# xinyandai/gradient-quantization

Hardware: NVIDIA B200
Metric: HSQ gradient elems/s (encode+allgather+decode) (higher is better)
Workload: dtype f32

## Files before the change

### gradient-quantization_b200/_lib.py

```python
import ctypes
import os

import torch

_HERE = os.path.dirname(os.path.abspath(__file__))
LIB_PATH = os.path.join(_HERE, "libgqb200.so")

c_void_p = ctypes.c_void_p
c_int = ctypes.c_int
c_i64 = ctypes.c_int64
c_u64 = ctypes.c_uint64
c_size = ctypes.c_size_t
c_float = ctypes.c_float

ALGO_AUTO, ALGO_EXACT, ALGO_TC = 0, 1, 2

_SIGNATURES = {
    "gq_abi_version": (c_int, []),
    "gq_device_info": (c_int, [ctypes.POINTER(c_int)] * 3 + [ctypes.POINTER(c_size)]),
    "gq_hsq_encode_workspace_bytes": (c_size, [c_i64, c_int, c_int, c_int]),
    "gq_hsq_encode": (c_int, [c_void_p, c_i64, c_int, c_void_p, c_int, c_void_p, c_int, c_int, c_int,
                              c_void_p, c_u64, c_u64, c_void_p, c_int, c_void_p, c_int, c_void_p,
                              c_void_p, c_void_p, c_size, c_int, c_void_p]),
    "gq_hsq_search": (c_int, [c_void_p, c_i64, c_int, c_void_p, c_int, c_void_p, c_int, c_void_p,
                              c_void_p, c_int, c_void_p, c_void_p, c_size, c_int, c_void_p]),
    "gq_norm_quantize": (c_int, [c_void_p, c_i64, c_void_p, c_int, c_int, c_int, c_void_p, c_u64, c_u64,
                                 c_void_p, c_int, c_void_p, c_void_p, c_int, c_void_p]),
    "gq_norm_dequantize": (c_int, [c_void_p, c_int, c_i64, c_void_p, c_int, c_int, c_void_p, c_void_p,
                                   c_void_p]),
    "gq_hsq_decode_reduce": (c_int, [c_void_p, c_int, c_void_p, c_int, c_void_p, c_void_p, c_i64, c_int,
                                     c_i64, c_int, c_void_p, c_int, c_void_p, c_int, c_int, c_int, c_int,
                                     c_void_p, c_void_p]),
    "gq_hsq_decode_reduce_scattered": (c_int, [c_void_p, c_int, c_void_p, c_int, c_void_p, c_void_p, c_int, c_i64,
                                               c_int, c_void_p, c_int, c_void_p, c_int, c_int, c_int, c_int,
                                               c_void_p, c_void_p]),
    "gq_f32_reduce_users_scattered": (c_int, [c_void_p, c_void_p, c_int, c_i64, c_int, c_int, c_void_p, c_void_p]),
    "gq_attach_f32_reduce": (c_int, [c_void_p, c_i64, c_void_p, c_int, c_i64, c_int, c_int, c_void_p]),
    "gq_ipc_alloc": (c_int, [c_size, ctypes.POINTER(c_void_p), c_void_p]),
    "gq_ipc_free": (c_int, [c_void_p]),
    "gq_ipc_open": (c_int, [c_void_p, ctypes.POINTER(c_void_p)]),
    "gq_ipc_close": (c_int, [c_void_p]),
    "gq_peer_barrier": (c_int, [c_void_p, c_int, c_int, ctypes.c_uint32, c_void_p]),
    "gq_peer_gather": (c_int, [c_void_p, c_void_p, c_size, c_size, c_int, c_void_p]),
    "gq_peer_push": (c_int, [c_void_p, c_void_p, c_size, c_int, c_void_p]),
    "gq_peer_push_multicast": (c_int, [c_void_p, c_void_p, c_size, c_void_p]),
    "gq_attach_remote_record": (c_int, [c_int, c_int, c_void_p, c_void_p, c_i64, c_void_p, c_int, ctypes.c_uint32]),
    "gq_attach_peer_wait": (c_int, [c_void_p, c_int, ctypes.c_uint32]),
    "gq_f32_reduce_users": (c_int, [c_void_p, c_i64, c_int, c_i64, c_int, c_int, c_void_p, c_void_p]),
    "gq_qsgd_wire_bits": (c_int, [c_int]),
    "gq_qsgd_encode": (c_int, [c_void_p, c_i64, c_void_p, c_i64, c_int, c_int, c_int, c_void_p, c_u64,
                               c_u64, c_void_p, c_void_p, c_void_p, c_void_p, c_void_p]),
    "gq_qsgd_decode_reduce": (c_int, [c_void_p, c_void_p, c_i64, c_int, c_i64, c_void_p, c_i64, c_int,
                                      c_int, c_int, c_int, c_void_p, c_void_p]),
    "gq_qsgd_decode_unpacked": (c_int, [c_void_p, c_void_p, c_void_p, c_i64, c_void_p, c_i64, c_int, c_int,
                                        c_void_p, c_void_p]),
    "gq_sign_encode": (c_int, [c_void_p, c_i64, c_void_p, c_void_p, c_void_p]),
    "gq_sign_decode_reduce": (c_int, [c_void_p, c_i64, c_int, c_i64, c_int, c_int, c_void_p, c_void_p]),
    "gq_sign_t5_bytes": (c_i64, [c_i64]),
    "gq_sign_encode_t5": (c_int, [c_void_p, c_i64, c_void_p, c_void_p]),
    "gq_sign_decode_reduce_t5": (c_int, [c_void_p, c_i64, c_int, c_i64, c_int, c_int, c_void_p, c_void_p]),
    "gq_topk_workspace_bytes": (c_size, [c_i64, c_int]),
    "gq_topk_select": (c_int, [c_void_p, c_i64, c_void_p, c_void_p, c_void_p, c_int, c_void_p, c_void_p,
                               c_void_p, c_void_p, c_size, c_void_p]),
    "gq_topk_scatter_reduce": (c_int, [c_void_p, c_void_p, c_i64, c_int, c_i64, c_i64, c_int, c_int,
                                       c_void_p, c_void_p]),
    "gq_pvc_search": (c_int, [c_void_p, c_i64, c_int, c_void_p, c_int, c_void_p, c_u64, c_u64, c_void_p,
                              c_int, c_void_p, c_void_p]),
    "gq_hsq_tc_debug": (c_int, [c_void_p, c_i64, c_void_p, c_void_p, c_void_p, c_void_p, c_int, c_void_p,
                                c_int, c_void_p]),
    "gq_hsq_tc2_trace": (c_int, [c_void_p, c_i64, c_void_p, c_void_p, c_void_p, c_void_p, c_int, c_void_p, c_void_p, c_void_p,
                                 c_void_p, c_void_p]),
    "gq_gather_f32": (c_int, [c_void_p, c_void_p, c_void_p, c_int, c_void_p, c_int, c_float, c_void_p]),
    "gq_axpy": (c_int, [c_void_p, c_void_p, c_float, c_i64, c_void_p, c_void_p]),
    "gq_sub": (c_int, [c_void_p, c_void_p, c_i64, c_void_p, c_void_p]),
    "gq_hsq_host_scratch_bytes": (c_size, [c_i64, c_int, c_int, c_int]),
    "gq_hsq_roundtrip_host": (c_int, [c_void_p, c_void_p, c_i64, c_int, c_void_p, c_int, c_void_p, c_int,
                                      c_int, c_int, c_u64, c_u64, c_void_p, c_size, c_int, c_void_p]),
}

EXPORTS = ["gq_last_error"] + sorted(_SIGNATURES)

_lib = None


class GQError(RuntimeError):
    pass


def load():
    global _lib
    if _lib is not None:
        return _lib
    if not os.path.exists(LIB_PATH):
        raise ImportError(
            "libgqb200.so is missing (%s). Build it with `python gradient-quantization_b200/build.py` "
            "or __graft_entry__.build(); there is no CPU fallback." % LIB_PATH)
    lib = ctypes.CDLL(LIB_PATH)
    lib.gq_last_error.restype = ctypes.c_char_p
    lib.gq_last_error.argtypes = []
    for name, (res, args) in _SIGNATURES.items():
        fn = getattr(lib, name)
        fn.restype = res
        fn.argtypes = args
    _lib = lib
    return lib


def call(name, *args):
    lib = load()
    rc = getattr(lib, name)(*args)
    if rc != 0:
        raise GQError("%s failed (%d): %s" % (name, rc, lib.gq_last_error().decode()))


def value(name, *args):
    return getattr(load(), name)(*args)


def require_cuda(t, what="tensor"):
    if not isinstance(t, torch.Tensor) or not t.is_cuda:
        raise GQError("%s must be a CUDA tensor: this implementation has no CPU path" % what)
    return t


def ptr(t):
    return None if t is None else t.data_ptr()


def stream():
    return torch.cuda.current_stream().cuda_stream


def f32c(t, what="tensor"):
    require_cuda(t, what)
    if t.dtype != torch.float32:
        t = t.float()
    return t if t.is_contiguous() else t.contiguous()


_M64 = 0xFFFFFFFFFFFFFFFF


def _mix64(seed, k):
    z = (seed + (k + 1) * 0x9E3779B97F4A7C15) & _M64
    z = ((z ^ (z >> 30)) * 0xBF58476D1CE4E5B9) & _M64
    z = ((z ^ (z >> 27)) * 0x94D049BB133111EB) & _M64
    return z ^ (z >> 31)


class PhiloxState:

    SHARED_STREAM = 1 << 32

    def __init__(self):
        self.shared_seed = None
        self.shared_offset = 0

    def _gen(self):
        return torch.cuda.default_generators[torch.cuda.current_device()]

    def take(self, n, user=0):
        gen = self._gen()
        seed = gen.initial_seed() & _M64
        off = int(gen.get_offset())
        gen.set_offset(off + (int(n) + 3) // 4 * 4)
        return _mix64(seed, int(user)), off

    def share_seed(self, seed=None):
        self.shared_seed = (self._gen().initial_seed() if seed is None else int(seed)) & _M64
        self.shared_offset = 0
        return self.shared_seed

    def take_shared(self, n):
        if self.shared_seed is None:
            self.share_seed()
        off = self.shared_offset
        self.shared_offset = off + (int(n) + 3) // 4 * 4
        return _mix64(self.shared_seed, self.SHARED_STREAM), off


PHILOX = PhiloxState()
```

### gradient-quantization_b200/csrc/abi.cu

```cuda
#include <stdarg.h>
#include <stdlib.h>
#include <string.h>

#include "gq_internal.cuh"

namespace gq {

static thread_local char g_err[512] = "";

void set_error(const char *fmt, ...)
{
    va_list ap;
    va_start(ap, fmt);
    vsnprintf(g_err, sizeof(g_err), fmt, ap);
    va_end(ap);
}

int check_cuda(cudaError_t e, const char *what)
{
    if (e == cudaSuccess) return GQ_OK;
    set_error("CUDA error %d (%s) at %s", (int)e, cudaGetErrorString(e), what);
    return GQ_ERR_CUDA;
}

int sm_count()
{
    static int cached[64] = {0};
    int dev = 0;
    if (cudaGetDevice(&dev) != cudaSuccess || dev < 0 || dev >= 64) return 148;
    if (cached[dev] == 0) {
        int n = 0;
        if (cudaDeviceGetAttribute(&n, cudaDevAttrMultiProcessorCount, dev) != cudaSuccess || n <= 0) n = 148;
        cached[dev] = n;
    }
    return cached[dev];
}

bool pdl_enabled()
{
    static const bool on = [] { const char *f = getenv("GQ_PDL"); return !(f && atoi(f) == 0); }();
    return on;
}

static size_t align_up(size_t x, size_t a) { return (x + a - 1) / a * a; }

int tc_generation()
{
    const char *f = getenv("GQ_TC_V");
    return (f && atoi(f) == 1) ? 1 : 2;
}

static thread_local Tc2Remote g_remote = {};
void set_remote(const Tc2Remote &r) { g_remote = r; }
Tc2Remote take_remote()
{
    Tc2Remote r = g_remote;
    g_remote = Tc2Remote{};
    return r;
}

}

using namespace gq;

extern "C" {

const char *gq_last_error(void) { return g_err; }
int gq_abi_version(void) { return 1; }

int gq_device_info(int *sm, int *cc_major, int *cc_minor, size_t *total_mem)
{
    int dev = 0;
    GQ_CUDA(cudaGetDevice(&dev));
    cudaDeviceProp p;
    GQ_CUDA(cudaGetDeviceProperties(&p, dev));
    if (sm) *sm = p.multiProcessorCount;
    if (cc_major) *cc_major = p.major;
    if (cc_minor) *cc_minor = p.minor;
    if (total_mem) *total_mem = p.totalGlobalMem;
    return GQ_OK;
}

size_t gq_hsq_encode_workspace_bytes(int64_t n_chunks, int d, int K, int n_seg)
{
    (void)d; (void)K;
    size_t keys = align_up((size_t)(n_seg > 0 ? n_seg : 1) * 2 * sizeof(uint32_t), 256);
    return keys + 256  + hsq_tc_workspace_bytes(n_chunks) + hsq_tck_workspace_bytes(d, K);
}

static int validate_group(const void *grad, int64_t n_chunks, int d, const void *codebook, int K,
                          const int64_t *seg_start, int n_seg)
{
    GQ_REQUIRE(n_chunks >= 0, "n_chunks %lld < 0", (long long)n_chunks);
    GQ_REQUIRE(d >= 1, "chunk dim %d < 1", d);
    GQ_REQUIRE(K >= 1, "codebook size %d < 1", K);
    GQ_REQUIRE(n_chunks == 0 || grad != nullptr, "null gradient pointer");
    GQ_REQUIRE(codebook != nullptr, "null codebook pointer");
    GQ_REQUIRE(n_seg >= 1 && seg_start != nullptr, "segment table required (n_seg >= 1)");
    return GQ_OK;
}

int gq_hsq_search(const float *grad, int64_t n_chunks, int d, const float *codebook, int K,
                  void *codes, int code_bytes, float *u_out, const int64_t *seg_start, int n_seg,
                  uint32_t *minmax_keys, void *workspace, size_t workspace_bytes, int algo,
                  gq_stream_t stream)
{
    int e = validate_group(grad, n_chunks, d, codebook, K, seg_start, n_seg);
    if (e) return e;
    GQ_REQUIRE(code_bytes == 1 || code_bytes == 4, "code_bytes must be 1 or 4 (got %d)", code_bytes);
    GQ_REQUIRE(code_bytes == 4 || K <= 256, "uint8 codes need K <= 256 (K = %d)", K);
    GQ_REQUIRE(n_chunks == 0 || (codes && u_out), "null output pointer");
    GQ_REQUIRE(((uintptr_t)grad & 15) == 0, "gradient must be 16-byte aligned");
    cudaStream_t st = as_stream(stream);
    const bool tc_ok = tc_generation() == 2 ? hsq_tc2_supported(d, K, code_bytes) : hsq_tc_supported(d, K, code_bytes);
    const bool tck_ok = !tc_ok && hsq_tck_supported(d, K, code_bytes) && workspace != nullptr &&
                        ((uintptr_t)workspace & 255) == 0 && workspace_bytes >= hsq_tck_workspace_bytes(d, K);
    if (algo == GQ_ALGO_TC && !tc_ok && !tck_ok) {
        set_error("tcgen05 search supports d in {8, 16, 32} with K == 256 (uint8 codes) or d == 16 with K = 512..4096, a multiple of 512 "
                  "(int32 codes, workspace of gq_hsq_encode_workspace_bytes); got d=%d K=%d code_bytes=%d",
                  d, K, code_bytes);
        return GQ_ERR_UNSUPPORTED;
    }
    if (tck_ok && algo != GQ_ALGO_EXACT && n_chunks > 0)
        return hsq_search_tck(grad, n_chunks, codebook, K, codes, u_out, seg_start, n_seg, minmax_keys, workspace,
                              workspace_bytes, st);
    if (tc_ok && algo != GQ_ALGO_EXACT && n_chunks > 0) {
        if (tc_generation() == 1)
            return hsq_search_tc(grad, n_chunks, d, codebook, K, codes, code_bytes, u_out, seg_start, n_seg,
                                 minmax_keys, workspace, workspace_bytes, st);
        return hsq_encode_tc2(grad, n_chunks, d, codebook, codes, u_out, seg_start, n_seg, minmax_keys, nullptr, nullptr,
                              Rider{}, nullptr, nullptr, st);
    }
    return hsq_search_exact(grad, n_chunks, d, codebook, K, codes, code_bytes, u_out, seg_start, n_seg,
                            minmax_keys, st);
}

int gq_hsq_tc2_trace(const float *grad, int64_t n_chunks, const float *codebook, void *codes, float *u_out,
                     const int64_t *seg_start, int n_seg, void *l, float *lbub, void *workspace, int64_t *trace,
                     gq_stream_t stream)
{
    GQ_REQUIRE(hsq_tc_supported(16, 256, 1), "tcgen05 search needs an sm_100 device");
    if (l == nullptr)
        return hsq_tc2_trace(grad, n_chunks, codebook, codes, u_out, nullptr, 0, nullptr, nullptr, nullptr, nullptr,
                             reinterpret_cast<long long *>(trace), as_stream(stream));
    GQ_REQUIRE(seg_start && n_seg >= 1 && lbub && workspace && ((uintptr_t)workspace & 255) == 0, "bad arguments");
    uint32_t *keys = reinterpret_cast<uint32_t *>(workspace);
    uint32_t *barrier = reinterpret_cast<uint32_t *>((char *)workspace + align_up((size_t)n_seg * 8, 256));
    Tc2Tail tail = {(uint8_t *)l, lbub, nullptr, 1234u, 0u, 6, 1};
    return hsq_tc2_trace(grad, n_chunks, codebook, codes, u_out, seg_start, n_seg, keys, reinterpret_cast<uint64_t *>(barrier) + 1,
                         barrier, &tail, reinterpret_cast<long long *>(trace), as_stream(stream));
}

int gq_norm_quantize(const float *u, int64_t n, const int64_t *seg_start, int n_seg, int n_bit,
                     int random, const float *uniforms, uint64_t philox_seed, uint64_t philox_offset,
                     void *l, int l_bytes, float *lbub, uint32_t *minmax_keys, int precomputed,
                     gq_stream_t stream)
{
    GQ_REQUIRE(n >= 0 && n_seg >= 1 && seg_start, "bad segment table");
    GQ_REQUIRE(n_bit >= 1 && n_bit <= 24, "n_bit %d out of range 1..24", n_bit);
    GQ_REQUIRE(l_bytes == 1 || l_bytes == 4, "l_bytes must be 1 or 4");
    GQ_REQUIRE(l_bytes == 4 || n_bit <= 7, "uint8 norm codes need n_bit <= 7 (levels 0..2^n)");
    GQ_REQUIRE(l && lbub && minmax_keys, "null output pointer");
    cudaStream_t st = as_stream(stream);
    if (!precomputed) {
        int e = launch_minmax_init(minmax_keys, n_seg, st);
        if (e) return e;
        e = launch_seg_minmax(u, n, seg_start, n_seg, minmax_keys, st);
        if (e) return e;
    }
    return launch_norm_quantize(u, n, seg_start, n_seg, n_bit, random, uniforms, philox_seed,
                                philox_offset, l, l_bytes, lbub, minmax_keys, st);
}

int gq_norm_dequantize(const void *l, int l_bytes, int64_t n, const int64_t *seg_start, int n_seg,
                       int n_bit, const float *lbub, float *out, gq_stream_t stream)
{
    GQ_REQUIRE(n >= 0 && n_seg >= 1 && seg_start, "bad segment table");
    GQ_REQUIRE(n_bit >= 1 && n_bit <= 24, "n_bit %d out of range 1..24", n_bit);
    GQ_REQUIRE(l_bytes == 1 || l_bytes == 4, "l_bytes must be 1 or 4");
    return launch_norm_dequantize(l, l_bytes, n, seg_start, n_seg, n_bit, lbub, out, as_stream(stream));
}

int gq_hsq_encode(const float *grad, int64_t n_chunks, int d, const float *codebook, int K,
                  const int64_t *seg_start, int n_seg, int n_bit, int random, const float *uniforms,
                  uint64_t philox_seed, uint64_t philox_offset, void *codes, int code_bytes, void *l,
                  int l_bytes, float *lbub, float *u_out, void *workspace, size_t workspace_bytes,
                  int algo, gq_stream_t stream)
{
    const Rider rider = take_rider();
    const Tc2Remote remote = take_remote();
    GQ_REQUIRE(n_bit == 32 || (n_bit >= 1 && n_bit <= 24), "n_bit %d out of range (1..24 or 32)", n_bit);
    const size_t need = gq_hsq_encode_workspace_bytes(n_chunks, d, K, n_seg);
    if (workspace_bytes < need || workspace == nullptr) {
        set_error("workspace too small: %zu < %zu", workspace_bytes, need);
        return GQ_ERR_WORKSPACE;
    }
    GQ_REQUIRE(((uintptr_t)workspace & 255) == 0, "workspace must be 256-byte aligned");
    cudaStream_t st = as_stream(stream);
    uint32_t *keys = reinterpret_cast<uint32_t *>(workspace);
    const size_t keys_bytes = align_up((size_t)n_seg * 2 * sizeof(uint32_t), 256);
    uint32_t *barrier = reinterpret_cast<uint32_t *>((char *)workspace + keys_bytes);
    const size_t head = keys_bytes + 256;
    int e = GQ_OK;
    static const bool want_fused = [] { const char *f = getenv("GQ_TC_FUSED"); return f && atoi(f) == 1; }();
    const bool fused = want_fused && (n_bit != 32) && (l_bytes == 1) && (algo != GQ_ALGO_EXACT) && n_chunks > 0 &&
                       hsq_tc_supported(d, K, code_bytes);
    if (fused) {
        e = validate_group(grad, n_chunks, d, codebook, K, seg_start, n_seg);
        if (e) return e;
        GQ_REQUIRE(codes && l && lbub && u_out, "null output pointer");
        GQ_REQUIRE(n_bit <= 7, "uint8 norm codes need n_bit <= 7 (levels 0..2^n)");
        GQ_REQUIRE(((uintptr_t)grad & 15) == 0, "gradient must be 16-byte aligned");
        e = launch_minmax_init_rider(keys, n_seg, st, barrier, rider);
        if (e) return e;
        return hsq_encode_tc_fused(grad, n_chunks, codebook, codes, u_out, seg_start, n_seg, keys, barrier, n_bit,
                                   random, uniforms, philox_seed, philox_offset, (uint8_t *)l, lbub, st);
    }
    const bool tc2_ok = tc_generation() == 2 && algo != GQ_ALGO_EXACT && n_chunks > 0 && hsq_tc2_supported(d, K, code_bytes);
    if (remote.n > 0 && !(tc2_ok && n_bit != 32 && hsq_tc2_tail_supported(n_seg, n_bit, l_bytes, u_out, uniforms, l, codes))) {
        set_error("a remote delivery is attached, but this encode cannot run as the fused tcgen05 kernel");
        return GQ_ERR_UNSUPPORTED;
    }
    if (tc2_ok) {
        e = validate_group(grad, n_chunks, d, codebook, K, seg_start, n_seg);
        if (e) return e;
        GQ_REQUIRE(codes && u_out, "null output pointer");
        uint64_t *flag = reinterpret_cast<uint64_t *>(barrier) + 1;
        if (n_bit == 32) {
            return hsq_encode_tc2(grad, n_chunks, d, codebook, codes, u_out, seg_start, n_seg, nullptr, nullptr, nullptr,
                                  rider, nullptr, nullptr, st);
        }
        GQ_REQUIRE(l && lbub, "null output pointer");
        if (hsq_tc2_tail_supported(n_seg, n_bit, l_bytes, u_out, uniforms, l, codes)) {
            Tc2Tail tail = {(uint8_t *)l, lbub, uniforms, philox_seed, philox_offset, n_bit, random};
            return hsq_encode_tc2(grad, n_chunks, d, codebook, codes, u_out, seg_start, n_seg, keys, flag, barrier, rider,
                                  &tail, remote.n > 0 ? &remote : nullptr, st);
        }
        e = hsq_encode_tc2(grad, n_chunks, d, codebook, codes, u_out, seg_start, n_seg, keys, flag, nullptr, rider,
                           nullptr, nullptr, st);
        if (e) return e;
        return gq_norm_quantize(u_out, n_chunks, seg_start, n_seg, n_bit, random, uniforms, philox_seed,
                                philox_offset, l, l_bytes, lbub, keys, 1, stream);
    }
    static const bool in_kernel_init = [] { const char *f = getenv("GQ_TC_INIT"); return !(f && atoi(f) == 0); }();
    if (n_bit != 32 && in_kernel_init && algo != GQ_ALGO_EXACT && n_chunks > 0 && hsq_tc_supported(d, K, code_bytes)) {
        e = validate_group(grad, n_chunks, d, codebook, K, seg_start, n_seg);
        if (e) return e;
        GQ_REQUIRE(codes && u_out, "null output pointer");
        GQ_REQUIRE(((uintptr_t)grad & 15) == 0, "gradient must be 16-byte aligned");
        e = hsq_search_tc_prepared(grad, n_chunks, codebook, codes, u_out, seg_start, n_seg, keys,
                                   reinterpret_cast<uint64_t *>(barrier) + 1, rider, st);
        if (e) return e;
        return gq_norm_quantize(u_out, n_chunks, seg_start, n_seg, n_bit, random, uniforms, philox_seed,
                                philox_offset, l, l_bytes, lbub, keys, 1, stream);
    }
    if (n_bit != 32) {
        e = launch_minmax_init_rider(keys, n_seg, st, nullptr, rider);
        if (e) return e;
    } else {
        e = launch_rider(rider, st);
        if (e) return e;
    }
    e = gq_hsq_search(grad, n_chunks, d, codebook, K, codes, code_bytes, u_out, seg_start, n_seg,
                      n_bit != 32 ? keys : nullptr, (char *)workspace + head, workspace_bytes - head, algo,
                      stream);
    if (e) return e;
    if (n_bit == 32) return GQ_OK;
    return gq_norm_quantize(u_out, n_chunks, seg_start, n_seg, n_bit, random, uniforms, philox_seed,
                            philox_offset, l, l_bytes, lbub, keys, 1, stream);
}

int gq_hsq_decode_reduce(const void *codes, int code_bytes, const void *l, int l_bytes,
                         const float *lbub, const float *norms_f32, int64_t user_stride_bytes,
                         int n_users, int64_t n_chunks, int d, const float *codebook, int K,
                         const int64_t *seg_start, int n_seg, int n_bit, int mean, int accumulate,
                         float *out, gq_stream_t stream)
{
    const Rider pending = take_rider();
    int e = validate_group(out, n_chunks, d, codebook, K, seg_start, n_seg);
    if (e) return e;
    GQ_REQUIRE(n_users >= 1, "n_users %d < 1", n_users);
    GQ_REQUIRE(code_bytes == 1 || code_bytes == 4, "code_bytes must be 1 or 4");
    GQ_REQUIRE(n_bit == 32 || (n_bit >= 1 && n_bit <= 24), "n_bit %d out of range", n_bit);
    if (n_bit == 32) {
        GQ_REQUIRE(norms_f32 != nullptr, "n_bit == 32 needs norms_f32");
        l_bytes = 1;
    } else {
        GQ_REQUIRE(l && lbub, "null l / lbub");
        GQ_REQUIRE(l_bytes == 1 || l_bytes == 4, "l_bytes must be 1 or 4");
    }
    GQ_REQUIRE(n_users == 1 || (user_stride_bytes % 4) == 0, "user stride must be a multiple of 4 bytes");
    GQ_REQUIRE(((uintptr_t)out & 15) == 0, "output must be 16-byte aligned");
    set_rider(pending);
    e = hsq_decode_reduce(codes, code_bytes, l, l_bytes, lbub, norms_f32, user_stride_bytes, nullptr, n_users,
                          n_chunks, d, codebook, K, seg_start, n_seg, n_bit, mean, accumulate, out,
                          as_stream(stream));
    const Rider left = take_rider();
    if (e) return e;
    return launch_rider(left, as_stream(stream));
}

int gq_hsq_decode_reduce_scattered(const void *codes, int code_bytes, const void *l, int l_bytes,
                                   const float *lbub, const int64_t *user_byte_offsets, int n_users,
                                   int64_t n_chunks, int d, const float *codebook, int K,
                                   const int64_t *seg_start, int n_seg, int n_bit, int mean, int accumulate,
                                   float *out, gq_stream_t stream)
{
    const Rider pending = take_rider();
    int e = validate_group(out, n_chunks, d, codebook, K, seg_start, n_seg);
    if (e) return e;
    GQ_REQUIRE(n_users >= 1 && n_users <= 8 && user_byte_offsets, "1..8 users with an offset table");
    GQ_REQUIRE(code_bytes == 1 || code_bytes == 4, "code_bytes must be 1 or 4");
    GQ_REQUIRE(n_bit >= 1 && n_bit <= 24 && l && lbub, "quantized norms required (n_bit 1..24)");
    GQ_REQUIRE(l_bytes == 1 || l_bytes == 4, "l_bytes must be 1 or 4");
    GQ_REQUIRE(((uintptr_t)out & 15) == 0, "output must be 16-byte aligned");
    set_rider(pending);
    e = hsq_decode_reduce(codes, code_bytes, l, l_bytes, lbub, nullptr, 0, user_byte_offsets, n_users, n_chunks,
                          d, codebook, K, seg_start, n_seg, n_bit, mean, accumulate, out, as_stream(stream));
    const Rider left = take_rider();
    if (e) return e;
    return launch_rider(left, as_stream(stream));
}

int gq_f32_reduce_users(const float *in, int64_t user_stride_bytes, int n_users, int64_t n, int mean,
                        int accumulate, float *out, gq_stream_t stream)
{
    GQ_REQUIRE(n >= 0 && n_users >= 1, "bad sizes");
    GQ_REQUIRE(n == 0 || (in && out), "null pointer");
    return launch_f32_reduce_users(in, user_stride_bytes, nullptr, n_users, n, mean, accumulate, out,
                                   as_stream(stream));
}

int gq_f32_reduce_users_scattered(const float *in, const int64_t *user_byte_offsets, int n_users, int64_t n,
                                  int mean, int accumulate, float *out, gq_stream_t stream)
{
    GQ_REQUIRE(n >= 0 && n_users >= 1 && n_users <= 8 && user_byte_offsets, "1..8 users with an offset table");
    GQ_REQUIRE(n == 0 || (in && out), "null pointer");
    return launch_f32_reduce_users(in, 0, user_byte_offsets, n_users, n, mean, accumulate, out, as_stream(stream));
}

int gq_attach_f32_reduce(const float *in, int64_t user_stride_bytes, const int64_t *user_byte_offsets, int n_users,
                         int64_t n, int mean, int accumulate, float *out)
{
    GQ_REQUIRE(n >= 0 && n_users >= 1 && n_users <= 8, "1..8 users");
    GQ_REQUIRE(n == 0 || (in && out), "null pointer");
    Rider r = {};
    r.in = in;
    for (int u = 0; u < n_users; ++u) r.off[u] = user_byte_offsets ? user_byte_offsets[u] : (int64_t)u * user_stride_bytes;
    r.n_users = n_users;
    r.n = n;
    r.mean = mean;
    r.accumulate = accumulate;
    r.out = out;
    set_rider(r);
    return GQ_OK;
}

int gq_axpy(const float *a, const float *b, float alpha, int64_t n, float *out, gq_stream_t stream)
{
    GQ_REQUIRE(n >= 0 && (n == 0 || (a && b && out)), "bad arguments");
    return launch_axpy(a, b, alpha, n, out, 0, as_stream(stream));
}

int gq_sub(const float *a, const float *b, int64_t n, float *out, gq_stream_t stream)
{
    GQ_REQUIRE(n >= 0 && (n == 0 || (a && b && out)), "bad arguments");
    return launch_axpy(a, b, 0.0f, n, out, 1, as_stream(stream));
}

static size_t host_scratch_layout(int64_t n_chunks, int d, int K, int n_seg, size_t off[6])
{
    size_t p = 0;
    off[0] = p; p += align_up((size_t)n_chunks * d * 4, 256);
    off[1] = p; p += align_up((size_t)n_chunks, 256);
    off[2] = p; p += align_up((size_t)n_chunks, 256);
    off[3] = p; p += align_up((size_t)n_seg * 2 * 4, 256);
    off[4] = p; p += align_up((size_t)n_chunks * 4, 256);
    off[5] = p; p += gq_hsq_encode_workspace_bytes(n_chunks, d, K, n_seg);
    return p;
}

size_t gq_hsq_host_scratch_bytes(int64_t n_chunks, int d, int K, int n_seg)
{
    size_t off[6];
    return host_scratch_layout(n_chunks, d, K, n_seg, off);
}

int gq_hsq_roundtrip_host(const float *host_grad, float *host_out, int64_t n_chunks, int d,
                          const float *dev_codebook, int K, const int64_t *dev_seg_start, int n_seg,
                          int n_bit, int random, uint64_t philox_seed, uint64_t philox_offset,
                          void *dev_scratch, size_t scratch_bytes, int algo, gq_stream_t stream)
{
    GQ_REQUIRE(K <= 256 && n_bit <= 7, "host round trip uses the uint8 wire format (K <= 256, n_bit <= 7)");
    size_t off[6];
    const size_t need = host_scratch_layout(n_chunks, d, K, n_seg, off);
    if (scratch_bytes < need || !dev_scratch) {
        set_error("scratch too small: %zu < %zu", scratch_bytes, need);
        return GQ_ERR_WORKSPACE;
    }
    cudaStream_t st = as_stream(stream);
    char *base = (char *)dev_scratch;
    float *g = (float *)(base + off[0]);
    const size_t bytes = (size_t)n_chunks * d * 4;
    GQ_CUDA(cudaMemcpyAsync(g, host_grad, bytes, cudaMemcpyHostToDevice, st));
    int e = gq_hsq_encode(g, n_chunks, d, dev_codebook, K, dev_seg_start, n_seg, n_bit, random, nullptr,
                          philox_seed, philox_offset, base + off[1], 1, base + off[2], 1,
                          (float *)(base + off[3]), (float *)(base + off[4]), base + off[5],
                          need - off[5], algo, stream);
    if (e) return e;
    e = gq_hsq_decode_reduce(base + off[1], 1, base + off[2], 1, (float *)(base + off[3]), nullptr, 0, 1,
                             n_chunks, d, dev_codebook, K, dev_seg_start, n_seg, n_bit, 0, 0, g, stream);
    if (e) return e;
    GQ_CUDA(cudaMemcpyAsync(host_out, g, bytes, cudaMemcpyDeviceToHost, st));
    GQ_CUDA(cudaStreamSynchronize(st));
    return GQ_OK;
}

}
```

### gradient-quantization_b200/csrc/gq_common.cuh

```cuda
#pragma once
#include <cuda_runtime.h>
#include <stdint.h>
#include <stdio.h>

#include "../../include/gqb200.h"

#if defined(__CUDA_ARCH__) && (__CUDA_ARCH__ < 1000)
#error "libgqb200 is written for sm_100a (B200) only"
#endif

namespace gq {

void set_error(const char *fmt, ...);
int check_cuda(cudaError_t e, const char *what);
int sm_count();

#define GQ_REQUIRE(cond, ...)                \
    do {                                     \
        if (!(cond)) {                       \
            gq::set_error(__VA_ARGS__);      \
            return GQ_ERR_INVALID;           \
        }                                    \
    } while (0)

#define GQ_CUDA(expr)                                        \
    do {                                                     \
        int _e = gq::check_cuda((expr), #expr);              \
        if (_e) return _e;                                   \
    } while (0)

#define GQ_LAUNCH_CHECK(name) GQ_CUDA((cudaError_t)cudaPeekAtLastError())

static inline cudaStream_t as_stream(gq_stream_t s) { return reinterpret_cast<cudaStream_t>(s); }

__device__ __forceinline__ void pdl_launch_dependents() { asm volatile("griddepcontrol.launch_dependents;" ::: "memory"); }
__device__ __forceinline__ void pdl_wait() { asm volatile("griddepcontrol.wait;" ::: "memory"); }
bool pdl_enabled();

template <typename... KArgs, typename... Args>
static inline cudaError_t launch_pdl(void (*kern)(KArgs...), dim3 grid, dim3 block, size_t smem, cudaStream_t st,
                                     Args... args)
{
    cudaLaunchConfig_t cfg = {};
    cfg.gridDim = grid;
    cfg.blockDim = block;
    cfg.dynamicSmemBytes = smem;
    cfg.stream = st;
    cudaLaunchAttribute attr[1];
    attr[0].id = cudaLaunchAttributeProgrammaticStreamSerialization;
    attr[0].val.programmaticStreamSerializationAllowed = 1;
    cfg.attrs = attr;
    cfg.numAttrs = pdl_enabled() ? 1 : 0;
    return cudaLaunchKernelEx(&cfg, kern, KArgs(args)...);
}

__host__ __device__ __forceinline__ uint32_t float_to_key(float f)
{
#ifdef __CUDA_ARCH__
    uint32_t b = __float_as_uint(f);
#else
    union { float f; uint32_t u; } c; c.f = f; uint32_t b = c.u;
#endif
    return (b & 0x80000000u) ? ~b : (b | 0x80000000u);
}
__host__ __device__ __forceinline__ float key_to_float(uint32_t k)
{
    uint32_t b = (k & 0x80000000u) ? (k & 0x7fffffffu) : ~k;
#ifdef __CUDA_ARCH__
    return __uint_as_float(b);
#else
    union { float f; uint32_t u; } c; c.u = b; return c.f;
#endif
}
#define GQ_KEY_MIN_INIT 0xffffffffu
#define GQ_KEY_MAX_INIT 0x00000000u
#define GQ_KEY_NAN 0xffc00000u

__device__ __forceinline__ uint4 philox4x32_10(uint64_t seed, uint64_t idx)
{
    uint32_t k0 = (uint32_t)seed, k1 = (uint32_t)(seed >> 32);
    uint32_t c0 = (uint32_t)idx, c1 = (uint32_t)(idx >> 32), c2 = 0u, c3 = 0u;
#pragma unroll
    for (int r = 0; r < 10; ++r) {
        uint32_t hi0 = __umulhi(0xD2511F53u, c0), lo0 = 0xD2511F53u * c0;
        uint32_t hi1 = __umulhi(0xCD9E8D57u, c2), lo1 = 0xCD9E8D57u * c2;
        uint32_t n0 = hi1 ^ c1 ^ k0, n1 = lo1, n2 = hi0 ^ c3 ^ k1, n3 = lo0;
        c0 = n0; c1 = n1; c2 = n2; c3 = n3;
        k0 += 0x9E3779B9u; k1 += 0xBB67AE85u;
    }
    return make_uint4(c0, c1, c2, c3);
}
__device__ __forceinline__ float u01(uint32_t x) { return (float)(x >> 8) * 5.9604644775390625e-08f; }
__device__ __forceinline__ float philox_uniform(uint64_t seed, uint64_t offset, uint64_t i)
{
    uint64_t g = offset + i;
    uint4 w = philox4x32_10(seed, g >> 2);
    uint32_t s = (uint32_t)(g & 3u);
    uint32_t x = (s == 0) ? w.x : (s == 1) ? w.y : (s == 2) ? w.z : w.w;
    return u01(x);
}

__device__ __forceinline__ int find_segment(const int64_t *__restrict__ seg_start, int n_seg, int64_t i)
{
    int lo = 0, hi = n_seg;
    while (hi - lo > 1) {
        int mid = (lo + hi) >> 1;
        if (__ldg(seg_start + mid) <= i) lo = mid; else hi = mid;
    }
    return lo;
}

struct SegCache {
    int seg = 0;
    int64_t lo = 0, hi = 0;
};
__device__ __forceinline__ int cached_segment(SegCache &sc, const int64_t *__restrict__ seg_start, int n_seg,
                                              int64_t i)
{
    if (i < sc.lo || i >= sc.hi) {
        sc.seg = find_segment(seg_start, n_seg, i);
        sc.lo = __ldg(seg_start + sc.seg);
        sc.hi = __ldg(seg_start + sc.seg + 1);
    }
    return sc.seg;
}

__device__ __forceinline__ int find_segment_smem(const int64_t *s_seg, int n_seg, int64_t i)
{
    int lo = 0, hi = n_seg;
    while (hi - lo > 1) {
        int mid = (lo + hi) >> 1;
        if (s_seg[mid] <= i) lo = mid; else hi = mid;
    }
    return lo;
}
__device__ __forceinline__ int cached_segment_smem(SegCache &sc, const int64_t *s_seg, int n_seg, int64_t i)
{
    if (i < sc.lo || i >= sc.hi) {
        sc.seg = find_segment_smem(s_seg, n_seg, i);
        sc.lo = s_seg[sc.seg];
        sc.hi = s_seg[sc.seg + 1];
    }
    return sc.seg;
}

__device__ __forceinline__ int psc_level(float v, float lb, float ub, float s, int random, float r)
{
    if (lb - ub == 0.0f) return 0;
    float scaled = fabsf(__fdiv_rn(__fsub_rn(v, lb), __fsub_rn(ub, lb))) * s;
    float c = fminf(fmaxf(scaled, 0.0f), s - 1.0f);
    int li = (int)c;
    if (random) {
        float prob = __fsub_rn(scaled, (float)li);
        li += (prob > r) ? 1 : 0;
    }
    return li;
}
__device__ __forceinline__ float psc_value(int l, float lb, float ub, float inv_s)
{
    return __fadd_rn(__fmul_rn(__fmul_rn((float)l, __fsub_rn(ub, lb)), inv_s), lb);
}

__device__ __forceinline__ float warp_min(float v)
{
#pragma unroll
    for (int o = 16; o > 0; o >>= 1) v = fminf(v, __shfl_xor_sync(0xffffffffu, v, o));
    return v;
}
__device__ __forceinline__ float warp_max(float v)
{
#pragma unroll
    for (int o = 16; o > 0; o >>= 1) v = fmaxf(v, __shfl_xor_sync(0xffffffffu, v, o));
    return v;
}

__device__ __forceinline__ float4 ld_stream_f4(const float4 *p)
{
    float4 r;
    asm volatile("ld.global.nc.L1::no_allocate.v4.f32 {%0,%1,%2,%3}, [%4];"
                 : "=f"(r.x), "=f"(r.y), "=f"(r.z), "=f"(r.w) : "l"(p));
    return r;
}

}
```

### gradient-quantization_b200/csrc/gq_internal.cuh

```cuda
#pragma once
#include "gq_common.cuh"

namespace gq {

int launch_minmax_init(uint32_t *keys, int n_seg, cudaStream_t st, uint32_t *barrier = nullptr);

struct Rider {
    const float *in;
    int64_t off[8];
    int n_users;
    int64_t n;
    int mean, accumulate;
    float *out;
};
Rider take_rider();
void set_rider(const Rider &r);
int launch_rider(const Rider &r, cudaStream_t st);
__device__ __forceinline__ void rider_run(const Rider &r, int64_t tid, int64_t nthreads)
{
    for (int64_t i = tid; i < r.n; i += nthreads) {
        float acc = 0.0f;
#pragma unroll
        for (int u = 0; u < 8; ++u) {
            if (u < r.n_users) {
                const float x = *reinterpret_cast<const float *>(reinterpret_cast<const char *>(r.in) + r.off[u] + 4 * i);
                acc = (u == 0) ? x : __fadd_rn(acc, x);
            }
        }
        if (r.mean) acc = __fdiv_rn(acc, (float)r.n_users);
        if (r.accumulate) acc = (r.accumulate == 2) ? __fsub_rn(r.out[i], acc) : __fadd_rn(r.out[i], acc);
        r.out[i] = acc;
    }
}
int launch_minmax_init_rider(uint32_t *keys, int n_seg, cudaStream_t st, uint32_t *barrier, const Rider &rider);
int hsq_search_exact(const float *grad, int64_t n_chunks, int d, const float *codebook, int K,
                     void *codes, int code_bytes, float *u_out, const int64_t *seg_start, int n_seg,
                     uint32_t *minmax_keys, cudaStream_t st);

bool hsq_tc_supported(int d, int K, int code_bytes);
size_t hsq_tc_workspace_bytes(int64_t n_chunks);
int hsq_search_tc(const float *grad, int64_t n_chunks, int d, const float *codebook, int K,
                  void *codes, int code_bytes, float *u_out, const int64_t *seg_start, int n_seg,
                  uint32_t *minmax_keys, void *workspace, size_t workspace_bytes, cudaStream_t st);

int hsq_search_tc_prepared(const float *grad, int64_t n_chunks, const float *codebook, void *codes, float *u_out,
                           const int64_t *seg_start, int n_seg, uint32_t *minmax_keys, uint64_t *flag,
                           const Rider &rider, cudaStream_t st);

int hsq_encode_tc_fused(const float *grad, int64_t n_chunks, const float *codebook, void *codes, float *u_out,
                        const int64_t *seg_start, int n_seg, uint32_t *minmax_keys, uint32_t *barrier,
                        int n_bit, int random, const float *uniforms, uint64_t seed, uint64_t offset,
                        uint8_t *l, float *lbub, cudaStream_t st);

bool hsq_tck_supported(int d, int K, int code_bytes);
size_t hsq_tck_workspace_bytes(int d, int K);
int hsq_search_tck(const float *grad, int64_t n_chunks, const float *codebook, int K, void *codes, float *u_out,
                   const int64_t *seg_start, int n_seg, uint32_t *minmax_keys, void *workspace, size_t workspace_bytes,
                   cudaStream_t st);

int tc_generation();

struct Tc2Tail {
    uint8_t *l;
    float *lbub;
    const float *uniforms;
    uint64_t seed, offset;
    int n_bit, random;
};
struct Tc2Remote {
    int n;
    int multicast;
    int64_t delta[7];
    const uint8_t *ident;
    int64_t ident_bytes;
    uint32_t *flag[8];
    int n_flag;
    uint32_t epoch;
};
bool hsq_tc2_tail_supported(int n_seg, int n_bit, int l_bytes, const void *u_out, const void *uniforms, const void *l,
                            const void *codes);
bool hsq_tc2_supported(int d, int K, int code_bytes);
int hsq_encode_tc2(const float *grad, int64_t n_chunks, int d, const float *codebook, void *codes, float *u_out,
                   const int64_t *seg_start, int n_seg, uint32_t *keys, uint64_t *flag, uint32_t *barrier,
                   const Rider &rider, const Tc2Tail *tail, const Tc2Remote *remote, cudaStream_t st);
int hsq_tc2_trace(const float *grad, int64_t n_chunks, const float *codebook, void *codes, float *u_out,
                  const int64_t *seg_start, int n_seg, uint32_t *keys, uint64_t *flag, uint32_t *barrier,
                  const Tc2Tail *tail, long long *trace, cudaStream_t st);
Tc2Remote take_remote();
void set_remote(const Tc2Remote &r);

struct PeerWait {
    const uint32_t *flags;
    int n;
    uint32_t epoch;
    unsigned long long timeout_ns;
};
void set_wait(const PeerWait &w);
PeerWait take_wait();
int flush_wait(cudaStream_t st);
__device__ __forceinline__ void peer_wait_flag(const uint32_t *flag, uint32_t epoch, unsigned long long timeout_ns)
{
    unsigned long long t0 = 0ull;
    for (;;) {
        uint32_t seen;
        asm volatile("ld.acquire.sys.global.u32 %0, [%1];" : "=r"(seen) : "l"(flag) : "memory");
        if ((int32_t)(seen - epoch) >= 0) return;
        __nanosleep(64);
        unsigned long long now;
        asm volatile("mov.u64 %0, %%globaltimer;" : "=l"(now));
        if (t0 == 0ull) t0 = now;
        else if (now - t0 > timeout_ns) __trap();
    }
}
unsigned long long peer_timeout_ns();
#define GQ_CUDA_INT(expr) do { int _e2 = (expr); if (_e2) return _e2; } while (0)

int launch_seg_minmax(const float *u, int64_t n, const int64_t *seg_start, int n_seg, uint32_t *keys,
                      cudaStream_t st);
int launch_norm_quantize(const float *u, int64_t n, const int64_t *seg_start, int n_seg, int n_bit,
                         int random, const float *uniforms, uint64_t seed, uint64_t offset, void *l,
                         int l_bytes, float *lbub, const uint32_t *keys, cudaStream_t st);
int launch_norm_dequantize(const void *l, int l_bytes, int64_t n, const int64_t *seg_start, int n_seg,
                           int n_bit, const float *lbub, float *out, cudaStream_t st);
struct UserOffsets {
    int64_t off[8];
};
int hsq_decode_reduce(const void *codes, int code_bytes, const void *l, int l_bytes, const float *lbub,
                      const float *norms_f32, int64_t user_stride, const int64_t *user_offsets, int n_users,
                      int64_t n_chunks, int d,
                      const float *codebook, int K, const int64_t *seg_start, int n_seg, int n_bit,
                      int mean, int accumulate, float *out, cudaStream_t st);
int launch_f32_reduce_users(const float *in, int64_t user_stride, const int64_t *user_offsets, int n_users,
                            int64_t n, int mean, int accumulate, float *out, cudaStream_t st);
int launch_axpy(const float *a, const float *b, float alpha, int64_t n, float *out, int sub,
                cudaStream_t st);

template <typename CodeT>
__device__ __forceinline__ void search_epilogue(bool valid, int64_t c, int best_k, float best_u,
                                                CodeT *__restrict__ codes, float *__restrict__ u_out,
                                                const int64_t *__restrict__ seg_start, int n_seg,
                                                uint32_t *__restrict__ minmax_keys, SegCache &segc)
{
    if (valid) {
        codes[c] = (CodeT)best_k;
        u_out[c] = best_u;
    }
    if (minmax_keys == nullptr) return;
    int seg = valid ? cached_segment(segc, seg_start, n_seg, c) : -1;
    int seg0 = __shfl_sync(0xffffffffu, seg, 0);
    bool uniform = __all_sync(0xffffffffu, (seg == seg0) || !valid) && (seg0 >= 0);
    if (valid && best_u != best_u) atomicMax(minmax_keys + 2 * seg + 1, GQ_KEY_NAN);
    if (uniform) {
        float mn = warp_min(valid ? best_u : INFINITY);
        float mx = warp_max(valid ? best_u : -INFINITY);
        if ((threadIdx.x & 31) == 0) {
            atomicMin(minmax_keys + 2 * seg0, float_to_key(mn));
            atomicMax(minmax_keys + 2 * seg0 + 1, float_to_key(mx));
        }
    } else if (valid) {
        atomicMin(minmax_keys + 2 * seg, float_to_key(best_u));
        atomicMax(minmax_keys + 2 * seg + 1, float_to_key(best_u));
    }
}


template <typename LT, bool VOLATILE_KEYS>
__device__ __forceinline__ void quantize_range(const float *__restrict__ u, int64_t i_begin, int64_t i_end,
                                               int64_t n, int tid, int nthreads,
                                               const int64_t *__restrict__ seg_start, int n_seg, float s,
                                               int random, const float *__restrict__ uniforms, uint64_t seed,
                                               uint64_t offset, LT *__restrict__ l, const uint32_t *keys)
{
    SegCache segc;
    float lb = 0.0f, ub = 0.0f;
    int cur = -1;
    const bool aligned = ((reinterpret_cast<uintptr_t>(u) & 15) == 0) &&
                         (uniforms == nullptr || (reinterpret_cast<uintptr_t>(uniforms) & 15) == 0) &&
                         ((reinterpret_cast<uintptr_t>(l) & (4 * sizeof(LT) - 1)) == 0);
    for (int64_t i0 = i_begin + 4 * (int64_t)tid; i0 < i_end; i0 += 4 * (int64_t)nthreads) {
        const int64_t q = i0 >> 2;
        const bool full = aligned && (i0 + 3 < n);
        float x[4], r[4] = {0.f, 0.f, 0.f, 0.f};
        if (full) {
            const float4 t = VOLATILE_KEYS ? __ldcg(reinterpret_cast<const float4 *>(u) + q)
                                           : __ldg(reinterpret_cast<const float4 *>(u) + q);
            x[0] = t.x; x[1] = t.y; x[2] = t.z; x[3] = t.w;
        } else {
#pragma unroll
            for (int t = 0; t < 4; ++t) x[t] = (i0 + t < n) ? u[i0 + t] : 0.0f;
        }
        if (random) {
            if (uniforms) {
                if (full) {
                    const float4 t = __ldg(reinterpret_cast<const float4 *>(uniforms) + q);
                    r[0] = t.x; r[1] = t.y; r[2] = t.z; r[3] = t.w;
                } else {
#pragma unroll
                    for (int t = 0; t < 4; ++t) r[t] = (i0 + t < n) ? uniforms[i0 + t] : 0.0f;
                }
            } else if (((offset + (uint64_t)i0) & 3u) == 0) {
                const uint4 w = philox4x32_10(seed, (offset + (uint64_t)i0) >> 2);
                r[0] = u01(w.x); r[1] = u01(w.y); r[2] = u01(w.z); r[3] = u01(w.w);
            } else {
#pragma unroll
                for (int t = 0; t < 4; ++t) r[t] = philox_uniform(seed, offset, (uint64_t)(i0 + t));
            }
        }
        int lv[4];
#pragma unroll
        for (int t = 0; t < 4; ++t) {
            const int64_t i = i0 + t;
            if (i < n) {
                const int seg = cached_segment(segc, seg_start, n_seg, i);
                if (seg != cur) {
                    cur = seg;
                    if (VOLATILE_KEYS) {
                        lb = key_to_float(__ldcg(keys + 2 * seg));
                        ub = key_to_float(__ldcg(keys + 2 * seg + 1));
                    } else {
                        lb = key_to_float(__ldg(keys + 2 * seg));
                        ub = key_to_float(__ldg(keys + 2 * seg + 1));
                    }
                }
                lv[t] = psc_level(x[t], lb, ub, s, random, r[t]);
            } else {
                lv[t] = 0;
            }
        }
        if (full) {
            if (sizeof(LT) == 1) {
                reinterpret_cast<uint32_t *>(l)[q] =
                    (uint32_t)lv[0] | ((uint32_t)lv[1] << 8) | ((uint32_t)lv[2] << 16) | ((uint32_t)lv[3] << 24);
            } else {
                reinterpret_cast<int4 *>(l)[q] = make_int4(lv[0], lv[1], lv[2], lv[3]);
            }
        } else {
#pragma unroll
            for (int t = 0; t < 4; ++t)
                if (i0 + t < n) l[i0 + t] = (LT)lv[t];
        }
    }
}

struct MinMaxAcc {
    int seg = -1;
    float mn = INFINITY, mx = -INFINITY;
};
__device__ __forceinline__ void minmax_flush_warp(MinMaxAcc &a, uint32_t *__restrict__ keys)
{
    const uint32_t have = __ballot_sync(0xffffffffu, a.seg >= 0);
    if (have != 0u) {
        const int seg0 = __shfl_sync(0xffffffffu, a.seg, __ffs(have) - 1);
        const bool uniform = __all_sync(0xffffffffu, a.seg == seg0 || a.seg < 0);
        if (uniform) {
            const float mn = warp_min(a.mn), mx = warp_max(a.mx);
            if ((threadIdx.x & 31) == 0) {
                atomicMin(keys + 2 * seg0, float_to_key(mn));
                atomicMax(keys + 2 * seg0 + 1, float_to_key(mx));
            }
        } else if (a.seg >= 0) {
            atomicMin(keys + 2 * a.seg, float_to_key(a.mn));
            atomicMax(keys + 2 * a.seg + 1, float_to_key(a.mx));
        }
    }
    a.seg = -1;
    a.mn = INFINITY;
    a.mx = -INFINITY;
}
__device__ __forceinline__ void minmax_add_warp(MinMaxAcc &a, bool valid, int seg, float u,
                                                uint32_t *__restrict__ keys)
{
    if (__any_sync(0xffffffffu, valid && a.seg >= 0 && seg != a.seg)) minmax_flush_warp(a, keys);
    if (valid && u != u) atomicMax(keys + 2 * seg + 1, GQ_KEY_NAN);
    if (valid) {
        a.seg = seg;
        a.mn = fminf(a.mn, u);
        a.mx = fmaxf(a.mx, u);
    }
}

}
```

### gradient-quantization_b200/csrc/hsq_tail.cu

```cuda
#include <stdlib.h>

#include "gq_internal.cuh"

namespace gq {

__global__ void __launch_bounds__(256)
seg_minmax_kernel(const float *__restrict__ u, int64_t n, const int64_t *__restrict__ seg_start,
                  int n_seg, uint32_t *__restrict__ keys)
{
    SegCache segc;
    for (int64_t base = (int64_t)blockIdx.x * 256; base < n; base += (int64_t)gridDim.x * 256) {
        int64_t i = base + threadIdx.x;
        bool valid = i < n;
        float x = valid ? u[i] : 0.0f;
        int seg = valid ? cached_segment(segc, seg_start, n_seg, i) : -1;
        int seg0 = __shfl_sync(0xffffffffu, seg, 0);
        bool uniform = __all_sync(0xffffffffu, (seg == seg0) || !valid) && (seg0 >= 0);
        if (valid && x != x) atomicMax(keys + 2 * seg + 1, GQ_KEY_NAN);
        if (uniform) {
            float mn = warp_min(valid ? x : INFINITY);
            float mx = warp_max(valid ? x : -INFINITY);
            if ((threadIdx.x & 31) == 0) {
                atomicMin(keys + 2 * seg0, float_to_key(mn));
                atomicMax(keys + 2 * seg0 + 1, float_to_key(mx));
            }
        } else if (valid) {
            atomicMin(keys + 2 * seg, float_to_key(x));
            atomicMax(keys + 2 * seg + 1, float_to_key(x));
        }
    }
}

template <typename LT>
__global__ void __launch_bounds__(256)
norm_quantize_kernel(const float *__restrict__ u, int64_t n, const int64_t *__restrict__ seg_start,
                     int n_seg, float s, int random, const float *__restrict__ uniforms,
                     uint64_t seed, uint64_t offset, LT *__restrict__ l, float *__restrict__ lbub,
                     const uint32_t *__restrict__ keys)
{
    if (blockIdx.x == 0) {
        for (int i = threadIdx.x; i < 2 * n_seg; i += 256) lbub[i] = key_to_float(keys[i]);
    }
    quantize_range<LT, false>(u, 0, n, n, (int)(blockIdx.x * 256 + threadIdx.x), (int)(gridDim.x * 256), seg_start,
                              n_seg, s, random, uniforms, seed, offset, l, keys);
}

constexpr int kQuantMaxSeg = 1024;
__device__ __forceinline__ int psc_level_nz(float v, float lb, float den, float s, int random, float r)
{
    const float scaled = fabsf(__fdiv_rn(__fsub_rn(v, lb), den)) * s;
    const float c = fminf(fmaxf(scaled, 0.0f), s - 1.0f);
    int li = (int)c;
    if (random) li += (__fsub_rn(scaled, (float)li) > r) ? 1 : 0;
    return li;
}
template <typename LT>
__global__ void __launch_bounds__(256)
norm_quantize_smem_kernel(const float *__restrict__ u, int n, const int64_t *__restrict__ seg_start,
                          int n_seg, float s, int random, const float *__restrict__ uniforms,
                          uint64_t seed, uint64_t offset, LT *__restrict__ l, float *__restrict__ lbub,
                          const uint32_t *__restrict__ keys, int items)
{
    extern __shared__ int s_segi[];
    float2 *s_lbub2 = reinterpret_cast<float2 *>(s_segi + ((n_seg + 2) & ~1));
    const int tid = threadIdx.x;
    pdl_launch_dependents();
    for (int i = tid; i <= n_seg; i += 256) s_segi[i] = (int)seg_start[i];
    pdl_wait();
    for (int i = tid; i < n_seg; i += 256) {
        const float lb = key_to_float(keys[2 * i]), ub = key_to_float(keys[2 * i + 1]);
        s_lbub2[i] = make_float2(lb, ub);
        if (blockIdx.x == 0) {
            lbub[2 * i] = lb;
            lbub[2 * i + 1] = ub;
        }
    }
    const int n4 = (n + 3) >> 2;
    const int stride = gridDim.x * 256;
    int q = blockIdx.x * 256 + tid;
    float4 xv = make_float4(0.f, 0.f, 0.f, 0.f), rv = make_float4(0.f, 0.f, 0.f, 0.f);
    if (q < n4 && q * 4 + 3 < n) {
        xv = __ldg(reinterpret_cast<const float4 *>(u) + q);
        if (random && uniforms) rv = __ldg(reinterpret_cast<const float4 *>(uniforms) + q);
    }
    const bool philox = random && !uniforms;
    const bool philox_aligned = (offset & 3u) == 0;
    __syncthreads();
    for (int it = 0; it < items; ++it, q += stride) {
        const int block_i0 = (blockIdx.x * 256 + it * stride) * 4;
        int base = -1;
        for (int j0 = 0; j0 < n_seg; j0 += 256)
            base += __syncthreads_count(j0 + tid < n_seg && s_segi[j0 + tid] <= block_i0);
        if (q >= n4) continue;
        const bool full = q * 4 + 3 < n;
        const int i0 = q * 4;
        float x[4] = {xv.x, xv.y, xv.z, xv.w}, r[4] = {rv.x, rv.y, rv.z, rv.w};
        {
            const int qn = q + stride;
            if (it + 1 < items && qn < n4 && qn * 4 + 3 < n) {
                xv = __ldg(reinterpret_cast<const float4 *>(u) + qn);
                if (random && uniforms) rv = __ldg(reinterpret_cast<const float4 *>(uniforms) + qn);
            }
        }
        if (!full) {
#pragma unroll
            for (int t = 0; t < 4; ++t) {
                x[t] = (i0 + t < n) ? u[i0 + t] : 0.0f;
                r[t] = (random && uniforms && i0 + t < n) ? uniforms[i0 + t] : 0.0f;
            }
        }
        if (philox) {
            if (philox_aligned) {
                const uint4 w = philox4x32_10(seed, (offset + (uint64_t)i0) >> 2);
                r[0] = u01(w.x); r[1] = u01(w.y); r[2] = u01(w.z); r[3] = u01(w.w);
            } else {
#pragma unroll
                for (int t = 0; t < 4; ++t) r[t] = philox_uniform(seed, offset, (uint64_t)(i0 + t));
            }
        }
        int seg = base < 0 ? 0 : base;
        while (i0 >= s_segi[seg + 1]) ++seg;
        int lv[4];
        if (i0 + 3 < s_segi[seg + 1]) {
            const float2 b = s_lbub2[seg];
            if (b.x - b.y == 0.0f) {
                lv[0] = lv[1] = lv[2] = lv[3] = 0;
            } else {
                const float den = __fsub_rn(b.y, b.x);
#pragma unroll
                for (int t = 0; t < 4; ++t) lv[t] = psc_level_nz(x[t], b.x, den, s, random, r[t]);
            }
        } else {
#pragma unroll
            for (int t = 0; t < 4; ++t) {
                const int i = i0 + t;
                if (i < n) {
                    while (i >= s_segi[seg + 1]) ++seg;
                    const float2 b = s_lbub2[seg];
                    lv[t] = psc_level(x[t], b.x, b.y, s, random, r[t]);
                } else {
                    lv[t] = 0;
                }
            }
        }
        if (full) {
            if (sizeof(LT) == 1) {
                reinterpret_cast<uint32_t *>(l)[q] =
                    (uint32_t)lv[0] | ((uint32_t)lv[1] << 8) | ((uint32_t)lv[2] << 16) | ((uint32_t)lv[3] << 24);
            } else {
                reinterpret_cast<int4 *>(l)[q] = make_int4(lv[0], lv[1], lv[2], lv[3]);
            }
        } else {
#pragma unroll
            for (int t = 0; t < 4; ++t)
                if (i0 + t < n) l[i0 + t] = (LT)lv[t];
        }
    }
}

template <typename LT>
__global__ void __launch_bounds__(256)
norm_dequantize_kernel(const LT *__restrict__ l, int64_t n, const int64_t *__restrict__ seg_start,
                       int n_seg, float s, const float *__restrict__ lbub, float *__restrict__ out)
{
    SegCache segc;
    for (int64_t base = (int64_t)blockIdx.x * 256; base < n; base += (int64_t)gridDim.x * 256) {
        int64_t i = base + threadIdx.x;
        if (i >= n) continue;
        int seg = cached_segment(segc, seg_start, n_seg, i);
        out[i] = psc_value((int)l[i], __ldg(lbub + 2 * seg), __ldg(lbub + 2 * seg + 1), 1.0f / s);
    }
}

static int grid_for(int64_t n, int per_block, int waves = 8)
{
    int64_t blocks = (n + per_block - 1) / per_block;
    int64_t cap = (int64_t)sm_count() * waves;
    int64_t g = blocks < cap ? blocks : cap;
    return (int)(g < 1 ? 1 : g);
}

int launch_seg_minmax(const float *u, int64_t n, const int64_t *seg_start, int n_seg, uint32_t *keys,
                      cudaStream_t st)
{
    if (n == 0) return GQ_OK;
    seg_minmax_kernel<<<grid_for(n, 256), 256, 0, st>>>(u, n, seg_start, n_seg, keys);
    GQ_LAUNCH_CHECK("seg_minmax");
    return GQ_OK;
}

int launch_norm_quantize(const float *u, int64_t n, const int64_t *seg_start, int n_seg, int n_bit,
                         int random, const float *uniforms, uint64_t seed, uint64_t offset, void *l,
                         int l_bytes, float *lbub, const uint32_t *keys, cudaStream_t st)
{
    const float s = (float)(1u << n_bit);
    const int64_t n4 = (n + 3) / 4;
    const bool aligned = (((uintptr_t)u & 15) == 0) && (uniforms == nullptr || ((uintptr_t)uniforms & 15) == 0) &&
                         (((uintptr_t)l & (4 * (size_t)l_bytes - 1)) == 0);
    if (n_seg <= kQuantMaxSeg && aligned && n4 > 0 && n < ((int64_t)1 << 31) - 8) {
        const size_t smem = (size_t)((n_seg + 2) & ~1) * 4 + (size_t)n_seg * 8;
        const int64_t blocks = (n4 + 255) / 256;
        int occ = 1;
        if (l_bytes == 1)
            GQ_CUDA(cudaOccupancyMaxActiveBlocksPerMultiprocessor(&occ, norm_quantize_smem_kernel<uint8_t>, 256, smem));
        else
            GQ_CUDA(cudaOccupancyMaxActiveBlocksPerMultiprocessor(&occ, norm_quantize_smem_kernel<int32_t>, 256, smem));
        const int64_t cap = (int64_t)sm_count() * (occ < 1 ? 1 : occ);
        const int items = (int)((blocks + cap - 1) / cap);
        const unsigned grid = (unsigned)((blocks + items - 1) / items);
        if (l_bytes == 1)
            GQ_CUDA(launch_pdl(norm_quantize_smem_kernel<uint8_t>, dim3(grid), dim3(256), smem, st, u, (int)n, seg_start,
                               n_seg, s, random, uniforms, seed, offset, (uint8_t *)l, lbub, keys, items));
        else
            GQ_CUDA(launch_pdl(norm_quantize_smem_kernel<int32_t>, dim3(grid), dim3(256), smem, st, u, (int)n, seg_start,
                               n_seg, s, random, uniforms, seed, offset, (int32_t *)l, lbub, keys, items));
        return GQ_OK;
    }
    const int grid = grid_for(n > 0 ? n4 : 1, 256);
    if (l_bytes == 1)
        norm_quantize_kernel<uint8_t><<<grid, 256, 0, st>>>(u, n, seg_start, n_seg, s, random, uniforms,
                                                            seed, offset, (uint8_t *)l, lbub, keys);
    else
        norm_quantize_kernel<int32_t><<<grid, 256, 0, st>>>(u, n, seg_start, n_seg, s, random, uniforms,
                                                            seed, offset, (int32_t *)l, lbub, keys);
    GQ_LAUNCH_CHECK("norm_quantize");
    return GQ_OK;
}

int launch_norm_dequantize(const void *l, int l_bytes, int64_t n, const int64_t *seg_start, int n_seg,
                           int n_bit, const float *lbub, float *out, cudaStream_t st)
{
    if (n == 0) return GQ_OK;
    const float s = (float)(1u << n_bit);
    const int grid = grid_for(n, 256);
    if (l_bytes == 1)
        norm_dequantize_kernel<uint8_t><<<grid, 256, 0, st>>>((const uint8_t *)l, n, seg_start, n_seg, s, lbub, out);
    else
        norm_dequantize_kernel<int32_t><<<grid, 256, 0, st>>>((const int32_t *)l, n, seg_start, n_seg, s, lbub, out);
    GQ_LAUNCH_CHECK("norm_dequantize");
    return GQ_OK;
}

__device__ __forceinline__ float combine1(float o, float r, int accumulate)
{
    return accumulate == 2 ? __fsub_rn(o, r) : __fadd_rn(o, r);
}
__device__ __forceinline__ float4 combine4(float4 o, float4 r, int accumulate)
{
    return accumulate == 2 ? make_float4(__fsub_rn(o.x, r.x), __fsub_rn(o.y, r.y), __fsub_rn(o.z, r.z), __fsub_rn(o.w, r.w))
                           : make_float4(__fadd_rn(o.x, r.x), __fadd_rn(o.y, r.y), __fadd_rn(o.z, r.z), __fadd_rn(o.w, r.w));
}

constexpr int kDecodeThreads = 256;
constexpr int kDecodeUnroll = 4;

template <int D, typename CodeT, typename LT, bool CB_SMEM>
__global__ void __launch_bounds__(kDecodeThreads)
hsq_decode_reduce_kernel(const CodeT *__restrict__ codes, const LT *__restrict__ l,
                         const float *__restrict__ lbub, const float *__restrict__ norms_f32,
                         int64_t user_stride, int n_users, int64_t n_chunks,
                         const float *__restrict__ codebook, int K,
                         const int64_t *__restrict__ seg_start, int n_seg, float s, int n_bit,
                         int mean, int accumulate, float *__restrict__ out)
{
    extern __shared__ float4 s_cbd[];
    constexpr int D4 = D / 4;
    const float4 *cb4g = reinterpret_cast<const float4 *>(codebook);
    if (CB_SMEM) {
        for (int i = threadIdx.x; i < K * D4; i += kDecodeThreads) s_cbd[i] = __ldg(cb4g + i);
        __syncthreads();
    }
    const float inv_s = 1.0f / s;
    const float nu = (float)n_users;
    const bool pow2 = (n_users & (n_users - 1)) == 0;
    const float inv_nu = 1.0f / nu;
    SegCache segc;
    const int64_t n4 = n_chunks * D4;
    constexpr int64_t kSpan = (int64_t)kDecodeThreads * kDecodeUnroll;
    float4 *o4 = reinterpret_cast<float4 *>(out);
    for (int64_t base = (int64_t)blockIdx.x * kSpan; base < n4; base += (int64_t)gridDim.x * kSpan) {
        int64_t f[kDecodeUnroll], c[kDecodeUnroll];
        int part[kDecodeUnroll], seg[kDecodeUnroll];
        bool ok[kDecodeUnroll];
        float4 acc[kDecodeUnroll];
#pragma unroll
        for (int j = 0; j < kDecodeUnroll; ++j) {
            f[j] = base + j * kDecodeThreads + threadIdx.x;
            ok[j] = f[j] < n4;
            c[j] = ok[j] ? f[j] / D4 : 0;
            part[j] = (int)(f[j] % D4);
            seg[j] = (ok[j] && n_bit != 32) ? cached_segment(segc, seg_start, n_seg, c[j]) : 0;
            acc[j] = make_float4(0.f, 0.f, 0.f, 0.f);
        }
        for (int u = 0; u < n_users; ++u) {
            const char *cu = reinterpret_cast<const char *>(codes) + u * user_stride;
            int code[kDecodeUnroll];
            float norm[kDecodeUnroll];
            if (n_bit == 32) {
                const char *nup = reinterpret_cast<const char *>(norms_f32) + u * user_stride;
#pragma unroll
                for (int j = 0; j < kDecodeUnroll; ++j) {
                    code[j] = ok[j] ? (int)reinterpret_cast<const CodeT *>(cu)[c[j]] : 0;
                    norm[j] = ok[j] ? reinterpret_cast<const float *>(nup)[c[j]] : 0.0f;
                }
            } else {
                const char *lu = reinterpret_cast<const char *>(l) + u * user_stride;
                const float *b = reinterpret_cast<const float *>(reinterpret_cast<const char *>(lbub) + u * user_stride);
                int lv[kDecodeUnroll];
#pragma unroll
                for (int j = 0; j < kDecodeUnroll; ++j) {
                    code[j] = ok[j] ? (int)reinterpret_cast<const CodeT *>(cu)[c[j]] : 0;
                    lv[j] = ok[j] ? (int)reinterpret_cast<const LT *>(lu)[c[j]] : 0;
                }
#pragma unroll
                for (int j = 0; j < kDecodeUnroll; ++j)
                    norm[j] = psc_value(lv[j], __ldg(b + 2 * seg[j]), __ldg(b + 2 * seg[j] + 1), inv_s);
            }
#pragma unroll
            for (int j = 0; j < kDecodeUnroll; ++j) {
                const float4 cw = CB_SMEM ? s_cbd[code[j] * D4 + part[j]]
                                          : __ldg(cb4g + (int64_t)code[j] * D4 + part[j]);
                float4 pr;
                pr.x = __fmul_rn(cw.x, norm[j]); pr.y = __fmul_rn(cw.y, norm[j]);
                pr.z = __fmul_rn(cw.z, norm[j]); pr.w = __fmul_rn(cw.w, norm[j]);
                if (u == 0) {
                    acc[j] = pr;
                } else {
                    acc[j].x = __fadd_rn(acc[j].x, pr.x); acc[j].y = __fadd_rn(acc[j].y, pr.y);
                    acc[j].z = __fadd_rn(acc[j].z, pr.z); acc[j].w = __fadd_rn(acc[j].w, pr.w);
                }
            }
        }
#pragma unroll
        for (int j = 0; j < kDecodeUnroll; ++j) {
            if (!ok[j]) continue;
            float4 r = acc[j];
            if (mean && n_users > 1) {
                if (pow2) {
                    r.x = __fmul_rn(r.x, inv_nu); r.y = __fmul_rn(r.y, inv_nu);
                    r.z = __fmul_rn(r.z, inv_nu); r.w = __fmul_rn(r.w, inv_nu);
                } else {
                    r.x = __fdiv_rn(r.x, nu); r.y = __fdiv_rn(r.y, nu);
                    r.z = __fdiv_rn(r.z, nu); r.w = __fdiv_rn(r.w, nu);
                }
            }
            if (accumulate) {
                const float4 o = o4[f[j]];
                r = combine4(o, r, accumulate);
            }
            o4[f[j]] = r;
        }
    }
}

template <typename CodeT, typename LT>
__global__ void __launch_bounds__(256)
hsq_decode_reduce_generic_kernel(const CodeT *__restrict__ codes, const LT *__restrict__ l,
                                 const float *__restrict__ lbub, const float *__restrict__ norms_f32,
                                 int64_t user_stride, int n_users, int64_t n_chunks, int d,
                                 const float *__restrict__ codebook,
                                 const int64_t *__restrict__ seg_start, int n_seg, float s, int n_bit,
                                 int mean, int accumulate, float *__restrict__ out)
{
    const int64_t n = n_chunks * (int64_t)d;
    for (int64_t e = (int64_t)blockIdx.x * 256 + threadIdx.x; e < n; e += (int64_t)gridDim.x * 256) {
        const int64_t c = e / d;
        const int j = (int)(e % d);
        int seg = (n_bit != 32) ? find_segment(seg_start, n_seg, c) : 0;
        float acc = 0.0f;
        for (int u = 0; u < n_users; ++u) {
            const char *cu = reinterpret_cast<const char *>(codes) + u * user_stride;
            int code = (int)reinterpret_cast<const CodeT *>(cu)[c];
            float norm;
            if (n_bit == 32) {
                const char *nu = reinterpret_cast<const char *>(norms_f32) + u * user_stride;
                norm = reinterpret_cast<const float *>(nu)[c];
            } else {
                const char *lu = reinterpret_cast<const char *>(l) + u * user_stride;
                const char *bu = reinterpret_cast<const char *>(lbub) + u * user_stride;
                const float *b = reinterpret_cast<const float *>(bu);
                norm = psc_value((int)reinterpret_cast<const LT *>(lu)[c], __ldg(b + 2 * seg),
                                 __ldg(b + 2 * seg + 1), 1.0f / s);
            }
            float pr = __fmul_rn(__ldg(codebook + (int64_t)code * d + j), norm);
            acc = (u == 0) ? pr : __fadd_rn(acc, pr);
        }
        if (mean) acc = __fdiv_rn(acc, (float)n_users);
        if (accumulate) acc = combine1(out[e], acc, accumulate);
        out[e] = acc;
    }
}

__device__ __forceinline__ float2 mul2(float2 a, float b)
{
    float2 r;
    asm("{\n\t.reg .b64 ra, rb, rd;\n\t"
        "mov.b64 ra, {%2, %3};\n\tmov.b64 rb, {%4, %4};\n\t"
        "mul.rn.f32x2 rd, ra, rb;\n\t"
        "mov.b64 {%0, %1}, rd;\n\t}"
        : "=f"(r.x), "=f"(r.y) : "f"(a.x), "f"(a.y), "f"(b));
    return r;
}
template <int D, int MAXU, typename CodeT, typename LT>
__global__ void __launch_bounds__(kDecodeThreads)
hsq_decode_reduce_warp_kernel(const CodeT *__restrict__ codes, const LT *__restrict__ l,
                              const float *__restrict__ lbub, const float *__restrict__ norms_f32,
                              const UserOffsets uoff, int n_users, int64_t n_chunks,
                              const float *__restrict__ codebook, int K,
                              const int64_t *__restrict__ seg_start, int n_seg, float s, int n_bit,
                              int mean, int accumulate, float *__restrict__ out)
{
    extern __shared__ float4 s_cbd[];
    constexpr int D4 = D / 4;
    static_assert((D4 & (D4 - 1)) == 0 && D4 <= 4, "D = 4, 8 or 16");
    const float4 *cb4g = reinterpret_cast<const float4 *>(codebook);
    pdl_launch_dependents();
    for (int i = threadIdx.x; i < K * D4; i += kDecodeThreads) s_cbd[i] = __ldg(cb4g + i);
    __syncthreads();
    pdl_wait();
    const int lane = threadIdx.x & 31;
    constexpr int kWarps = kDecodeThreads / 32;
    const float inv_s = 1.0f / s;
    const float nu = (float)n_users;
    const bool pow2 = (n_users & (n_users - 1)) == 0;
    const float inv_nu = 1.0f / nu;
    SegCache segc;
    const int64_t n_slots = (n_chunks + 31) / 32;
    const int64_t n4 = n_chunks * D4;
    float4 *o4 = reinterpret_cast<float4 *>(out);
    for (int64_t slot = (int64_t)blockIdx.x * kWarps + (threadIdx.x >> 5); slot < n_slots;
         slot += (int64_t)gridDim.x * kWarps) {
        const int64_t c = slot * 32 + lane;
        const bool ok = c < n_chunks;
        int code[MAXU];
        float nrm[MAXU];
#pragma unroll
        for (int u = 0; u < MAXU; ++u) {
            code[u] = 0;
            nrm[u] = 0.0f;
            if (u < n_users && ok) {
                const char *cu = reinterpret_cast<const char *>(codes) + uoff.off[u];
                code[u] = (int)reinterpret_cast<const CodeT *>(cu)[c];
                if (n_bit == 32) {
                    const char *nf = reinterpret_cast<const char *>(norms_f32) + uoff.off[u];
                    nrm[u] = reinterpret_cast<const float *>(nf)[c];
                } else {
                    const char *lu = reinterpret_cast<const char *>(l) + uoff.off[u];
                    nrm[u] = (float)(int)reinterpret_cast<const LT *>(lu)[c];
                }
            }
        }
        if (n_bit != 32) {
            const int seg = ok ? cached_segment(segc, seg_start, n_seg, c) : 0;
#pragma unroll
            for (int u = 0; u < MAXU; ++u) {
                if (u < n_users) {
                    const float *b = reinterpret_cast<const float *>(reinterpret_cast<const char *>(lbub) + uoff.off[u]);
                    const float lb = __ldg(b + 2 * seg), ub = __ldg(b + 2 * seg + 1);
                    nrm[u] = __fadd_rn(__fmul_rn(__fmul_rn(nrm[u], __fsub_rn(ub, lb)), inv_s), lb);
                }
            }
        }
        const int64_t f0 = slot * 32 * D4;
#pragma unroll
        for (int r = 0; r < D4; ++r) {
            const int fl = r * 32 + lane;
            const int owner = fl / D4;
            const int part = fl % D4;
            float2 a0 = make_float2(0.f, 0.f), a1 = make_float2(0.f, 0.f);
#pragma unroll
            for (int u = 0; u < MAXU; ++u) {
                if (u < n_users) {
                    const int cd = __shfl_sync(0xffffffffu, code[u], owner);
                    const float nm = __shfl_sync(0xffffffffu, nrm[u], owner);
                    const float4 cw = s_cbd[cd * D4 + part];
                    const float2 p0 = mul2(make_float2(cw.x, cw.y), nm);
                    const float2 p1 = mul2(make_float2(cw.z, cw.w), nm);
                    if (u == 0) {
                        a0 = p0; a1 = p1;
                    } else {
                        a0.x = __fadd_rn(a0.x, p0.x); a0.y = __fadd_rn(a0.y, p0.y);
                        a1.x = __fadd_rn(a1.x, p1.x); a1.y = __fadd_rn(a1.y, p1.y);
                    }
                }
            }
            float4 acc = make_float4(a0.x, a0.y, a1.x, a1.y);
            const int64_t f = f0 + fl;
            if (f < n4) {
                if (mean && n_users > 1) {
                    if (pow2) {
                        acc.x = __fmul_rn(acc.x, inv_nu); acc.y = __fmul_rn(acc.y, inv_nu);
                        acc.z = __fmul_rn(acc.z, inv_nu); acc.w = __fmul_rn(acc.w, inv_nu);
                    } else {
                        acc.x = __fdiv_rn(acc.x, nu); acc.y = __fdiv_rn(acc.y, nu);
                        acc.z = __fdiv_rn(acc.z, nu); acc.w = __fdiv_rn(acc.w, nu);
                    }
                }
                if (accumulate) {
                    const float4 o = o4[f];
                    acc = combine4(o, acc, accumulate);
                }
                o4[f] = acc;
            }
        }
    }
}

constexpr int kStTile = 1024;
__device__ __forceinline__ void cp_async16(void *smem_dst, const void *gsrc)
{
    asm volatile("cp.async.cg.shared.global [%0], [%1], 16;" ::"r"((uint32_t)__cvta_generic_to_shared(smem_dst)),
                 "l"(gsrc) : "memory");
}
__device__ __forceinline__ float4 lds128(uint32_t saddr)
{
    float4 r;
    asm("ld.shared.v4.f32 {%0, %1, %2, %3}, [%4];" : "=f"(r.x), "=f"(r.y), "=f"(r.z), "=f"(r.w) : "r"(saddr));
    return r;
}
__device__ __forceinline__ uint32_t lds_u8(uint32_t saddr)
{
    uint32_t r;
    asm volatile("ld.shared.u8 %0, [%1];" : "=r"(r) : "r"(saddr) : "memory");
    return r;
}
template <int NU>
__global__ void __launch_bounds__(kDecodeThreads)
hsq_decode_reduce_staged_kernel(const uint8_t *__restrict__ codes, const uint8_t *__restrict__ l,
                                const float *__restrict__ lbub, const UserOffsets uoff,
                                int64_t n_chunks, const float *__restrict__ codebook,
                                const int64_t *__restrict__ seg_start, int n_seg, float s, int mean,
                                int accumulate, float *__restrict__ out, const Rider rider, const PeerWait wait)
{
    extern __shared__ float4 s_dyn[];
    float4 *s_cb = s_dyn;
    uint8_t *s_stage = reinterpret_cast<uint8_t *>(s_cb + 256 * 8);
    float2 *s_lbub = reinterpret_cast<float2 *>(s_stage + 2 * NU * 2 * kStTile);
    int64_t *s_seg = reinterpret_cast<int64_t *>(s_lbub + NU * n_seg);
    __shared__ int64_t s_off[8];
    const int tid = threadIdx.x, lane = tid & 31;
    const int warp = __shfl_sync(0xffffffffu, tid >> 5, 0);
    pdl_launch_dependents();
    if (tid == 0) {
#pragma unroll
        for (int u = 0; u < 8; ++u) s_off[u] = uoff.off[u];
    }
    for (int i = tid; i < 256 * 8; i += kDecodeThreads)
        s_cb[i] = __ldg(reinterpret_cast<const float4 *>(codebook) + (i >> 3) * 4 + (i & 3));
    for (int i = tid; i <= n_seg; i += kDecodeThreads) s_seg[i] = __ldg(seg_start + i);
    __syncthreads();
    pdl_wait();
    if (wait.n > 0) {
        if (tid < wait.n) peer_wait_flag(wait.flags + tid, wait.epoch, wait.timeout_ns);
        __syncthreads();
    }
    const int64_t n_tiles = (n_chunks + kStTile - 1) / kStTile;
    auto issue = [&](int64_t tile, int buf) {
        const int64_t c0 = tile * kStTile;
        const int64_t left = n_chunks - c0;
        const int pieces = (int)(((left < kStTile ? left : (int64_t)kStTile) + 15) >> 4);
        for (int i = tid; i < NU * 128; i += kDecodeThreads) {
            const int u = i >> 7, which = (i >> 6) & 1, piece = i & 63;
            if (piece < pieces) {
                const char *src = (which ? reinterpret_cast<const char *>(l) : reinterpret_cast<const char *>(codes)) +
                                  s_off[u] + c0 + piece * 16;
                cp_async16(s_stage + ((buf * NU + u) * 2 + which) * kStTile + piece * 16, src);
            }
        }
        asm volatile("cp.async.commit_group;" ::: "memory");
    };
    const float inv_s = 1.0f / s;
    const float nu = (float)NU;
    constexpr bool pow2 = (NU & (NU - 1)) == 0;
    const float inv_nu = 1.0f / nu;
    const uint32_t cb_lane = (uint32_t)__cvta_generic_to_shared(s_cb) + (uint32_t)(((lane >> 2) & 1) * 64 + (lane & 3) * 16);
    const uint32_t stage0 = (uint32_t)__cvta_generic_to_shared(s_stage);
    SegCache segc;
    float4 *o4 = reinterpret_cast<float4 *>(out);
    const int64_t n4 = n_chunks * 4;
    int64_t tile = blockIdx.x;
    int buf = 0;
    if (tile < n_tiles) issue(tile, 0);
    for (int i = tid; i < NU * n_seg; i += kDecodeThreads) {
        const int u = i / n_seg, sg = i - u * n_seg;
        const float2 *b = reinterpret_cast<const float2 *>(reinterpret_cast<const char *>(lbub) + s_off[u]);
        s_lbub[i] = __ldcv(b + sg);
    }
    rider_run(rider, (int64_t)blockIdx.x * kDecodeThreads + tid, (int64_t)gridDim.x * kDecodeThreads);
    for (; tile < n_tiles; tile += gridDim.x, buf ^= 1) {
        const int64_t next = tile + gridDim.x;
        if (next < n_tiles) {
            issue(next, buf ^ 1);
            asm volatile("cp.async.wait_group 1;" ::: "memory");
        } else {
            asm volatile("cp.async.wait_group 0;" ::: "memory");
        }
        __syncthreads();
        const uint32_t st = stage0 + (uint32_t)(buf * NU * 2 * kStTile);
        const int64_t c0 = tile * kStTile;
        for (int sl = warp; sl < kStTile / 32; sl += kDecodeThreads / 32) {
            const int64_t c = c0 + sl * 32 + lane;
            if (c0 + sl * 32 >= n_chunks) break;
            const bool ok = c < n_chunks;
            const int seg = ok ? cached_segment_smem(segc, s_seg, n_seg, c) : 0;
            constexpr bool kPack = NU >= 3;
            const int seg0 = __shfl_sync(0xffffffffu, seg, 0);
            const bool uni = kPack && __all_sync(0xffffffffu, !ok || seg == seg0);
            uint32_t code[NU];
            float nrm[NU];
            float den[NU];
            uint32_t pk[(NU + 1) / 2];
#pragma unroll
            for (int u = 0; u < NU; ++u) {
                const uint32_t cb8 = lds_u8(st + (uint32_t)((u * 2) * kStTile + sl * 32 + lane));
                const uint32_t lv8 = lds_u8(st + (uint32_t)((u * 2 + 1) * kStTile + sl * 32 + lane));
                const float2 b = s_lbub[u * n_seg + (uni ? seg0 : seg)];
                code[u] = cb8 << 7;
                den[u] = __fsub_rn(b.y, b.x);
                if (uni) {
                    nrm[u] = b.x;
                    const uint32_t h = cb8 | (lv8 << 8);
                    if (u & 1) pk[u >> 1] |= h << 16; else pk[u >> 1] = h;
                } else {
                    nrm[u] = __fadd_rn(__fmul_rn(__fmul_rn((float)(int)lv8, den[u]), inv_s), b.x);
                }
            }
            const int64_t f0 = (c0 + sl * 32) * 4;
#pragma unroll
            for (int r = 0; r < 4; ++r) {
                const int owner = r * 8 + (lane >> 2);
                float4 cw[NU];
                float nm[NU];
                if (uni) {
#pragma unroll
                    for (int j = 0; j < (NU + 1) / 2; ++j) {
                        const uint32_t w = __shfl_sync(0xffffffffu, pk[j], owner);
                        cw[2 * j] = lds128(cb_lane + ((w & 0xffu) << 7));
                        nm[2 * j] = __fadd_rn(__fmul_rn(__fmul_rn((float)(int)((w >> 8) & 0xffu), den[2 * j]), inv_s), nrm[2 * j]);
                        if (2 * j + 1 < NU) {
                            cw[2 * j + 1] = lds128(cb_lane + (((w >> 16) & 0xffu) << 7));
                            nm[2 * j + 1] = __fadd_rn(__fmul_rn(__fmul_rn((float)(int)(w >> 24), den[2 * j + 1]), inv_s), nrm[2 * j + 1]);
                        }
                    }
                } else {
#pragma unroll
                    for (int u = 0; u < NU; ++u) {
                        const uint32_t cd = __shfl_sync(0xffffffffu, code[u], owner);
                        nm[u] = __shfl_sync(0xffffffffu, nrm[u], owner);
                        cw[u] = lds128(cb_lane + cd);
                    }
                }
                float2 a0 = mul2(make_float2(cw[0].x, cw[0].y), nm[0]);
                float2 a1 = mul2(make_float2(cw[0].z, cw[0].w), nm[0]);
#pragma unroll
                for (int u = 1; u < NU; ++u) {
                    const float2 p0 = mul2(make_float2(cw[u].x, cw[u].y), nm[u]);
                    const float2 p1 = mul2(make_float2(cw[u].z, cw[u].w), nm[u]);
                    a0.x = __fadd_rn(a0.x, p0.x); a0.y = __fadd_rn(a0.y, p0.y);
                    a1.x = __fadd_rn(a1.x, p1.x); a1.y = __fadd_rn(a1.y, p1.y);
                }
                float4 acc = make_float4(a0.x, a0.y, a1.x, a1.y);
                const int64_t f = f0 + r * 32 + lane;
                if (f < n4) {
                    if (mean && NU > 1) {
                        if (pow2) {
                            acc.x = __fmul_rn(acc.x, inv_nu); acc.y = __fmul_rn(acc.y, inv_nu);
                            acc.z = __fmul_rn(acc.z, inv_nu); acc.w = __fmul_rn(acc.w, inv_nu);
                        } else {
                            acc.x = __fdiv_rn(acc.x, nu); acc.y = __fdiv_rn(acc.y, nu);
                            acc.z = __fdiv_rn(acc.z, nu); acc.w = __fdiv_rn(acc.w, nu);
                        }
                    }
                    if (accumulate) {
                        const float4 o = o4[f];
                        acc = combine4(o, acc, accumulate);
                    }
                    o4[f] = acc;
                }
            }
        }
        __syncthreads();
    }
}

template <int NU>
static int launch_decode_staged(const void *codes, const void *l, const float *lbub, const UserOffsets &uoff,
                                int64_t n_chunks, const float *codebook, const int64_t *seg_start,
                                int n_seg, float s, int mean, int accumulate, float *out, cudaStream_t st)
{
    auto kern = hsq_decode_reduce_staged_kernel<NU>;
    const size_t smem = 256 * 128 + (size_t)2 * NU * 2 * kStTile + (size_t)NU * n_seg * 8 + (size_t)(n_seg + 1) * 8;
    GQ_CUDA(cudaFuncSetAttribute(kern, cudaFuncAttributeMaxDynamicSharedMemorySize, (int)smem));
    int occ = 1;
    GQ_CUDA(cudaOccupancyMaxActiveBlocksPerMultiprocessor(&occ, kern, kDecodeThreads, smem));
    const int64_t n_tiles = (n_chunks + kStTile - 1) / kStTile;
    const int64_t cap = (int64_t)sm_count() * (occ < 1 ? 1 : occ);
    const int64_t per = (n_tiles + cap - 1) / cap;
    int64_t grid = (n_tiles + per - 1) / per;
    if (grid < 1) grid = 1;
    const Rider rider = take_rider();
    const PeerWait wait = take_wait();
    GQ_CUDA(launch_pdl(kern, dim3((unsigned)grid), dim3(kDecodeThreads), smem, st, (const uint8_t *)codes,
                       (const uint8_t *)l, lbub, uoff, n_chunks, codebook, seg_start, n_seg, s, mean,
                       accumulate, out, rider, wait));
    return GQ_OK;
}

template <int D, int MAXU, typename CodeT, typename LT>
static int launch_decode_warp(const void *codes, const void *l, const float *lbub, const float *norms_f32,
                              const UserOffsets &uoff, int n_users, int64_t n_chunks, const float *codebook,
                              int K, const int64_t *seg_start, int n_seg, float s, int n_bit, int mean,
                              int accumulate, float *out, cudaStream_t st)
{
    const size_t cb_bytes = (size_t)K * D * 4;
    auto kern = hsq_decode_reduce_warp_kernel<D, MAXU, CodeT, LT>;
    GQ_CUDA(cudaFuncSetAttribute(kern, cudaFuncAttributeMaxDynamicSharedMemorySize, (int)cb_bytes));
    int occ = 1;
    GQ_CUDA(cudaOccupancyMaxActiveBlocksPerMultiprocessor(&occ, kern, kDecodeThreads, cb_bytes));
    const int64_t iters = (n_chunks + 31) / 32;
    const int64_t wblocks = (iters + kDecodeThreads / 32 - 1) / (kDecodeThreads / 32);
    int64_t cap = (int64_t)sm_count() * (occ < 1 ? 1 : occ);
    int grid = (int)(wblocks < cap ? wblocks : cap);
    GQ_CUDA(launch_pdl(kern, dim3(grid < 1 ? 1 : grid), dim3(kDecodeThreads), cb_bytes, st, (const CodeT *)codes,
                       (const LT *)l, lbub, norms_f32, uoff, n_users, n_chunks, codebook, K, seg_start, n_seg, s,
                       n_bit, mean, accumulate, out));
    return GQ_OK;
}

template <int D, typename CodeT, typename LT>
static int launch_decode_d(const void *codes, const void *l, const float *lbub, const float *norms_f32,
                           int64_t user_stride, const int64_t *user_offsets, int n_users, int64_t n_chunks,
                           const float *codebook, int K, const int64_t *seg_start, int n_seg, int n_bit,
                           int mean, int accumulate, float *out, cudaStream_t st)
{
    const float s = (n_bit == 32) ? 1.0f : (float)(1u << n_bit);
    const size_t cb_bytes = (size_t)K * D * 4;
    const int64_t span = (int64_t)kDecodeThreads * kDecodeUnroll;
    const int64_t blocks = (n_chunks * (D / 4) + span - 1) / span;
    constexpr int D4c = D / 4;
    constexpr bool kWarpPath = ((D4c & (D4c - 1)) == 0) && D4c <= 4;
    constexpr int DW = kWarpPath ? D : 16;
    if (kWarpPath && cb_bytes <= 64 * 1024 && n_users <= 8) {
        UserOffsets uoff;
        for (int u = 0; u < 8; ++u)
            uoff.off[u] = (u < n_users) ? (user_offsets ? user_offsets[u] : (int64_t)u * user_stride) : 0;
        bool staged = true;
        if (const char *e = getenv("GQ_DECODE_STAGED")) staged = atoi(e) != 0;
        if (staged && D == 16 && K == 256 && sizeof(CodeT) == 1 && sizeof(LT) == 1 && n_bit != 32 &&
            (size_t)n_users * n_seg * 8 <= 48 * 1024) {
            bool aligned = (((uintptr_t)codes | (uintptr_t)l | (uintptr_t)lbub) & 15) == 0;
            for (int u = 0; u < n_users; ++u) aligned = aligned && ((uoff.off[u] & 15) == 0);
            if (aligned) {
#define GQ_S(MU) case MU: return launch_decode_staged<MU>(codes, l, lbub, uoff, n_chunks, codebook, seg_start, n_seg, s, mean, accumulate, out, st)
                switch (n_users) {
                    GQ_S(1); GQ_S(2); GQ_S(3); GQ_S(4); GQ_S(5); GQ_S(6); GQ_S(7); GQ_S(8);
                    default: break;
                }
#undef GQ_S
            }
        }
        GQ_CUDA_INT(flush_wait(st));
#define GQ_W(MU) return launch_decode_warp<DW, MU, CodeT, LT>(codes, l, lbub, norms_f32, uoff, n_users, n_chunks, codebook, K, seg_start, n_seg, s, n_bit, mean, accumulate, out, st)
        if (n_users == 1) GQ_W(1);
        if (n_users == 2) GQ_W(2);
        if (n_users <= 4) GQ_W(4);
        GQ_W(8);
#undef GQ_W
    }
    if (user_offsets != nullptr) {
        set_error("scattered user records need chunk dim 4/8/16, a codebook <= 64 KB and <= 8 users");
        return GQ_ERR_UNSUPPORTED;
    }
    GQ_CUDA_INT(flush_wait(st));
    if (cb_bytes <= 64 * 1024) {
        auto kern = hsq_decode_reduce_kernel<D, CodeT, LT, true>;
        GQ_CUDA(cudaFuncSetAttribute(kern, cudaFuncAttributeMaxDynamicSharedMemorySize, (int)cb_bytes));
        int occ = 1;
        GQ_CUDA(cudaOccupancyMaxActiveBlocksPerMultiprocessor(&occ, kern, kDecodeThreads, cb_bytes));
        int64_t cap = (int64_t)sm_count() * (occ < 1 ? 1 : occ);
        int grid = (int)(blocks < cap ? blocks : cap);
        kern<<<grid < 1 ? 1 : grid, kDecodeThreads, cb_bytes, st>>>(
            (const CodeT *)codes, (const LT *)l, lbub, norms_f32, user_stride, n_users, n_chunks,
            codebook, K, seg_start, n_seg, s, n_bit, mean, accumulate, out);
    } else {
        auto kern = hsq_decode_reduce_kernel<D, CodeT, LT, false>;
        int64_t cap = (int64_t)sm_count() * 8;
        int grid = (int)(blocks < cap ? blocks : cap);
        kern<<<grid < 1 ? 1 : grid, kDecodeThreads, 0, st>>>(
            (const CodeT *)codes, (const LT *)l, lbub, norms_f32, user_stride, n_users, n_chunks,
            codebook, K, seg_start, n_seg, s, n_bit, mean, accumulate, out);
    }
    GQ_LAUNCH_CHECK("hsq_decode_reduce");
    return GQ_OK;
}

template <typename CodeT, typename LT>
static int launch_decode(const void *codes, const void *l, const float *lbub, const float *norms_f32,
                         int64_t user_stride, const int64_t *user_offsets, int n_users, int64_t n_chunks, int d,
                         const float *codebook, int K, const int64_t *seg_start, int n_seg, int n_bit,
                         int mean, int accumulate, float *out, cudaStream_t st)
{
    switch (d) {
#define GQ_CASE(DD) case DD: return launch_decode_d<DD, CodeT, LT>(codes, l, lbub, norms_f32, user_stride, user_offsets, n_users, n_chunks, codebook, K, seg_start, n_seg, n_bit, mean, accumulate, out, st);
        GQ_CASE(4) GQ_CASE(8) GQ_CASE(12) GQ_CASE(16) GQ_CASE(24) GQ_CASE(32) GQ_CASE(48) GQ_CASE(64)
#undef GQ_CASE
        default: break;
    }
    if (user_offsets != nullptr) {
        set_error("scattered user records are not supported for chunk dim %d", d);
        return GQ_ERR_UNSUPPORTED;
    }
    const float s = (n_bit == 32) ? 1.0f : (float)(1u << n_bit);
    GQ_CUDA_INT(flush_wait(st));
    hsq_decode_reduce_generic_kernel<CodeT, LT><<<grid_for(n_chunks * (int64_t)d, 256), 256, 0, st>>>(
        (const CodeT *)codes, (const LT *)l, lbub, norms_f32, user_stride, n_users, n_chunks, d,
        codebook, seg_start, n_seg, s, n_bit, mean, accumulate, out);
    GQ_LAUNCH_CHECK("hsq_decode_reduce_generic");
    return GQ_OK;
}

int hsq_decode_reduce(const void *codes, int code_bytes, const void *l, int l_bytes, const float *lbub,
                      const float *norms_f32, int64_t user_stride, const int64_t *user_offsets, int n_users,
                      int64_t n_chunks, int d,
                      const float *codebook, int K, const int64_t *seg_start, int n_seg, int n_bit,
                      int mean, int accumulate, float *out, cudaStream_t st)
{
    if (n_chunks == 0) return GQ_OK;
#define GQ_GO(CT, LTT) return launch_decode<CT, LTT>(codes, l, lbub, norms_f32, user_stride, user_offsets, n_users, n_chunks, d, codebook, K, seg_start, n_seg, n_bit, mean, accumulate, out, st)
    if (code_bytes == 1 && l_bytes == 1) GQ_GO(uint8_t, uint8_t);
    if (code_bytes == 1 && l_bytes == 4) GQ_GO(uint8_t, int32_t);
    if (code_bytes == 4 && l_bytes == 1) GQ_GO(int32_t, uint8_t);
    GQ_GO(int32_t, int32_t);
#undef GQ_GO
}

__global__ void __launch_bounds__(256)
f32_reduce_users_kernel(const float *__restrict__ in, int64_t user_stride, int n_users, int64_t n,
                        int mean, int accumulate, float *__restrict__ out)
{
    pdl_launch_dependents();
    pdl_wait();
    for (int64_t i = (int64_t)blockIdx.x * 256 + threadIdx.x; i < n; i += (int64_t)gridDim.x * 256) {
        float acc = in[i];
        for (int u = 1; u < n_users; ++u)
            acc = __fadd_rn(acc, *reinterpret_cast<const float *>(
                                     reinterpret_cast<const char *>(in) + u * user_stride + 4 * i));
        if (mean) acc = __fdiv_rn(acc, (float)n_users);
        if (accumulate) acc = combine1(out[i], acc, accumulate);
        out[i] = acc;
    }
}

__global__ void __launch_bounds__(256)
f32_reduce_users_scattered_kernel(const float *__restrict__ in, const UserOffsets uoff, int n_users, int64_t n,
                                  int mean, int accumulate, float *__restrict__ out)
{
    for (int64_t i = (int64_t)blockIdx.x * 256 + threadIdx.x; i < n; i += (int64_t)gridDim.x * 256) {
        float acc = 0.0f;
#pragma unroll
        for (int u = 0; u < 8; ++u) {
            if (u < n_users) {
                const float x = *reinterpret_cast<const float *>(reinterpret_cast<const char *>(in) + uoff.off[u] + 4 * i);
                acc = (u == 0) ? x : __fadd_rn(acc, x);
            }
        }
        if (mean) acc = __fdiv_rn(acc, (float)n_users);
        if (accumulate) acc = combine1(out[i], acc, accumulate);
        out[i] = acc;
    }
}

int launch_f32_reduce_users(const float *in, int64_t user_stride, const int64_t *user_offsets, int n_users,
                            int64_t n, int mean, int accumulate, float *out, cudaStream_t st)
{
    if (n == 0) return GQ_OK;
    if (user_offsets != nullptr) {
        GQ_REQUIRE(n_users <= 8, "scattered user records support at most 8 users");
        UserOffsets uoff;
        for (int u = 0; u < 8; ++u) uoff.off[u] = (u < n_users) ? user_offsets[u] : 0;
        f32_reduce_users_scattered_kernel<<<grid_for(n, 256), 256, 0, st>>>(in, uoff, n_users, n, mean, accumulate, out);
        GQ_LAUNCH_CHECK("f32_reduce_users_scattered");
        return GQ_OK;
    }
    GQ_CUDA(launch_pdl(f32_reduce_users_kernel, dim3(grid_for(n, 256)), dim3(256), 0, st, in, user_stride, n_users,
                       n, mean, accumulate, out));
    return GQ_OK;
}

static thread_local PeerWait g_wait = {};
void set_wait(const PeerWait &w) { g_wait = w; }
PeerWait take_wait()
{
    PeerWait w = g_wait;
    g_wait = PeerWait{};
    return w;
}
__global__ void peer_wait_kernel(const PeerWait wait)
{
    pdl_launch_dependents();
    pdl_wait();
    if ((int)threadIdx.x < wait.n) peer_wait_flag(wait.flags + threadIdx.x, wait.epoch, wait.timeout_ns);
}
int flush_wait(cudaStream_t st)
{
    const PeerWait w = take_wait();
    if (w.n <= 0) return GQ_OK;
    GQ_CUDA(launch_pdl(peer_wait_kernel, dim3(1), dim3(32), 0, st, w));
    return GQ_OK;
}

static thread_local Rider g_rider = {};

void set_rider(const Rider &r) { g_rider = r; }

Rider take_rider()
{
    Rider r = g_rider;
    g_rider = Rider{};
    return r;
}

__global__ void __launch_bounds__(256) rider_kernel(const Rider rider)
{
    pdl_launch_dependents();
    pdl_wait();
    rider_run(rider, (int64_t)blockIdx.x * 256 + threadIdx.x, (int64_t)gridDim.x * 256);
}

int launch_rider(const Rider &r, cudaStream_t st)
{
    if (r.n == 0) return GQ_OK;
    GQ_CUDA(launch_pdl(rider_kernel, dim3(grid_for(r.n, 256)), dim3(256), 0, st, r));
    return GQ_OK;
}

__global__ void __launch_bounds__(256)
axpy_kernel(const float *__restrict__ a, const float *__restrict__ b, float alpha, int64_t n,
            float *__restrict__ out, int sub)
{
    for (int64_t i = (int64_t)blockIdx.x * 256 + threadIdx.x; i < n; i += (int64_t)gridDim.x * 256) {
        out[i] = sub ? __fsub_rn(a[i], b[i]) : __fadd_rn(a[i], __fmul_rn(alpha, b[i]));
    }
}

int launch_axpy(const float *a, const float *b, float alpha, int64_t n, float *out, int sub,
                cudaStream_t st)
{
    if (n == 0) return GQ_OK;
    axpy_kernel<<<grid_for(n, 256), 256, 0, st>>>(a, b, alpha, n, out, sub);
    GQ_LAUNCH_CHECK("axpy");
    return GQ_OK;
}

}
```

### gradient-quantization_b200/csrc/hsq_tc2.cu

```cuda
#include <cuda.h>
#include <stdlib.h>
#include <string.h>
#include <time.h>

#include <atomic>
#include <mutex>

#include "gq_internal.cuh"
#include "tc_ptx.cuh"

namespace gq {
namespace tc2 {

using namespace tcptx;

constexpr int kK = 256;
constexpr int kTileM = 128;
constexpr int kGroup = 4;
constexpr int kNumGroups = kK / kGroup;
template <int D>
struct Dim {
    static_assert(D == 8 || D == 16 || D == 32, "chunk dimension");
    static constexpr uint32_t kRowBytes = D * 4;
    static constexpr uint32_t kTileBytes = kTileM * kRowBytes;
// ... 406 lines not shown
                        }
                    }
                    tmem_ld_wait16(sb);
                    if (h + 1 < kK / 32) tmem_ld16(taddr + h * 32 + 32, sa);
#pragma unroll
                    for (int g = 0; g < 4; ++g) {
                        if (PAIR) {
                            gm[h * 8 + 4 + g] = pair_group_max(sb[4 * g], sb[4 * g + 1], sb[4 * g + 2], sb[4 * g + 3]);
                        } else {
                            const float m = fmaxf(fabsf(__uint_as_float(sb[4 * g])), fabsf(__uint_as_float(sb[4 * g + 1])));
                            gm[h * 8 + 4 + g] = max3(m, fabsf(__uint_as_float(sb[4 * g + 2])), fabsf(__uint_as_float(sb[4 * g + 3])));
                        }
                    }
                    if (h + 1 < kK / 32) tmem_ld_wait16(sa);
                }
            }
            tc_fence_before();
            __syncwarp();
            if (lane == 0) mbar_arrive(bar_tempty + 8 * s);
            if (tracer) GQ_TRACE(3, it);
            if (TRACE && quad != 0 && lane == 0) GQ_TRACE(8 + quad, it);

            mbar_wait_hw(bar_full + 8 * s, ph);
            float v[kD];
            {
                const uint32_t arow = smem_u32(s_a) + s * kTileBytes + row * kRowBytes;
                const uint32_t sw = Dim<D>::sw(row);
#pragma unroll
                for (int u = 0; u < kUnits; ++u) {
                    const float4 t = lds_f4(arow + ((u ^ sw) << 4));
                    v[4 * u] = t.x; v[4 * u + 1] = t.y; v[4 * u + 2] = t.z; v[4 * u + 3] = t.w;
                }
            }
            float n2 = 0.0f;
#pragma unroll
            for (int j = 0; j < kD; ++j) n2 = fmaf(v[j], v[j], n2);
            const uint32_t all_loaded = __ballot_sync(0xffffffffu, !(n2 < 0.0f));
            if (lane == 0) mbar_arrive(bar_empty + 8 * s + ((all_loaded == 0u) ? 8u : 0u));
            if (tracer) GQ_TRACE(4, it);

            float am[4];
#pragma unroll
            for (int q = 0; q < 4; ++q) {
                am[q] = max3(gm[16 * q], gm[16 * q + 1], gm[16 * q + 2]);
#pragma unroll
                for (int g = 3; g < 15; g += 2) am[q] = max3(am[q], gm[16 * q + g], gm[16 * q + g + 1]);
                am[q] = fmaxf(am[q], gm[16 * q + 15]);
            }
            const float amax = fmaxf(fmaxf(am[0], am[1]), fmaxf(am[2], am[3]));
            float nrm;
            asm("sqrt.approx.f32 %0, %1;" : "=f"(nrm) : "f"(n2));
            const float thr = amax - margin * nrm;
            uint32_t clo, chi;
            bool special;
            if (FMASK) {
                special = !(n2 < 3.0e38f) || !(amax < 3.0e38f) || (n2 < 1.0e-30f) || !(thr >= 1.0e-30f);
                const uint32_t tb = __float_as_uint(thr);
                const float thrm = __uint_as_float(tb - 1u);
                const float S = __uint_as_float(0x8B000000u - (tb & 0x7F800000u));
                const float T = -__fmul_rn(thrm, S);
                const unsigned long long two2 = pack2(2.0f, 2.0f);
                unsigned long long mk01 = pack2(1.0f, 1.0f), mk23 = mk01;
#pragma unroll
                for (int g = 15; g >= 0; --g) {
                    mk01 = ffma2(mk01, two2, pack2(fma_sat(gm[g], S, T), fma_sat(gm[16 + g], S, T)));
                    mk23 = ffma2(mk23, two2, pack2(fma_sat(gm[32 + g], S, T), fma_sat(gm[48 + g], S, T)));
                }
                float mk[4];
                unpack2(mk01, mk[0], mk[1]);
                unpack2(mk23, mk[2], mk[3]);
                clo = ((__float_as_uint(mk[0]) >> 7) & 0xffffu) | ((__float_as_uint(mk[1]) << 9) & 0xffff0000u);
                chi = ((__float_as_uint(mk[2]) >> 7) & 0xffffu) | ((__float_as_uint(mk[3]) << 9) & 0xffff0000u);
            } else {
                special = !(n2 < 3.0e38f) || !(amax < 3.0e38f) || (n2 < 1.0e-30f);
                uint32_t bl[4] = {0u, 0u, 0u, 0u};
#pragma unroll
                for (int g = 15; g >= 0; --g) {
#pragma unroll
                    for (int q = 0; q < 4; ++q)
                        bl[q] = __funnelshift_l(__float_as_uint(gm[16 * q + g] - thr), bl[q], 1);
                }
                clo = ~((bl[0] & 0xffffu) | (bl[1] << 16));
                chi = ~((bl[2] & 0xffffu) | (bl[3] << 16));
            }
            if (special || (clo | chi) == 0u) {
                uint32_t any = 0u;
#pragma unroll
                for (int j = 0; j < kD; ++j) any |= __float_as_uint(v[j]);
                const bool zero = (any << 1) == 0u;
                clo = zero ? 1u : 0xffffffffu;
                chi = zero ? 0u : 0xffffffffu;
            }

            if (TRACE) {
                __syncwarp();
                if (tracer) GQ_TRACE(5, it);
            }
            int n_iter = 0;
            int best_bits = -1, best_k = 0;
            float best_u = 0.0f;
            unsigned long long vv[F2 ? kD : 1];
            if constexpr (F2) {
#pragma unroll
                for (int j = 0; j < kD; ++j) vv[j] = pack2(v[j], v[j]);
            }
            auto score_group = [&](int g, float (&p)[kGroup]) {
                if constexpr (F2) {
                    const uint32_t slot = pbase + (uint32_t)g * 256u;
                    unsigned long long a01, a23;
#pragma unroll
                    for (int t = 0; t < kD / 2; ++t) {
                        unsigned long long c0, c1, e0, e1;
                        lds_2x64(slot + uo[t], c0, c1);
                        lds_2x64(slot + 128u + uo[t], e0, e1);
                        if (t == 0) {
                            a01 = fmul2(c0, vv[0]);
                            a23 = fmul2(e0, vv[0]);
                        } else {
                            a01 = ffma2(c0, vv[2 * t], a01);
                            a23 = ffma2(e0, vv[2 * t], a23);
                        }
                        a01 = ffma2(c1, vv[2 * t + 1], a01);
                        a23 = ffma2(e1, vv[2 * t + 1], a23);
                    }
                    unpack2(a01, p[0], p[1]);
                    unpack2(a23, p[2], p[3]);
                } else {
                    const uint32_t rowa = pbase + (uint32_t)(g * kGroup) * 128u;
#pragma unroll
                    for (int u = 0; u < kUnits; ++u) {
#pragma unroll
                        for (int i = 0; i < kGroup; ++i) {
                            const float4 c = lds_f4(rowa + 128u * i + uo[u]);
                            p[i] = (u == 0) ? __fmul_rn(c.x, v[0]) : __fmaf_rn(c.x, v[4 * u], p[i]);
                            p[i] = __fmaf_rn(c.y, v[4 * u + 1], p[i]);
                            p[i] = __fmaf_rn(c.z, v[4 * u + 2], p[i]);
                            p[i] = __fmaf_rn(c.w, v[4 * u + 3], p[i]);
                        }
                    }
                }
            };
            auto take_group = [&](int g, const float (&p)[kGroup]) {
                const float gmax = fmaxf(fmaxf(fabsf(p[0]), fabsf(p[1])), fmaxf(fabsf(p[2]), fabsf(p[3])));
                const int gb = __float_as_int(gmax);
                const float psum = (p[0] + p[1]) + (p[2] + p[3]);
                if (gb > best_bits || psum != psum) {
#pragma unroll
                    for (int i = 0; i < kGroup; ++i) {
                        const int ab = __float_as_int(p[i]) & 0x7fffffff;
                        if (ab > best_bits) { best_bits = ab; best_k = g * kGroup + i; best_u = p[i]; }
                    }
                }
            };
            uint32_t cur = clo, nxt = chi;
            int gbase = 0;
            if (cur == 0u) { cur = nxt; nxt = 0u; gbase = 32; }
            while (cur != 0u) {
                const int g0 = gbase + __ffs((int)cur) - 1;
                cur &= cur - 1u;
                if (cur == 0u) { cur = nxt; nxt = 0u; gbase = 32; }
                if constexpr (R2) {
                    int g1 = g0;
                    if (cur != 0u) {
                        g1 = gbase + __ffs((int)cur) - 1;
                        cur &= cur - 1u;
                        if (cur == 0u) { cur = nxt; nxt = 0u; gbase = 32; }
                    }
                    float p0[kGroup], p1[kGroup];
                    score_group(g0, p0);
                    score_group(g1, p1);
                    take_group(g0, p0);
                    take_group(g1, p1);
                } else {
                    float p0[kGroup];
                    score_group(g0, p0);
                    take_group(g0, p0);
                }
                if (TRACE) ++n_iter;
            }
            __syncwarp();
            if (TRACE) {
                n_iter = (int)__reduce_max_sync(0xffffffffu, (unsigned)n_iter);
                if (tracer) {
                    GQ_TRACE(6, it);
                    if (blockIdx.x == 0 && it < 128) P.trace[8 * 128 + it] = n_iter;
                }
            }
            if (valid) P.u_out[c] = best_u;
            if (codes16) {
                uint8_t *slot = s_codes + (warp - 4) * 32;
                slot[lane] = valid ? (uint8_t)best_k : (uint8_t)0;
                __syncwarp();
                if ((lane & 15) == 0) {
                    const uint4 w = *reinterpret_cast<const uint4 *>(slot + lane);
                    if (c + 15 < n_chunks) {
                        *reinterpret_cast<uint4 *>(P.codes + c) = w;
                    } else {
                        for (int t = 0; t < 16; ++t)
                            if (c + t < n_chunks) P.codes[c + t] = slot[lane + t];
                    }
                    if (P.remote.n > 0 && c < n_chunks) remote_st128(P.remote, P.codes + c, w);
                }
                __syncwarp();
            } else if (valid) {
                P.codes[c] = (uint8_t)best_k;
            }
            if (P.keys != nullptr) {
                if (!keys_ready) {
                    unsigned long long seen;
                    uint32_t spins = 0;
#pragma unroll 1
                    do {
                        asm volatile("ld.acquire.gpu.global.u64 %0, [%1];" : "=l"(seen) : "l"(P.flag) : "memory");
                        if (seen == P.id) break;
                        __nanosleep(64);
                    } while (++spins < (1u << 22));
                    if (seen != P.id) __trap();
                    keys_ready = true;
                }
                const int seg = valid ? cached_segment(segc, P.seg_start, P.n_seg, (int64_t)c) : -1;
                minmax_add_warp(mm, valid, seg, best_u, P.keys);
            }
            if (tracer) GQ_TRACE(7, it);
        }
        if (P.keys != nullptr) minmax_flush_warp(mm, P.keys);
    }

    tc_fence_before();
    __syncthreads();
    tc_fence_after();
    if (warp == 2) {
        asm volatile("tcgen05.dealloc.cta_group::1.sync.aligned.b32 %0, %1;" ::"r"(tmem_base), "r"(512));
    }
    GQ_STAMP(1);
    if (P.l == nullptr) return;

    if (threadIdx.x == 0) {
        __threadfence();
        atomicAdd(P.barrier, 1u);
    }
    const int n_seg = P.n_seg;
    int *s_seg = reinterpret_cast<int *>(smem + L::kOffA);
    float2 *s_lbub = reinterpret_cast<float2 *>(smem + L::kOffA + 4 * ((n_seg + 2) & ~1));
    for (int i = threadIdx.x; i <= n_seg; i += kThreads) s_seg[i] = (int)P.seg_start[i];
    const Remote &R = P.remote;
    const int c_begin = tile0 * kTileM;
    const int c_end = min((tile0 + my_tiles) * kTileM, n_chunks);
    const int qb = c_begin >> 2, qe = (c_end + 3) >> 2;
    const float s = P.s;
    const int random = P.random;
    const bool ext = random && P.uniforms != nullptr;
    const bool philox = random && P.uniforms == nullptr;
    const bool philox_aligned = (P.offset & 3u) == 0;
    constexpr int J = 5;
    auto load_pass = [&](int q0, float4 (&xv)[J], float4 (&rv)[J]) {
#pragma unroll
        for (int j = 0; j < J; ++j) {
            const int q = q0 + j * kThreads;
            xv[j] = make_float4(0.f, 0.f, 0.f, 0.f);
            rv[j] = make_float4(0.f, 0.f, 0.f, 0.f);
            if (q < qe) {
                if (q * 4 + 3 < n_chunks) {
                    xv[j] = __ldcg(reinterpret_cast<const float4 *>(P.u_out) + q);
                    if (ext) rv[j] = __ldg(reinterpret_cast<const float4 *>(P.uniforms) + q);
                } else {
                    float x[4] = {0.f, 0.f, 0.f, 0.f}, r[4] = {0.f, 0.f, 0.f, 0.f};
                    for (int t = 0; t < 4; ++t) {
                        if (q * 4 + t < n_chunks) {
                            x[t] = __ldcg(P.u_out + q * 4 + t);
                            if (ext) r[t] = __ldg(P.uniforms + q * 4 + t);
                        }
                    }
                    xv[j] = make_float4(x[0], x[1], x[2], x[3]);
                    rv[j] = make_float4(r[0], r[1], r[2], r[3]);
                }
            }
        }
        if (philox) {
#pragma unroll
            for (int j = 0; j < J; ++j) {
                const int q = q0 + j * kThreads;
                if (q >= qe) continue;
                const int i0 = q * 4;
                if (philox_aligned) {
                    const uint4 w = philox4x32_10(P.seed, (P.offset + (uint64_t)i0) >> 2);
                    rv[j] = make_float4(u01(w.x), u01(w.y), u01(w.z), u01(w.w));
                } else {
                    rv[j] = make_float4(philox_uniform(P.seed, P.offset, (uint64_t)i0), philox_uniform(P.seed, P.offset, (uint64_t)(i0 + 1)),
                                        philox_uniform(P.seed, P.offset, (uint64_t)(i0 + 2)), philox_uniform(P.seed, P.offset, (uint64_t)(i0 + 3)));
                }
            }
        }
    };
    auto finish_pass = [&](int q0, const float4 (&xv)[J], const float4 (&rv)[J], int &seg) {
#pragma unroll
        for (int j = 0; j < J; ++j) {
            const int q = q0 + j * kThreads;
            const bool act = q < qe;
            uint32_t packed = 0u;
            if (act) {
            const int i0 = q * 4;
            const float x[4] = {xv[j].x, xv[j].y, xv[j].z, xv[j].w};
            const float r[4] = {rv[j].x, rv[j].y, rv[j].z, rv[j].w};
            while (i0 >= s_seg[seg + 1]) ++seg;
            int lv[4];
            if (i0 + 3 < s_seg[seg + 1]) {
                const float2 bb = s_lbub[seg];
                if (bb.x - bb.y == 0.0f) {
                    lv[0] = lv[1] = lv[2] = lv[3] = 0;
                } else {
                    const float den = __fsub_rn(bb.y, bb.x);
#pragma unroll
                    for (int t = 0; t < 4; ++t) {
                        const float scaled = fabsf(__fdiv_rn(__fsub_rn(x[t], bb.x), den)) * s;
                        const float cl = fminf(fmaxf(scaled, 0.0f), s - 1.0f);
                        int li = (int)cl;
                        if (random) li += (__fsub_rn(scaled, (float)li) > r[t]) ? 1 : 0;
                        lv[t] = li;
                    }
                }
            } else {
                int sg = seg;
#pragma unroll
                for (int t = 0; t < 4; ++t) {
                    const int i = i0 + t;
                    if (i < n_chunks) {
                        while (i >= s_seg[sg + 1]) ++sg;
                        const float2 bb = s_lbub[sg];
                        lv[t] = psc_level(x[t], bb.x, bb.y, s, random, r[t]);
                    } else {
                        lv[t] = 0;
                    }
                }
            }
            packed = (uint32_t)lv[0] | ((uint32_t)lv[1] << 8) | ((uint32_t)lv[2] << 16) | ((uint32_t)lv[3] << 24);
            if (i0 + 3 < n_chunks) {
                reinterpret_cast<uint32_t *>(P.l)[q] = packed;
            } else {
                for (int t = 0; t < 4; ++t)
                    if (i0 + t < n_chunks) P.l[i0 + t] = (uint8_t)lv[t];
            }
            }
            if (R.n > 0) {
                const uint32_t p1 = __shfl_down_sync(0xffffffffu, packed, 1), p2 = __shfl_down_sync(0xffffffffu, packed, 2);
                const uint32_t p3 = __shfl_down_sync(0xffffffffu, packed, 3);
                if (act && (threadIdx.x & 3) == 0)
                    remote_st128(R, reinterpret_cast<uint32_t *>(P.l) + q, make_uint4(packed, p1, p2, p3));
            }
        }
    };
    float4 xv[J], rv[J];
    int q0 = qb + (int)threadIdx.x;
    load_pass(q0, xv, rv);
    if (threadIdx.x == 0) {
        uint32_t seen, spins = 0;
        do {
            asm volatile("ld.acquire.gpu.global.u32 %0, [%1];" : "=r"(seen) : "l"(P.barrier) : "memory");
            if (seen >= gridDim.x) break;
            __nanosleep(32);
        } while (++spins < (1u << 24));
        if (seen < gridDim.x) __trap();
    }
    __syncthreads();
    GQ_STAMP(2);
    for (int i = threadIdx.x; i < n_seg; i += kThreads) {
        const float lb = key_to_float(__ldcg(P.keys + 2 * i)), ub = key_to_float(__ldcg(P.keys + 2 * i + 1));
        s_lbub[i] = make_float2(lb, ub);
        if (blockIdx.x == 0) {
            P.lbub[2 * i] = lb;
            P.lbub[2 * i + 1] = ub;
            if (R.n > 0) {
                remote_st32(R, P.lbub + 2 * i, __float_as_uint(lb));
                remote_st32(R, P.lbub + 2 * i + 1, __float_as_uint(ub));
            }
        }
    }
    __syncthreads();
    {
        int seg = 0;
        {
            int lo = 0, hi = n_seg;
            while (hi - lo > 1) {
                const int mid = (lo + hi) >> 1;
                if (s_seg[mid] <= c_begin) lo = mid; else hi = mid;
            }
            seg = lo;
        }
        finish_pass(q0, xv, rv, seg);
        for (q0 += J * kThreads; q0 - (int)threadIdx.x < qe; q0 += J * kThreads) {
            load_pass(q0, xv, rv);
            finish_pass(q0, xv, rv, seg);
        }
    }
    if (TRACE) __syncthreads();
    GQ_STAMP(3);
    if (R.n > 0) {
        const int64_t n16 = R.ident_bytes >> 4;
        for (int64_t i = (int64_t)blockIdx.x * kThreads + threadIdx.x; i < n16; i += (int64_t)gridDim.x * kThreads) {
            const uint4 w = __ldcg(reinterpret_cast<const uint4 *>(R.ident) + i);
            remote_st128(R, const_cast<uint8_t *>(R.ident) + 16 * i, w);
        }
        __threadfence_system();
        __syncthreads();
        if (threadIdx.x == 0) {
            const uint32_t prev = atomicAdd(R.done, 1u);
            s_misc[0] = (prev == gridDim.x - 1) ? 1 : 0;
            __threadfence_system();
        }
        __syncthreads();
        if (s_misc[0] && (int)threadIdx.x < R.n_flag)
            asm volatile("st.release.sys.global.u32 [%0], %1;" ::"l"(R.flag[threadIdx.x]), "r"(R.epoch) : "memory");
    }
}

typedef CUresult (*EncodeTiledFn)(CUtensorMap *, CUtensorMapDataType, cuuint32_t, void *, const cuuint64_t *,
                                  const cuuint64_t *, const cuuint32_t *, const cuuint32_t *,
                                  CUtensorMapInterleave, CUtensorMapSwizzle, CUtensorMapL2promotion,
                                  CUtensorMapFloatOOBfill);

static EncodeTiledFn encode_fn()
{
    static EncodeTiledFn fn = nullptr;
    static std::once_flag once;
    std::call_once(once, [] {
        void *p = nullptr;
        cudaDriverEntryPointQueryResult q;
        if (cudaGetDriverEntryPoint("cuTensorMapEncodeTiled", &p, cudaEnableDefault, &q) == cudaSuccess &&
            q == cudaDriverEntryPointSuccess)
            fn = reinterpret_cast<EncodeTiledFn>(p);
    });
    return fn;
}

static int make_map(CUtensorMap *map, const float *base, int64_t rows, int kD = 16)
{
    EncodeTiledFn fn = encode_fn();
    if (!fn) {
        set_error("cuTensorMapEncodeTiled is not available from the driver");
        return GQ_ERR_CUDA;
    }
    cuuint64_t dims[2] = {(cuuint64_t)kD, (cuuint64_t)rows};
    cuuint64_t strides[1] = {(cuuint64_t)kD * 4};
    cuuint32_t box[2] = {(cuuint32_t)kD, (cuuint32_t)kTileM};
    cuuint32_t estr[2] = {1, 1};
    CUresult r = fn(map, CU_TENSOR_MAP_DATA_TYPE_FLOAT32, 2, const_cast<float *>(base), dims, strides, box, estr,
                    CU_TENSOR_MAP_INTERLEAVE_NONE,
                    kD == 8 ? CU_TENSOR_MAP_SWIZZLE_32B : (kD == 16 ? CU_TENSOR_MAP_SWIZZLE_64B : CU_TENSOR_MAP_SWIZZLE_128B),
                    CU_TENSOR_MAP_L2_PROMOTION_L2_128B,
                    CU_TENSOR_MAP_FLOAT_OOB_FILL_NONE);
    if (r != CUDA_SUCCESS) {
        set_error("cuTensorMapEncodeTiled failed with CUresult %d (base %p, rows %lld)", (int)r, (const void *)base,
                  (long long)rows);
        return GQ_ERR_CUDA;
    }
    return GQ_OK;
}

struct Variant {
    int groups;
    bool pair, fmask, f2, r2;
};

static Variant pick_variant()
{
    Variant v = {3, true, true, true, false};
    if (const char *e = getenv("GQ_TC2")) {
        if (strstr(e, "g4")) v.groups = 4;
        if (strstr(e, "g3")) v.groups = 3;
        if (strstr(e, "nopair")) v.pair = false; else if (strstr(e, "pair")) v.pair = true;
        if (strstr(e, "nofmask")) v.fmask = false; else if (strstr(e, "fmask")) v.fmask = true;
        if (strstr(e, "nof2")) v.f2 = false; else if (strstr(e, "f2")) v.f2 = true;
        if (strstr(e, "r1")) v.r2 = false; else if (strstr(e, "r2")) v.r2 = true;
    }
    return v;
}

template <int G, bool PAIR, bool FMASK, bool F2, bool R2, int D = 16>
static int launch_one(const CUtensorMap &mg, const Enc2 &P, int grid, cudaStream_t st)
{
    auto kern = hsq_encode_tc2_kernel<G, PAIR, FMASK, F2, R2, false, D>;
    static bool attr_set = false;
    if (!attr_set) {
        GQ_CUDA(cudaFuncSetAttribute(kern, cudaFuncAttributeMaxDynamicSharedMemorySize, (int)Layout<G, D>::kSmemBytes));
        attr_set = true;
    }
    GQ_CUDA(launch_pdl(kern, dim3(grid), dim3(128 + 128 * G), (size_t)Layout<G, D>::kSmemBytes, st, mg, P));
    return GQ_OK;
}

static int launch_variant(const Variant &v, const CUtensorMap &mg, const Enc2 &P, int grid, cudaStream_t st)
{
    const int sel = (v.groups == 4 ? 16 : 0) | (v.pair ? 8 : 0) | (v.fmask ? 4 : 0) | (v.f2 ? 2 : 0) | (v.r2 ? 1 : 0);
    switch (sel) {
    case 0: return launch_one<3, false, false, false, false>(mg, P, grid, st);
    case 8: return launch_one<3, true, false, false, false>(mg, P, grid, st);
    case 12: return launch_one<3, true, true, false, false>(mg, P, grid, st);
    case 13: return launch_one<3, true, true, false, true>(mg, P, grid, st);
    case 14: return launch_one<3, true, true, true, false>(mg, P, grid, st);
    case 15: return launch_one<3, true, true, true, true>(mg, P, grid, st);
    case 9: return launch_one<3, true, false, false, true>(mg, P, grid, st);
    case 16 + 14: return launch_one<4, true, true, true, false>(mg, P, grid, st);
    case 16 + 15: return launch_one<4, true, true, true, true>(mg, P, grid, st);
    case 16 + 13: return launch_one<4, true, true, false, true>(mg, P, grid, st);
    case 16 + 12: return launch_one<4, true, true, false, false>(mg, P, grid, st);
    default:
        set_error("GQ_TC2: this combination of switches is not built");
        return GQ_ERR_UNSUPPORTED;
    }
}


}

int hsq_tc2_trace(const float *grad, int64_t n_chunks, const float *codebook, void *codes, float *u_out,
                  const int64_t *seg_start, int n_seg, uint32_t *keys, uint64_t *flag, uint32_t *barrier,
                  const Tc2Tail *tail, long long *trace, cudaStream_t st)
{
    using namespace tc2;
    GQ_REQUIRE(((uintptr_t)grad & 15) == 0 && ((uintptr_t)codebook & 15) == 0, "TMA needs 16-byte aligned bases");
    GQ_REQUIRE(n_chunks > 0 && n_chunks < ((int64_t)1 << 31) - 256 && trace, "bad arguments");
    CUtensorMap mg;
    int e = make_map(&mg, grad, n_chunks);
    if (e) return e;
    static std::atomic<unsigned long long> counter{0x7ace000000000000ull};
    Enc2 P = {};
    P.codebook = codebook;
    P.n_chunks = (int)n_chunks;
    P.codes = (uint8_t *)codes;
    P.u_out = u_out;
    P.trace = trace;
    if (tail != nullptr) {
        P.seg_start = seg_start;
        P.n_seg = n_seg;
        P.keys = keys;
        P.flag = reinterpret_cast<unsigned long long *>(flag);
        P.id = counter.fetch_add(1) + 1;
        P.l = tail->l;
        P.lbub = tail->lbub;
        P.barrier = barrier;
        P.uniforms = tail->uniforms;
        P.seed = tail->seed;
        P.offset = tail->offset;
        P.s = (float)(1u << tail->n_bit);
        P.random = tail->random;
    }
    const int n_tiles = (int)((n_chunks + kTileM - 1) / kTileM);
    int sms = sm_count();
    if (const char *g = getenv("GQ_TC_GRID")) {
        int v = atoi(g);
        if (v > 0 && v < sms) sms = v;
    }
    const int grid = n_tiles < sms ? n_tiles : sms;
    const Variant v = pick_variant();
    auto launch = [&](auto kern, int threads, size_t smem) -> int {
        GQ_CUDA(cudaFuncSetAttribute(kern, cudaFuncAttributeMaxDynamicSharedMemorySize, (int)smem));
        GQ_CUDA(launch_pdl(kern, dim3(grid), dim3(threads), smem, st, mg, P));
        return GQ_OK;
    };
    if (v.groups == 4) e = launch(hsq_encode_tc2_kernel<4, true, true, true, true, true>, 640, Layout<4>::kSmemBytes);
    else if (v.r2) e = launch(hsq_encode_tc2_kernel<3, true, true, true, true, true>, 512, Layout<3>::kSmemBytes);
    else e = launch(hsq_encode_tc2_kernel<3, true, true, true, false, true>, 512, Layout<3>::kSmemBytes);
    if (e) return e;
    GQ_LAUNCH_CHECK("hsq_tc2_trace");
    return GQ_OK;
}

bool hsq_tc2_supported(int d, int K, int code_bytes)
{
    return (d == 8 || d == 16 || d == 32) && K == tc2::kK && code_bytes == 1;
}

bool hsq_tc2_tail_supported(int n_seg, int n_bit, int l_bytes, const void *u_out, const void *uniforms, const void *l,
                            const void *codes)
{
    return n_seg <= tc2::kTailMaxSeg && n_bit >= 1 && n_bit <= 7 && l_bytes == 1 && ((uintptr_t)u_out & 15) == 0 &&
           ((uintptr_t)uniforms & 15) == 0 && ((uintptr_t)l & 3) == 0 && ((uintptr_t)codes & 3) == 0;
}

int hsq_encode_tc2(const float *grad, int64_t n_chunks, int d, const float *codebook, void *codes, float *u_out,
                   const int64_t *seg_start, int n_seg, uint32_t *keys, uint64_t *flag, uint32_t *barrier,
                   const Rider &rider, const Tc2Tail *tail, const Tc2Remote *remote, cudaStream_t st)
{
    using namespace tc2;
    GQ_REQUIRE(d == 8 || d == 16 || d == 32, "tcgen05 encode: chunk dimension %d (8, 16 or 32)", d);
    GQ_REQUIRE(((uintptr_t)grad & 15) == 0 && ((uintptr_t)codebook & 15) == 0, "TMA needs 16-byte aligned bases");
    GQ_REQUIRE(n_chunks > 0 && n_chunks < ((int64_t)1 << 31) - 256, "n_chunks out of range for one tensor map");
    CUtensorMap mg;
    int e = make_map(&mg, grad, n_chunks, d);
    if (e) return e;
    static std::atomic<unsigned long long> counter{[] {
        unsigned long long seed = (unsigned long long)(uintptr_t)&seed ^ (unsigned long long)clock();
        seed = seed * 6364136223846793005ull + 1442695040888963407ull;
        return (seed >> 16) << 32;
    }()};
    Enc2 P = {};
    P.codebook = codebook;
    P.n_chunks = (int)n_chunks;
    P.codes = (uint8_t *)codes;
    P.u_out = u_out;
    P.seg_start = seg_start;
    P.n_seg = n_seg;
    P.keys = keys;
    P.flag = keys ? reinterpret_cast<unsigned long long *>(flag) : nullptr;
    P.id = counter.fetch_add(1) + 1;
    P.rider = rider;
    if (tail != nullptr) {
        GQ_REQUIRE(keys && flag && barrier, "the fused tail needs keys, flag and barrier scratch");
        P.l = tail->l;
        P.lbub = tail->lbub;
        P.barrier = barrier;
        P.uniforms = tail->uniforms;
        P.seed = tail->seed;
        P.offset = tail->offset;
        P.s = (float)(1u << tail->n_bit);
        P.random = tail->random;
        if (remote != nullptr && remote->n > 0) {
            GQ_REQUIRE(((uintptr_t)codes & 15) == 0 && ((uintptr_t)tail->l & 15) == 0,
                       "remote delivery needs 16-byte aligned codes / l sections");
            Remote &R = P.remote;
            R.n = remote->n;
            R.multicast = remote->multicast;
            for (int i = 0; i < 7; ++i) R.delta[i] = i < remote->n ? remote->delta[i] : 0;
            R.ident = remote->ident;
            R.ident_bytes = remote->ident_bytes;
            R.done = barrier + 1;
            R.n_flag = remote->n_flag;
            for (int i = 0; i < 8; ++i) R.flag[i] = i < remote->n_flag ? remote->flag[i] : nullptr;
            R.epoch = remote->epoch;
        }
    }
    const int n_tiles = (int)((n_chunks + kTileM - 1) / kTileM);
    int sms = sm_count();
    if (const char *g = getenv("GQ_TC_GRID")) {
        int v = atoi(g);
        if (v > 0 && v < sms) sms = v;
    }
    const int grid = n_tiles < sms ? n_tiles : sms;
// ... 15 lines not shown
```

### gradient-quantization_b200/quantizers/fused.py

```python
import torch

from .. import _lib
from ..compressors import (IdenticalCompressor, NearestNeighborCompressor, QSGDCompressor,
                           SignSGDCompressor, TopKSparsificationCompressor)
from ..compressors._common import chunk_dim, load_codebook

_ALIGN = 256


def _up(x, a=_ALIGN):
    return (x + a - 1) // a * a


class _Group:

    def __init__(self, kind, key):
        self.kind, self.key = kind, key
        self.tensors = []
        self.sizes = []
        self.arena_off = 0
        self.n = 0

    def add(self, idx, size):
        self.tensors.append(idx)
        self.sizes.append(size)
        self.n += size


class FusedPlan:
    SUPPORTED = (NearestNeighborCompressor, QSGDCompressor, SignSGDCompressor,
                 TopKSparsificationCompressor, IdenticalCompressor)

    @classmethod
    def supports(cls, Compressor):
        return Compressor in cls.SUPPORTED

    def __init__(self, Compressor, shapes, args, device, n_users):
        self.Compressor = Compressor
        self.shapes = [tuple(s) for s in shapes]
        self.sizes = [int(torch.Size(s).numel()) for s in self.shapes]
        self.args = args
        self.device = device
        self.n_users = n_users
        self.random = 1 if getattr(args, "random", True) else 0
        self.algo = getattr(args, "hsq_algo", _lib.ALGO_AUTO)
        self.groups = []
        self._classify()
        self._layout()
        self.arena = torch.zeros(self.arena_elems, dtype=torch.float32, device=device)
        self.records = torch.zeros(n_users, self.record_bytes, dtype=torch.uint8, device=device)
        self.workspace = torch.empty(max(self.workspace_bytes, _ALIGN), dtype=torch.uint8, device=device)
        self.u_scratch = torch.empty(max(self.max_chunks, 1), dtype=torch.float32, device=device)

    def _classify(self):
        a = self.args
        by_key = {}
        order = []

        def group(kind, key):
            if (kind, key) not in by_key:
                by_key[(kind, key)] = _Group(kind, key)
                order.append((kind, key))
            return by_key[(kind, key)]

        self.tensor_group = []
        for i, size in enumerate(self.sizes):
            if size <= 1000 or self.Compressor is IdenticalCompressor:
                g = group("identity", None)
            elif self.Compressor is NearestNeighborCompressor:
                assert a.c_dim > 0 and a.k_bit >= 0 and a.n_bit > 0
                dim = chunk_dim(size, a.c_dim)
                assert size % dim == 0, "not divisible size {} c_dim {} dim {}".format(size, a.c_dim, dim)
                K = dim if a.k_bit <= 0 else 2 ** a.k_bit
                if K == dim:
                    raise _lib.GQError("fused plan: random orthogonal codebooks (K == dim) are per-tensor; "
                                       "use the per-parameter path")
                g = group("hsq", (dim, K))
            elif self.Compressor is QSGDCompressor:
                dim = chunk_dim(size, a.c_dim)
                assert dim != 0 and size % dim == 0
                g = group("qsgd", "tensor" if (a.c_dim == 0 or size < a.c_dim) else dim)
            elif self.Compressor is SignSGDCompressor:
                g = group("sign", None)
            elif self.Compressor is TopKSparsificationCompressor:
                g = group("topk", None)
            else:
                raise _lib.GQError("fused plan does not support %r" % (self.Compressor,))
            g.add(i, size)
            self.tensor_group.append(g)
        for (kind, key), g in by_key.items():
            if kind == "hsq":
                pairs = sorted(zip(g.tensors, g.sizes), key=lambda p: (p[1] // key[0]) % 16 != 0)
                g.tensors, g.sizes = [p[0] for p in pairs], [p[1] for p in pairs]
        self.groups = [by_key[k] for k in order if k[0] != "identity"]
        self.groups += [by_key[k] for k in order if k[0] == "identity"]

    def _layout(self):
        a = self.args
        dev = self.device
        off_el = 0
        rec = 0
        ws = 0
        self.max_chunks = 0
        self.tensor_off = [0] * len(self.sizes)
        for g in self.groups:
            off_el = _up(off_el * 4) // 4
            g.arena_off = off_el
            t_off = off_el
            for idx, size in zip(g.tensors, g.sizes):
                self.tensor_off[idx] = t_off
                t_off += size
            off_el += g.n
            if g.kind == "hsq":
                dim, K = g.key
                g.dim, g.K = dim, K
                g.n_chunks = g.n // dim
                g.n_seg = len(g.tensors)
                starts = [0]
                for size in g.sizes:
                    starts.append(starts[-1] + size // dim)
                g.seg_start = torch.tensor(starts, dtype=torch.int64, device=dev)
                g.seg_start_host = starts
                g.codebook = torch.from_numpy(load_codebook(dim, K)).to(dev)
                g.code_bytes = 1 if a.k_bit <= 8 else 4
                g.n_bit = a.n_bit
                g.l_bytes = 1 if a.n_bit <= 7 else 4
                g.codes_off = rec
                rec += _up(g.n_chunks * g.code_bytes)
                g.l_off = rec
                rec += _up(g.n_chunks * (4 if a.n_bit == 32 else g.l_bytes))
                g.lbub_off = rec
                rec += _up(g.n_seg * 8)
                ws = max(ws, _lib.value("gq_hsq_encode_workspace_bytes", g.n_chunks, dim, K, g.n_seg))
                self.max_chunks = max(self.max_chunks, g.n_chunks)
            elif g.kind == "qsgd":
                g.n_bit = a.n_bit
                g.bits = _lib.value("gq_qsgd_wire_bits", a.n_bit)
                if g.key == "tensor":
                    g.dim = 0
                    g.n_chunks = len(g.tensors)
                    starts = [0]
                    for size in g.sizes:
                        starts.append(starts[-1] + size)
                    g.chunk_start = torch.tensor(starts, dtype=torch.int64, device=dev)
                else:
                    g.dim = g.key
                    g.n_chunks = g.n // g.dim
                    g.chunk_start = None
                g.norm_off = rec
                rec += _up(g.n_chunks * 4)
                g.packed_off = rec
                rec += _up((g.n + 3) // 4 * 4 * g.bits // 8)
            elif g.kind == "sign":
                g.t5 = getattr(a, "sign_wire", "2bit") == "t5"
                g.wire_bytes = int(_lib.value("gq_sign_t5_bytes", g.n)) if g.t5 else (g.n + 3) // 4
                g.packed_off = rec
                rec += _up(g.wire_bytes)
            elif g.kind == "topk":
                g.n_seg = len(g.tensors)
                starts, ks, kp = [0], [], [0]
                for size in g.sizes:
                    starts.append(starts[-1] + size)
                    ks.append(size // a.cr)
                    kp.append(kp[-1] + ks[-1])
                g.k_total = kp[-1]
                g.seg_start = torch.tensor(starts, dtype=torch.int64, device=dev)
                g.k = torch.tensor(ks, dtype=torch.int64, device=dev)
                g.k_prefix = torch.tensor(kp[:-1], dtype=torch.int64, device=dev)
                g.idx_off = rec
                rec += _up(g.k_total * 4)
                g.val_off = rec
                rec += _up(g.k_total * 4)
                ws = max(ws, _lib.value("gq_topk_workspace_bytes", g.n, g.n_seg))
            elif g.kind == "identity":
                g.raw_off = rec
                rec += _up(g.n * 4)
        self.arena_elems = _up(off_el * 4) // 4
        self.record_bytes = _up(rec)
        self.workspace_bytes = ws

    def make_parts(self, n_parts):
        n_parts = max(1, int(n_parts))
        for g in self.groups:
            g.part_cuts = None
            if g.kind != "hsq" or n_parts == 1 or g.n_bit == 32:
                continue
            starts = g.seg_start_host
            cuts = [0]
            for k in range(1, n_parts):
                target = g.n_chunks * k // n_parts
                t = next((i for i in range(cuts[-1] + 1, g.n_seg) if starts[i] >= target and starts[i] % 16 == 0), None)
                if t is None:
                    break
                cuts.append(t)
            cuts.append(g.n_seg)
            if len(cuts) > 2:
                g.part_cuts = cuts
                g.part_seg = [torch.tensor([x - starts[cuts[k]] for x in starts[cuts[k]:cuts[k + 1] + 1]],
                                           dtype=torch.int64, device=self.device) for k in range(len(cuts) - 1)]
        self.n_parts = max([len(g.part_cuts) - 1 for g in self.groups if getattr(g, "part_cuts", None)] or [1])
        return self.n_parts

    def _part_range(self, g, part):
        cuts = getattr(g, "part_cuts", None)
        if cuts is None:
            return (0, g.n_seg, 0, g.n_chunks) if part == 0 else None
        if part >= len(cuts) - 1:
            return None
        ta, tb = cuts[part], cuts[part + 1]
        return ta, tb, g.seg_start_host[ta], g.seg_start_host[tb]

    def part_byte_ranges(self, part):
        out = []
        for g in self.groups:
            if g.kind == "hsq" and getattr(g, "part_cuts", None) is not None:
                r = self._part_range(g, part)
                if r is None:
                    continue
                ta, tb, ca, cb = r
                out.append((g.codes_off + ca * g.code_bytes, g.codes_off + cb * g.code_bytes))
                out.append((g.l_off + ca * g.l_bytes, g.l_off + cb * g.l_bytes))
                out.append((g.lbub_off + 8 * ta, g.lbub_off + 8 * tb))
            elif part == 0:
                if g.kind == "hsq":
                    out.append((g.codes_off, g.lbub_off + _up(g.n_seg * 8)))
                elif g.kind == "qsgd":
                    out.append((g.norm_off, g.packed_off + _up((g.n + 3) // 4 * 4 * g.bits // 8)))
                elif g.kind == "sign":
                    out.append((g.packed_off, g.packed_off + _up(g.wire_bytes)))
                elif g.kind == "topk":
                    out.append((g.idx_off, g.val_off + _up(g.k_total * 4)))
                elif g.kind == "identity" and g.n:
                    out.append((g.raw_off, g.raw_off + _up(g.n * 4)))
        return out

    def view(self, i, buf=None):
        buf = self.arena if buf is None else buf
        o = self.tensor_off[i]
        return buf[o:o + self.sizes[i]].view(self.shapes[i])

    def views(self, buf=None):
        return [self.view(i, buf) for i in range(len(self.sizes))]

    def locate(self, tensors):
        if len(tensors) != len(self.sizes) or not tensors:
            return None
        base = tensors[0].data_ptr() - self.tensor_off[0] * 4
        for t, o in zip(tensors, self.tensor_off):
            if t.data_ptr() != base + o * 4 or t.dtype != torch.float32 or not t.is_contiguous():
                return None
        return base if base % 256 == 0 else None

    def gather(self, tensors, buf=None, feedback=0, scale=0.0):
        import ctypes
        buf = self.arena if buf is None else buf
        base = buf.data_ptr()
        ptrs, offs, sizes, keep = [], [], [], []
        for i, t in enumerate(tensors):
            if t.data_ptr() == base + self.tensor_off[i] * 4 and not feedback:
                continue
            if t.dtype != torch.float32 or not t.is_contiguous():
                t = _lib.f32c(t.detach())
                keep.append(t)
            _lib.require_cuda(t, "gradient")
            ptrs.append(t.data_ptr())
            offs.append(self.tensor_off[i])
            sizes.append(self.sizes[i])
        n = len(ptrs)
        if n:
            _lib.call("gq_gather_f32", (ctypes.c_void_p * n)(*ptrs), (ctypes.c_int64 * n)(*offs),
                      (ctypes.c_int64 * n)(*sizes), n, base, int(feedback), float(scale), _lib.stream())

    def compressed_elems(self):
        return sum(g.n for g in self.groups if g.kind != "identity")

    def total_elems(self):
        return sum(self.sizes)

    def wire_bytes(self):
        b = 0
        for g in self.groups:
            if g.kind == "hsq":
                b += g.n_chunks * g.code_bytes + g.n_chunks * (4 if g.n_bit == 32 else g.l_bytes) + g.n_seg * 8
            elif g.kind == "qsgd":
                b += g.n_chunks * 4 + (g.n * g.bits + 7) // 8
            elif g.kind == "sign":
                b += g.wire_bytes
            elif g.kind == "topk":
                b += g.k_total * 8
            else:
                b += g.n * 4
        return b

    def split_uniform_stream(self, stream, skip=()):
        per_group = {id(g): {} for g in self.groups}
        pos = 0
        for i, g in enumerate(self.tensor_group):
            if g.kind == "hsq":
                n = self.sizes[i] // g.dim
            elif g.kind == "qsgd":
                n = self.sizes[i]
            else:
                continue
            if i in skip:
                chunk = torch.zeros(n, dtype=torch.float32)
            else:
                chunk = torch.as_tensor(stream[pos:pos + n], dtype=torch.float32)
                assert chunk.numel() == n, "uniform stream exhausted"
                pos += n
            per_group[id(g)][i] = chunk
        out = {}
        for g in self.groups:
            if per_group[id(g)]:
                out[id(g)] = torch.cat([per_group[id(g)][i] for i in g.tensors]).to(self.device)
        return out, pos

    def encode(self, user, src=None, uniforms=None, rng_user=None, shared_rng=False, part=None):
        src = self.arena if src is None else src
        src_ptr = src if isinstance(src, int) else src.data_ptr()
        rng_user = user if rng_user is None else rng_user
        take = _lib.PHILOX.take_shared if shared_rng else (lambda n: _lib.PHILOX.take(n, rng_user))
        rec = self.records[user]
        st = _lib.stream()
        base = rec.data_ptr()
        ident, carrier = self._rider_pair()
        if part is not None and not hasattr(self, "n_parts"):
            raise _lib.GQError("encode(part=...) needs make_parts() first")
        for g in self.groups:
            gp = src_ptr + g.arena_off * 4
            r = None if uniforms is None else uniforms.get(id(g))
            if part is not None:
                if g.kind == "hsq" and getattr(g, "part_cuts", None) is not None:
                    pr = self._part_range(g, part)
                    if pr is None:
                        continue
                    ta, tb, ca, cb = pr
                    if g is carrier and part == 0:
                        _lib.call("gq_attach_f32_reduce", src_ptr + ident.arena_off * 4, 0, None, 1, ident.n, 0, 0,
                                  base + ident.raw_off)
                    if part == 0:
                        n_rand = g.n_chunks if self.random else 0
                        g._part_rng = take(n_rand) if (n_rand and r is None) else (0, 0)
                    seed, off = g._part_rng
                    _lib.call("gq_hsq_encode", gp + ca * g.dim * 4, cb - ca, g.dim, _lib.ptr(g.codebook), g.K,
                              _lib.ptr(g.part_seg[part]), tb - ta, g.n_bit, self.random,
                              None if r is None else r.data_ptr() + ca * 4, seed, off + (ca if r is None else 0),
                              base + g.codes_off + ca * g.code_bytes, g.code_bytes, base + g.l_off + ca * g.l_bytes,
                              g.l_bytes, base + g.lbub_off + 8 * ta, self.u_scratch.data_ptr() + ca * 4,
                              _lib.ptr(self.workspace), self.workspace.numel(), self.algo, st)
                    continue
                if part != 0:
                    continue
            if g is carrier:
                _lib.call("gq_attach_f32_reduce", src_ptr + ident.arena_off * 4, 0, None, 1, ident.n, 0, 0,
                          base + ident.raw_off)
            if g.kind == "hsq":
                n_rand = g.n_chunks if (self.random and g.n_bit != 32) else 0
                seed, off = take(n_rand) if (n_rand and r is None) else (0, 0)
                if g.n_bit == 32:
                    _lib.call("gq_hsq_encode", gp, g.n_chunks, g.dim, _lib.ptr(g.codebook), g.K,
                              _lib.ptr(g.seg_start), g.n_seg, 32, 0, None, 0, 0, base + g.codes_off,
                              g.code_bytes, None, 4, None, base + g.l_off, _lib.ptr(self.workspace),
                              self.workspace.numel(), self.algo, st)
                else:
                    _lib.call("gq_hsq_encode", gp, g.n_chunks, g.dim, _lib.ptr(g.codebook), g.K,
                              _lib.ptr(g.seg_start), g.n_seg, g.n_bit, self.random, _lib.ptr(r), seed, off,
                              base + g.codes_off, g.code_bytes, base + g.l_off, g.l_bytes,
                              base + g.lbub_off, _lib.ptr(self.u_scratch), _lib.ptr(self.workspace),
                              self.workspace.numel(), self.algo, st)
            elif g.kind == "qsgd":
                seed, off = take(g.n) if (self.random and r is None) else (0, 0)
                _lib.call("gq_qsgd_encode", gp, g.n, _lib.ptr(g.chunk_start), g.n_chunks, g.dim, g.n_bit,
                          self.random, _lib.ptr(r), seed, off, base + g.norm_off, None, None,
                          base + g.packed_off, st)
            elif g.kind == "sign":
                if g.t5:
                    _lib.call("gq_sign_encode_t5", gp, g.n, base + g.packed_off, st)
                else:
                    _lib.call("gq_sign_encode", gp, g.n, None, base + g.packed_off, st)
            elif g.kind == "topk":
                _lib.call("gq_topk_select", gp, g.n, _lib.ptr(g.seg_start), _lib.ptr(g.k),
                          _lib.ptr(g.k_prefix), g.n_seg, None, base + g.idx_off, base + g.val_off,
                          _lib.ptr(self.workspace), self.workspace.numel(), st)
            elif g.kind == "identity":
                if g.n and carrier is None:
                    _lib.call("gq_f32_reduce_users", gp, 0, 1, g.n, 0, 0, base + g.raw_off, st)

    def _rider_pair(self, n_users=1):
        ident = next((g for g in self.groups if g.kind == "identity" and g.n), None)
        carrier = max((g for g in self.groups if g.kind in ("hsq", "sign", "qsgd", "topk")), key=lambda g: g.n, default=None)
        if ident is None or carrier is None or n_users > 8:
            return None, None
        return ident, carrier

    def supports_scattered(self):
        for g in self.groups:
            if g.kind == "identity":
                continue
            if g.kind != "hsq" or g.dim not in (4, 8, 16) or g.K * g.dim * 4 > 65536 or g.n_bit == 32:
                return False
        return True

    def supports_fused_delivery(self):
        import os
        if os.environ.get("GQ_TC_V", "2") == "1" or self.algo == _lib.ALGO_EXACT:
            return False
        hsq = [g for g in self.groups if g.kind != "identity"]
        if len(hsq) != 1 or hsq[0].kind != "hsq":
            return False
        g = hsq[0]
        return (g.dim in (8, 16, 32) and g.K == 256 and g.code_bytes == 1 and g.n_bit <= 7 and g.l_bytes == 1
                and g.n_seg <= 1024 and g.n_chunks > 0)

    def supports_inplace_feedback(self):
        return all(g.kind != "topk" for g in self.groups)

    def decode(self, first_user=0, n_users=None, mean=True, accumulate=False, out=None,
               base_ptr=None, user_offsets=None, part=None):
        out = self.arena if out is None else out
        n_users = self.n_users if n_users is None else n_users
        st = _lib.stream()
        mean = 1 if mean else 0
        acc = int(accumulate)
        ident, carrier = self._rider_pair(n_users)
        if user_offsets is not None:
            for g in self.groups:
                op = out.data_ptr() + g.arena_off * 4
                if g is carrier:
                    _lib.call("gq_attach_f32_reduce", base_ptr + ident.raw_off, 0, user_offsets, n_users, ident.n,
                              mean, acc, out.data_ptr() + ident.arena_off * 4)
                if g.kind == "hsq":
                    _lib.call("gq_hsq_decode_reduce_scattered", base_ptr + g.codes_off, g.code_bytes,
                              base_ptr + g.l_off, g.l_bytes, base_ptr + g.lbub_off, user_offsets, n_users,
                              g.n_chunks, g.dim, _lib.ptr(g.codebook), g.K, _lib.ptr(g.seg_start), g.n_seg,
                              g.n_bit, mean, acc, op, st)
                elif carrier is None:
                    _lib.call("gq_f32_reduce_users_scattered", base_ptr + g.raw_off, user_offsets, n_users, g.n,
                              mean, acc, op, st)
            return out
        base = self.records.data_ptr() + first_user * self.record_bytes
        stride = self.record_bytes
        for g in self.groups:
            op = out.data_ptr() + g.arena_off * 4
            if part is not None:
                if g.kind == "hsq" and getattr(g, "part_cuts", None) is not None:
                    pr = self._part_range(g, part)
                    if pr is None:
                        continue
                    ta, tb, ca, cb = pr
                    if g is carrier and part == 0:
                        _lib.call("gq_attach_f32_reduce", base + ident.raw_off, stride, None, n_users, ident.n, mean, acc,
                                  out.data_ptr() + ident.arena_off * 4)
                    _lib.call("gq_hsq_decode_reduce", base + g.codes_off + ca * g.code_bytes, g.code_bytes,
                              base + g.l_off + ca * g.l_bytes, g.l_bytes, base + g.lbub_off + 8 * ta, None, stride,
                              n_users, cb - ca, g.dim, _lib.ptr(g.codebook), g.K, _lib.ptr(g.part_seg[part]), tb - ta,
                              g.n_bit, mean, acc, op + ca * g.dim * 4, st)
                    continue
                if part != 0:
                    continue
            if g is carrier:
                _lib.call("gq_attach_f32_reduce", base + ident.raw_off, stride, None, n_users, ident.n, mean, acc,
                          out.data_ptr() + ident.arena_off * 4)
            if g.kind == "hsq":
                if g.n_bit == 32:
                    _lib.call("gq_hsq_decode_reduce", base + g.codes_off, g.code_bytes, None, 1, None,
                              base + g.l_off, stride, n_users, g.n_chunks, g.dim, _lib.ptr(g.codebook), g.K,
                              _lib.ptr(g.seg_start), g.n_seg, 32, mean, acc, op, st)
                else:
                    _lib.call("gq_hsq_decode_reduce", base + g.codes_off, g.code_bytes, base + g.l_off,
                              g.l_bytes, base + g.lbub_off, None, stride, n_users, g.n_chunks, g.dim,
                              _lib.ptr(g.codebook), g.K, _lib.ptr(g.seg_start), g.n_seg, g.n_bit, mean,
                              acc, op, st)
            elif g.kind == "qsgd":
                _lib.call("gq_qsgd_decode_reduce", base + g.norm_off, base + g.packed_off, stride, n_users,
                          g.n, _lib.ptr(g.chunk_start), g.n_chunks, g.dim, g.n_bit, mean, acc, op, st)
            elif g.kind == "sign":
                _lib.call("gq_sign_decode_reduce_t5" if g.t5 else "gq_sign_decode_reduce", base + g.packed_off, stride,
                          n_users, g.n, mean, acc, op, st)
            elif g.kind == "topk":
                _lib.call("gq_topk_scatter_reduce", base + g.idx_off, base + g.val_off, stride, n_users,
                          g.k_total, g.n, mean, acc, op, st)
            elif g.kind == "identity" and carrier is None:
                _lib.call("gq_f32_reduce_users", base + g.raw_off, stride, n_users, g.n, mean, acc, op, st)
        return out

    def launches_per_encode(self):
        per = {"hsq": 3, "qsgd": 3, "sign": 1, "topk": 10, "identity": 1}
        n = 0
        for g in self.groups:
            k = per[g.kind]
            if g.kind == "hsq" and g.n_bit == 32:
                k -= 2
            elif (g.kind == "hsq" and g.dim in (8, 16, 32) and g.K == 256 and g.code_bytes == 1
                  and self.algo != _lib.ALGO_EXACT):
                import os
                v1 = os.environ.get("GQ_TC_V", "2") == "1"
                k -= 1 if (v1 or g.n_seg > 1024 or g.n_bit > 7) else 2
            n += k
        ident, carrier = self._rider_pair()
        if carrier is not None and (carrier.kind != "hsq" or carrier.n_bit != 32):
            n -= 1
        return n

    def launches_per_decode(self, n_users):
        n = 0
        for g in self.groups:
            n += (2 + n_users) if g.kind == "topk" else 1
        ident, carrier = self._rider_pair(n_users)
        if carrier is not None and (carrier.kind != "hsq" or (
                carrier.dim == 16 and carrier.K == 256 and carrier.code_bytes == 1
                and carrier.l_bytes == 1 and carrier.n_bit != 32)):
            n -= 1
        return n
```

### gradient-quantization_b200/quantizers/ps_quantizer.py

```python
import os
import sys

import torch

from .. import _lib
from . import exchange as xch
from ._shared import QuantizerBase, feedback_scale


class PSQuantizer(QuantizerBase):

    def __init__(self, Compressor, parameters, args):
        super().__init__(Compressor, parameters, args)
        self.two_phase = self.args.two_phase
        if self.error_feedback and self.two_phase:
            for param in self.parameters:
                param.server_error = torch.zeros_like(param)
        if self.plan is not None and self.two_phase:
            self._phase2_plan = None
        self.p2p = None
        self.fused_push = False
        if self.distributed and self.plan is not None:
            self._setup_p2p()
        if self.distributed and self.two_phase:
            import torch.distributed as dist
            box = [_lib.PHILOX.share_seed() if self.rank == 0 else None]
            dist.broadcast_object_list(box, src=0)
            _lib.PHILOX.share_seed(box[0])

    def _setup_p2p(self):
        import torch.distributed as dist
        want = getattr(self.args, "p2p", True) and os.environ.get("GQ_P2P", "1") != "0"
        ok = 1 if (want and self.world <= 8 and self.plan.supports_scattered()) else 0
        p2p = None
        err = None
        if ok:
            try:
                from .p2p import PeerRecords
                p2p = PeerRecords(self.plan.record_bytes, self.rank, self.world, self.device)
            except Exception as e:
                err = e
                ok = 0
        flag = torch.tensor([ok], device=self.device)
        dist.all_reduce(flag, op=dist.ReduceOp.MIN)
        if want and err is not None and os.environ.get("GQ_P2P_FALLBACK", "0") != "1":
            raise _lib.GQError("peer-to-peer exchange could not be set up on rank %d: %r (set GQ_P2P=0 to use "
                               "the NCCL all-gather, or GQ_P2P_FALLBACK=1 to fall back automatically)" % (self.rank, err))
        if int(flag.item()) == 1:
            self.p2p = p2p
            self.p2p_mode = os.environ.get("GQ_P2P_MODE", getattr(self.args, "p2p_mode", "push"))
            if self.p2p_mode not in ("push", "gather", "direct"):
                raise _lib.GQError("unknown peer-to-peer mode %r" % (self.p2p_mode,))
            self.plan.records = p2p.records
            self.fused_push = (self.p2p_mode == "push" and os.environ.get("GQ_P2P_FUSED", "1") != "0"
                               and self.plan.supports_fused_delivery())
        elif p2p is not None:
            p2p.close()
        if self.rank == 0:
            print("gq_b200: ps exchange = %s" % self.exchange_name(), file=sys.stderr, flush=True)

    def exchange_name(self):
        if self.p2p is None:
            return "NCCL all-gather"
        if self.p2p_mode == "push":
            how = "NVLS multicast stores" if self.p2p.mc_base else "peer stores"
            return ("push fused into the encode kernel, %s, flags instead of a barrier launch" % how
                    if self.fused_push else "push kernel (%s) + barrier kernel" % how)
        return self.p2p_mode

    def launches_per_step(self):
        n = self.plan.launches_per_encode() + self.plan.launches_per_decode(self.world if self.distributed else self.args.num_users)
        if self.p2p is not None:
            n += {"push": 0 if self.fused_push else 2, "gather": 2, "direct": 1}[self.p2p_mode]
        return n

    def record(self, user, epoch, uniforms=None):
        scale = feedback_scale(self.args, epoch)
        if self.plan is None:
            return self._record_per_parameter(user, scale)
        plan = self.plan
        if self.distributed and user != self.rank:
            raise _lib.GQError("distributed mode: rank %d records user %d only" % (self.rank, self.rank))
        slot = self.p2p.row() if self.p2p is not None else user
        grads = self._grads()
        if not self.error_feedback:
            flat = plan.locate(grads)
            if flat is not None:
                self._encode(slot, user, src=flat, uniforms=uniforms)
                return
        if self.error_feedback and plan.supports_inplace_feedback():
            err = self._ef_buffers(user)
            plan.gather(grads, buf=err, feedback=2, scale=scale)
            self._encode(slot, user, src=err, uniforms=uniforms)
            plan.decode(first_user=slot, n_users=1, mean=False, accumulate=2, out=err)
            return
        plan.gather(grads)
        if self.error_feedback:
            err = self._ef_buffers(user)
            n = plan.arena.numel()
            _lib.call("gq_axpy", _lib.ptr(plan.arena), _lib.ptr(err), float(scale), n,
                      _lib.ptr(plan.arena), _lib.stream())
            for p, v in zip(self.parameters, plan.views()):
                p.grad.data = v
            self._encode(slot, user, uniforms=uniforms)
            dec = plan.decode(first_user=slot, n_users=1, mean=False, out=self._scratch())
            _lib.call("gq_sub", _lib.ptr(plan.arena), _lib.ptr(dec), n, _lib.ptr(err), _lib.stream())
        else:
            self._encode(slot, user, uniforms=uniforms)

    def _encode(self, slot, user, src=None, uniforms=None):
        if self.fused_push:
            self.p2p.attach_delivery(self.plan)
        self.plan.encode(slot, src=src, uniforms=uniforms, rng_user=user)

    def _scratch(self):
        if not hasattr(self, "_scratch_buf"):
            self._scratch_buf = torch.empty_like(self.plan.arena)
        return self._scratch_buf

    def _record_per_parameter(self, user, scale):
        for i, param in enumerate(self.parameters):
            if self.error_feedback:
                param.grad.data.add_(scale * param.error[user])
                decompressed_g = self.compressors[i].decompress(
                    self.compressors[i].compress(param.grad.data))
                param.error[user].data = param.grad.data - decompressed_g
            else:
                decompressed_g = self.compressors[i].decompress(
                    self.compressors[i].compress(param.grad.data))
            self.compressed_gradients[i].append(decompressed_g)

    def encode_local(self, user, src=None, uniforms=None):
        slot = self.p2p.row() if self.p2p is not None else user
        self._encode(slot, user, src=src, uniforms=uniforms)
        return slot

    def exchange_and_decode(self, out=None):
        plan = self.plan
        out = plan.arena if out is None else out
        if self.p2p is not None:
            if self.fused_push:
                self.p2p.attach_wait()
            else:
                if self.p2p_mode == "push":
                    self.p2p.push()
                self.p2p.barrier()
                if self.p2p_mode == "gather":
                    self.p2p.gather()
            g = self.decode_exchanged(out)
            self.p2p.advance()
            return g
        self.exchange()
        return plan.decode(mean=True, out=out)

    def decode_exchanged(self, out=None):
        plan = self.plan
        out = plan.arena if out is None else out
        if self.p2p is None:
            return plan.decode(mean=True, out=out)
        if self.p2p_mode == "direct":
            return plan.decode(n_users=self.world, mean=True, out=out, base_ptr=self.p2p.user0_record_ptr(),
                               user_offsets=self.p2p.user_offsets())
        return plan.decode(first_user=self.p2p.row(0), n_users=self.world, mean=True, out=out)

    def exchange(self):
        if self.distributed:
            xch.ps_all_gather(self.plan.records, self.rank)

    def apply(self, uniforms=None):
        if self.plan is None:
            return self._apply_per_parameter()
        g = self.exchange_and_decode()
        if self.two_phase:
            g = self._second_phase(g, uniforms)
        self._set_grads_from(g)

    def phase2_plan(self):
        from .fused import FusedPlan
        if self._phase2_plan is None:
            self._phase2_plan = FusedPlan(self.plan.Compressor, self.plan.shapes, self.args, self.device, 1)
        return self._phase2_plan

    def _second_phase(self, g, uniforms):
        p2 = self.phase2_plan()
        n = g.numel()
        if self.error_feedback and p2.supports_inplace_feedback():
            if not hasattr(self, "_server_err"):
                self._server_err = torch.zeros_like(g)
                for p, v in zip(self.parameters, self.plan.views(self._server_err)):
                    p.server_error = v
            p2.gather(self.plan.views(g), buf=self._server_err, feedback=1, scale=1.0)
            p2.encode(0, src=self._server_err, uniforms=uniforms, shared_rng=True)
            p2.decode(mean=False, out=g)
            p2.decode(mean=False, accumulate=2, out=self._server_err)
            return g
        if self.error_feedback:
            if not hasattr(self, "_server_err"):
                self._server_err = torch.zeros_like(g)
                for p, v in zip(self.parameters, self.plan.views(self._server_err)):
                    p.server_error = v
            _lib.call("gq_axpy", _lib.ptr(g), _lib.ptr(self._server_err), 1.0, n, _lib.ptr(g), _lib.stream())
        p2.encode(0, src=g, uniforms=uniforms, shared_rng=True)
        dec = p2.decode(mean=False, out=self._scratch())
        if self.error_feedback:
            _lib.call("gq_sub", _lib.ptr(g), _lib.ptr(dec), n, _lib.ptr(self._server_err), _lib.stream())
        g.copy_(dec)
        return g

    def _apply_per_parameter(self):
        for i, param in enumerate(self.parameters):
            stacked = torch.stack([_lib.f32c(t) for t in self.compressed_gradients[i]], dim=0)
            g = torch.empty_like(stacked[0])
            _lib.call("gq_f32_reduce_users", _lib.ptr(stacked), g.numel() * 4, stacked.shape[0],
                      g.numel(), 1, 0, _lib.ptr(g), _lib.stream())
            if self.two_phase:
                if self.error_feedback:
                    g.add_(param.server_error)
                    decompressed_g = self.compressors[i].decompress(self.compressors[i].compress(g))
                    param.server_error = g - decompressed_g
                    g = decompressed_g
                else:
                    g = self.compressors[i].decompress(self.compressors[i].compress(g))
            param.grad.data = g
        for compressed in self.compressed_gradients:
            compressed.clear()
```

### include/gqb200.h

```cpp
#ifndef GQB200_H
#define GQB200_H

#include <stddef.h>
#include <stdint.h>

#ifdef __cplusplus
extern "C" {
#endif

#define GQ_OK 0
#define GQ_ERR_INVALID 1
#define GQ_ERR_CUDA 2
#define GQ_ERR_UNSUPPORTED 3
#define GQ_ERR_WORKSPACE 4

#define GQ_ALGO_AUTO 0
#define GQ_ALGO_EXACT 1
#define GQ_ALGO_TC 2

typedef void *gq_stream_t;

const char *gq_last_error(void);
int gq_abi_version(void);
int gq_device_info(int *sm_count, int *cc_major, int *cc_minor, size_t *total_mem);

size_t gq_hsq_encode_workspace_bytes(int64_t n_chunks, int d, int K, int n_seg);
int gq_hsq_encode(const float *grad, int64_t n_chunks, int d,
                  const float *codebook, int K,
                  const int64_t *seg_start, int n_seg,
                  int n_bit, int random, const float *uniforms,
                  uint64_t philox_seed, uint64_t philox_offset,
                  void *codes, int code_bytes, void *l, int l_bytes,
                  float *lbub, float *u_out,
                  void *workspace, size_t workspace_bytes, int algo, gq_stream_t stream);

int gq_hsq_search(const float *grad, int64_t n_chunks, int d, const float *codebook, int K,
                  void *codes, int code_bytes, float *u_out,
                  const int64_t *seg_start, int n_seg, uint32_t *minmax_keys ,
                  void *workspace, size_t workspace_bytes, int algo, gq_stream_t stream);

int gq_norm_quantize(const float *u, int64_t n, const int64_t *seg_start, int n_seg,
                     int n_bit, int random, const float *uniforms,
                     uint64_t philox_seed, uint64_t philox_offset,
                     void *l, int l_bytes, float *lbub,
                     uint32_t *minmax_keys, int precomputed, gq_stream_t stream);

int gq_norm_dequantize(const void *l, int l_bytes, int64_t n, const int64_t *seg_start, int n_seg,
                       int n_bit, const float *lbub, float *out, gq_stream_t stream);

int gq_hsq_decode_reduce(const void *codes, int code_bytes, const void *l, int l_bytes,
                         const float *lbub, const float *norms_f32,
                         int64_t user_stride_bytes, int n_users,
                         int64_t n_chunks, int d, const float *codebook, int K,
                         const int64_t *seg_start, int n_seg, int n_bit,
                         int mean, int accumulate, float *out, gq_stream_t stream);

int gq_hsq_decode_reduce_scattered(const void *codes, int code_bytes, const void *l, int l_bytes,
                                   const float *lbub, const int64_t *user_byte_offsets, int n_users,
                                   int64_t n_chunks, int d, const float *codebook, int K,
                                   const int64_t *seg_start, int n_seg, int n_bit, int mean, int accumulate,
                                   float *out, gq_stream_t stream);
int gq_f32_reduce_users_scattered(const float *in, const int64_t *user_byte_offsets, int n_users, int64_t n,
                                  int mean, int accumulate, float *out, gq_stream_t stream);

int gq_attach_f32_reduce(const float *in, int64_t user_stride_bytes, const int64_t *user_byte_offsets,
                         int n_users, int64_t n, int mean, int accumulate, float *out);

int gq_f32_reduce_users(const float *in, int64_t user_stride_bytes, int n_users, int64_t n,
                        int mean, int accumulate, float *out, gq_stream_t stream);

int gq_qsgd_wire_bits(int n_bit);
int gq_qsgd_encode(const float *grad, int64_t n, const int64_t *chunk_start, int64_t n_chunks, int dim,
                   int n_bit, int random, const float *uniforms, uint64_t philox_seed,
                   uint64_t philox_offset, float *norm, uint8_t *signs, int32_t *l, void *packed,
                   gq_stream_t stream);
int gq_qsgd_decode_reduce(const float *norm, const void *packed, int64_t user_stride_bytes, int n_users,
                          int64_t n, const int64_t *chunk_start, int64_t n_chunks, int dim, int n_bit,
                          int mean, int accumulate, float *out, gq_stream_t stream);
int gq_qsgd_decode_unpacked(const float *norm, const uint8_t *signs, const int32_t *l, int64_t n,
                            const int64_t *chunk_start, int64_t n_chunks, int dim, int n_bit, float *out,
                            gq_stream_t stream);

int gq_sign_encode(const float *grad, int64_t n, float *out_f32, uint8_t *packed, gq_stream_t stream);
int gq_sign_decode_reduce(const uint8_t *packed, int64_t user_stride_bytes, int n_users, int64_t n,
                          int mean, int accumulate, float *out, gq_stream_t stream);

int64_t gq_sign_t5_bytes(int64_t n);
int gq_sign_encode_t5(const float *grad, int64_t n, void *packed, gq_stream_t stream);
int gq_sign_decode_reduce_t5(const void *packed, int64_t user_stride_bytes, int n_users, int64_t n,
                             int mean, int accumulate, float *out, gq_stream_t stream);

size_t gq_topk_workspace_bytes(int64_t n, int n_seg);
int gq_topk_select(const float *grad, int64_t n, const int64_t *seg_start, const int64_t *k,
                   const int64_t *k_prefix, int n_seg, float *out_dense, int32_t *out_idx,
                   float *out_val, void *workspace, size_t workspace_bytes, gq_stream_t stream);
int gq_topk_scatter_reduce(const int32_t *idx, const float *val, int64_t user_stride_bytes,
                           int n_users, int64_t k_total, int64_t n, int mean, int accumulate,
                           float *out, gq_stream_t stream);

int gq_pvc_search(const float *grad, int64_t n_chunks, int d, const float *dagger, int K,
                  const float *uniforms, uint64_t philox_seed, uint64_t philox_offset,
                  void *codes, int code_bytes, float *u_out, gq_stream_t stream);

int gq_hsq_tc_debug(const float *grad, int64_t n_chunks, const float *codebook, void *codes,
                    float *u_out, const int64_t *seg_start, int n_seg, float *dbg_scores,
                    int dbg_tiles, gq_stream_t stream);

int gq_gather_f32(const void *const *src_ptrs, const int64_t *dst_offsets, const int64_t *sizes,
                  int n_tensors, float *dst, int feedback, float scale, gq_stream_t stream);

int gq_hsq_tc2_trace(const float *grad, int64_t n_chunks, const float *codebook, void *codes,
                     float *u_out, const int64_t *seg_start, int n_seg, void *l, float *lbub,
                     void *workspace, int64_t *trace, gq_stream_t stream);

int gq_ipc_alloc(size_t bytes, void **dev_ptr, void *handle_out_64);
int gq_ipc_free(void *dev_ptr);
int gq_ipc_open(const void *handle_64, void **peer_ptr);
int gq_ipc_close(void *peer_ptr);
int gq_peer_barrier(void *const *flag_ptrs, int rank, int n_ranks, uint32_t epoch, gq_stream_t stream);
int gq_peer_gather(void *dst, void *const *src_ptrs, size_t bytes, size_t dst_stride, int n_ranks,
                   gq_stream_t stream);

int gq_peer_push(const void *src, void *const *dst_ptrs, size_t bytes, int n_dst, gq_stream_t stream);

int gq_peer_push_multicast(const void *src, void *mc_dst, size_t bytes, gq_stream_t stream);

int gq_attach_remote_record(int n_remote, int multicast, const int64_t *delta, const void *ident,
                            int64_t ident_bytes, void *const *flag_ptrs, int n_flags, uint32_t epoch);
int gq_attach_peer_wait(const void *local_flags, int n_ranks, uint32_t epoch);

int gq_axpy(const float *a, const float *b, float alpha, int64_t n, float *out, gq_stream_t stream);
int gq_sub(const float *a, const float *b, int64_t n, float *out, gq_stream_t stream);

size_t gq_hsq_host_scratch_bytes(int64_t n_chunks, int d, int K, int n_seg);
int gq_hsq_roundtrip_host(const float *host_grad, float *host_out, int64_t n_chunks, int d,
                          const float *dev_codebook, int K, const int64_t *dev_seg_start, int n_seg,
                          int n_bit, int random, uint64_t philox_seed, uint64_t philox_offset,
                          void *dev_scratch, size_t scratch_bytes, int algo, gq_stream_t stream);

#ifdef __cplusplus
}
#endif
#endif
```

Baseline: 246.8 billion.

## Defer HSQ norm quantization into the decode kernel for single-user encode/decode

When the plan has a single d=16 HSQ group and one user with no peer transport, encode now runs only the codebook search and leaves the norm scalars in scratch. The norm-level quantization is postponed and fused into the staged decode kernel, which computes the levels, writes them and lbub back to the record, and decodes in the same pass. This removes a separate quantize launch and a round trip of the level array through global memory. The cost is pending-state bookkeeping with a fallback completion path, plus a narrower kernel specialization with higher register pressure under its launch bounds.

```diff
diff --git a/gradient-quantization_b200/_lib.py b/gradient-quantization_b200/_lib.py
--- a/gradient-quantization_b200/_lib.py
+++ b/gradient-quantization_b200/_lib.py
@@ -31,6 +31,11 @@
     "gq_hsq_decode_reduce": (c_int, [c_void_p, c_int, c_void_p, c_int, c_void_p, c_void_p, c_i64, c_int,
                                      c_i64, c_int, c_void_p, c_int, c_void_p, c_int, c_int, c_int, c_int,
                                      c_void_p, c_void_p]),
+    "gq_hsq_encode_search": (c_int, [c_void_p, c_i64, c_int, c_void_p, c_int, c_void_p, c_int, c_void_p, c_int,
+                                     c_void_p, c_void_p, c_size, c_void_p]),
+    "gq_hsq_decode_quantize": (c_int, [c_void_p, c_void_p, c_void_p, c_void_p, c_void_p, c_i64, c_int, c_void_p,
+                                       c_int, c_void_p, c_int, c_int, c_int, c_void_p, c_u64, c_u64, c_int,
+                                       c_void_p, c_void_p]),
     "gq_hsq_decode_reduce_scattered": (c_int, [c_void_p, c_int, c_void_p, c_int, c_void_p, c_void_p, c_int, c_i64,
                                                c_int, c_void_p, c_int, c_void_p, c_int, c_int, c_int, c_int,
                                                c_void_p, c_void_p]),
diff --git a/gradient-quantization_b200/csrc/abi.cu b/gradient-quantization_b200/csrc/abi.cu
--- a/gradient-quantization_b200/csrc/abi.cu
+++ b/gradient-quantization_b200/csrc/abi.cu
@@ -270,6 +270,62 @@
                             philox_offset, l, l_bytes, lbub, keys, 1, stream);
 }
 
+int gq_hsq_encode_search(const float *grad, int64_t n_chunks, int d, const float *codebook, int K,
+                         const int64_t *seg_start, int n_seg, void *codes, int code_bytes, float *u_out,
+                         void *workspace, size_t workspace_bytes, gq_stream_t stream)
+{
+    const Rider rider = take_rider();
+    const Tc2Remote remote = take_remote();
+    GQ_REQUIRE(remote.n == 0, "a remote delivery needs the levels: use gq_hsq_encode");
+    int e = validate_group(grad, n_chunks, d, codebook, K, seg_start, n_seg);
+    if (e) return e;
+    const size_t need = gq_hsq_encode_workspace_bytes(n_chunks, d, K, n_seg);
+    if (workspace_bytes < need || workspace == nullptr) {
+        set_error("workspace too small: %zu < %zu", workspace_bytes, need);
+        return GQ_ERR_WORKSPACE;
+    }
+    GQ_REQUIRE(((uintptr_t)workspace & 255) == 0, "workspace must be 256-byte aligned");
+    GQ_REQUIRE(codes && u_out, "null output pointer");
+    if (tc_generation() != 2 || n_chunks == 0 || !hsq_tc2_supported(d, K, code_bytes)) {
+        set_error("gq_hsq_encode_search runs the second-generation tcgen05 search only (d in {8, 16, 32}, K == 256, "
+                  "uint8 codes, n_chunks > 0); got d=%d K=%d code_bytes=%d n_chunks=%lld",
+                  d, K, code_bytes, (long long)n_chunks);
+        return GQ_ERR_UNSUPPORTED;
+    }
+    uint32_t *keys = reinterpret_cast<uint32_t *>(workspace);
+    uint32_t *barrier = reinterpret_cast<uint32_t *>((char *)workspace + align_up((size_t)n_seg * 2 * sizeof(uint32_t), 256));
+    return hsq_encode_tc2(grad, n_chunks, d, codebook, codes, u_out, seg_start, n_seg, keys,
+                          reinterpret_cast<uint64_t *>(barrier) + 1, nullptr, rider, nullptr, nullptr, as_stream(stream));
+}
+
+static const int64_t kStageChunks = 1024;
+int gq_hsq_decode_quantize(const void *codes, void *l, float *lbub, const float *u, const uint32_t *minmax_keys,
+                           int64_t n_chunks, int d, const float *codebook, int K, const int64_t *seg_start,
+                           int n_seg, int n_bit, int random, const float *uniforms, uint64_t philox_seed,
+                           uint64_t philox_offset, int accumulate, float *out, gq_stream_t stream)
+{
+    const Rider pending = take_rider();
+    int e = validate_group(out, n_chunks, d, codebook, K, seg_start, n_seg);
+    if (e) return e;
+    if (d != 16 || K != 256 || n_chunks == 0 || n_chunks >= ((int64_t)1 << 31) - kStageChunks || n_seg > 1024) {
+        set_error("gq_hsq_decode_quantize: d == 16, K == 256, 1 <= n_seg <= 1024, 0 < n_chunks < 2^31 - 1024 "
+                  "(got d=%d K=%d n_seg=%d n_chunks=%lld)", d, K, n_seg, (long long)n_chunks);
+        return GQ_ERR_UNSUPPORTED;
+    }
+    GQ_REQUIRE(n_bit >= 1 && n_bit <= 7, "uint8 norm codes need n_bit 1..7 (got %d)", n_bit);
+    GQ_REQUIRE(accumulate >= 0 && accumulate <= 2, "accumulate must be 0, 1 or 2");
+    GQ_REQUIRE(codes && l && lbub && u && minmax_keys, "null pointer");
+    GQ_REQUIRE((((uintptr_t)codes | (uintptr_t)l | (uintptr_t)lbub | (uintptr_t)u | (uintptr_t)uniforms |
+                 (uintptr_t)out) & 15) == 0,
+               "codes, l, lbub, u, uniforms and out must be 16-byte aligned");
+    set_rider(pending);
+    e = hsq_decode_quantize(codes, l, lbub, u, minmax_keys, n_chunks, codebook, seg_start, n_seg, n_bit, random,
+                            uniforms, philox_seed, philox_offset, accumulate, out, as_stream(stream));
+    const Rider left = take_rider();
+    if (e) return e;
+    return launch_rider(left, as_stream(stream));
+}
+
 int gq_hsq_decode_reduce(const void *codes, int code_bytes, const void *l, int l_bytes,
                          const float *lbub, const float *norms_f32, int64_t user_stride_bytes,
                          int n_users, int64_t n_chunks, int d, const float *codebook, int K,
diff --git a/gradient-quantization_b200/csrc/gq_common.cuh b/gradient-quantization_b200/csrc/gq_common.cuh
--- a/gradient-quantization_b200/csrc/gq_common.cuh
+++ b/gradient-quantization_b200/csrc/gq_common.cuh
@@ -99,6 +99,21 @@
     uint32_t x = (s == 0) ? w.x : (s == 1) ? w.y : (s == 2) ? w.z : w.w;
     return u01(x);
 }
+__device__ __forceinline__ void philox_uniform4(uint64_t seed, uint64_t offset, uint64_t i, float (&r)[4])
+{
+    const uint64_t g = offset + i;
+    const uint4 a = philox4x32_10(seed, g >> 2);
+    const uint32_t sh = (uint32_t)(g & 3u);
+    if (sh == 0) {
+        r[0] = u01(a.x); r[1] = u01(a.y); r[2] = u01(a.z); r[3] = u01(a.w);
+        return;
+    }
+    const uint4 b = philox4x32_10(seed, (g >> 2) + 1);
+    r[0] = u01(sh == 1 ? a.y : sh == 2 ? a.z : a.w);
+    r[1] = u01(sh == 1 ? a.z : sh == 2 ? a.w : b.x);
+    r[2] = u01(sh == 1 ? a.w : sh == 2 ? b.x : b.y);
+    r[3] = u01(sh == 1 ? b.x : sh == 2 ? b.y : b.z);
+}
 
 __device__ __forceinline__ int find_segment(const int64_t *__restrict__ seg_start, int n_seg, int64_t i)
 {
@@ -156,6 +171,44 @@
     }
     return li;
 }
+__device__ __forceinline__ int psc_level_nz(float v, float lb, float den, float s, int random, float r)
+{
+    const float scaled = fabsf(__fdiv_rn(__fsub_rn(v, lb), den)) * s;
+    const float c = fminf(fmaxf(scaled, 0.0f), s - 1.0f);
+    int li = (int)c;
+    if (random) li += (__fsub_rn(scaled, (float)li) > r) ? 1 : 0;
+    return li;
+}
+template <typename SegT, typename IdxT>
+__device__ __forceinline__ void psc_levels4(const float (&x)[4], const float (&r)[4], IdxT i0, IdxT n,
+                                            const SegT *s_seg, const float2 *s_lbub, int &seg, float s, int random,
+                                            int (&lv)[4])
+{
+    while (i0 >= s_seg[seg + 1]) ++seg;
+    if (i0 + 3 < s_seg[seg + 1]) {
+        const float2 b = s_lbub[seg];
+        if (b.x - b.y == 0.0f) {
+            lv[0] = lv[1] = lv[2] = lv[3] = 0;
+        } else {
+            const float den = __fsub_rn(b.y, b.x);
+#pragma unroll
+            for (int t = 0; t < 4; ++t) lv[t] = psc_level_nz(x[t], b.x, den, s, random, r[t]);
+        }
+    } else {
+        int sg = seg;
+#pragma unroll
+        for (int t = 0; t < 4; ++t) {
+            const IdxT i = i0 + t;
+            if (i < n) {
+                while (i >= s_seg[sg + 1]) ++sg;
+                const float2 b = s_lbub[sg];
+                lv[t] = psc_level(x[t], b.x, b.y, s, random, r[t]);
+            } else {
+                lv[t] = 0;
+            }
+        }
+    }
+}
 __device__ __forceinline__ float psc_value(int l, float lb, float ub, float inv_s)
 {
     return __fadd_rn(__fmul_rn(__fmul_rn((float)l, __fsub_rn(ub, lb)), inv_s), lb);
diff --git a/gradient-quantization_b200/csrc/gq_internal.cuh b/gradient-quantization_b200/csrc/gq_internal.cuh
--- a/gradient-quantization_b200/csrc/gq_internal.cuh
+++ b/gradient-quantization_b200/csrc/gq_internal.cuh
@@ -130,6 +130,10 @@
                       int64_t n_chunks, int d,
                       const float *codebook, int K, const int64_t *seg_start, int n_seg, int n_bit,
                       int mean, int accumulate, float *out, cudaStream_t st);
+int hsq_decode_quantize(const void *codes, void *l, float *lbub, const float *u, const uint32_t *keys,
+                        int64_t n_chunks, const float *codebook, const int64_t *seg_start, int n_seg, int n_bit,
+                        int random, const float *uniforms, uint64_t seed, uint64_t offset, int accumulate,
+                        float *out, cudaStream_t st);
 int launch_f32_reduce_users(const float *in, int64_t user_stride, const int64_t *user_offsets, int n_users,
                             int64_t n, int mean, int accumulate, float *out, cudaStream_t st);
 int launch_axpy(const float *a, const float *b, float alpha, int64_t n, float *out, int sub,
diff --git a/gradient-quantization_b200/csrc/hsq_tail.cu b/gradient-quantization_b200/csrc/hsq_tail.cu
--- a/gradient-quantization_b200/csrc/hsq_tail.cu
+++ b/gradient-quantization_b200/csrc/hsq_tail.cu
@@ -1,4 +1,6 @@
 #include <stdlib.h>
+
+#include <type_traits>
 
 #include "gq_internal.cuh"
 
@@ -46,14 +48,6 @@
 }
 
 constexpr int kQuantMaxSeg = 1024;
-__device__ __forceinline__ int psc_level_nz(float v, float lb, float den, float s, int random, float r)
-{
-    const float scaled = fabsf(__fdiv_rn(__fsub_rn(v, lb), den)) * s;
-    const float c = fminf(fmaxf(scaled, 0.0f), s - 1.0f);
-    int li = (int)c;
-    if (random) li += (__fsub_rn(scaled, (float)li) > r) ? 1 : 0;
-    return li;
-}
 template <typename LT>
 __global__ void __launch_bounds__(256)
 norm_quantize_smem_kernel(const float *__restrict__ u, int n, const int64_t *__restrict__ seg_start,
@@ -119,30 +113,8 @@
             }
         }
         int seg = base < 0 ? 0 : base;
-        while (i0 >= s_segi[seg + 1]) ++seg;
         int lv[4];
-        if (i0 + 3 < s_segi[seg + 1]) {
-            const float2 b = s_lbub2[seg];
-            if (b.x - b.y == 0.0f) {
-                lv[0] = lv[1] = lv[2] = lv[3] = 0;
-            } else {
-                const float den = __fsub_rn(b.y, b.x);
-#pragma unroll
-                for (int t = 0; t < 4; ++t) lv[t] = psc_level_nz(x[t], b.x, den, s, random, r[t]);
-            }
-        } else {
-#pragma unroll
-            for (int t = 0; t < 4; ++t) {
-                const int i = i0 + t;
-                if (i < n) {
-                    while (i >= s_segi[seg + 1]) ++seg;
-                    const float2 b = s_lbub2[seg];
-                    lv[t] = psc_level(x[t], b.x, b.y, s, random, r[t]);
-                } else {
-                    lv[t] = 0;
-                }
-            }
-        }
+        psc_levels4(x, r, i0, n, s_segi, s_lbub2, seg, s, random, lv);
         if (full) {
             if (sizeof(LT) == 1) {
                 reinterpret_cast<uint32_t *>(l)[q] =
@@ -512,6 +484,11 @@
     asm volatile("cp.async.cg.shared.global [%0], [%1], 16;" ::"r"((uint32_t)__cvta_generic_to_shared(smem_dst)),
                  "l"(gsrc) : "memory");
 }
+__device__ __forceinline__ void cp_async16_part(void *smem_dst, const void *gsrc, int src_bytes)
+{
+    asm volatile("cp.async.cg.shared.global [%0], [%1], 16, %2;" ::"r"((uint32_t)__cvta_generic_to_shared(smem_dst)),
+                 "l"(gsrc), "r"(src_bytes) : "memory");
+}
 __device__ __forceinline__ float4 lds128(uint32_t saddr)
 {
     float4 r;
@@ -524,18 +501,28 @@
     asm volatile("ld.shared.u8 %0, [%1];" : "=r"(r) : "r"(saddr) : "memory");
     return r;
 }
-template <int NU>
-__global__ void __launch_bounds__(kDecodeThreads)
-hsq_decode_reduce_staged_kernel(const uint8_t *__restrict__ codes, const uint8_t *__restrict__ l,
-                                const float *__restrict__ lbub, const UserOffsets uoff,
+struct DecQuant {
+    const float *u;
+    const uint32_t *keys;
+    const float *uniforms;
+    uint64_t seed, offset;
+    int random;
+};
+template <int NU, bool QUANT>
+__global__ void __launch_bounds__(kDecodeThreads, QUANT ? 5 : 0)
+hsq_decode_reduce_staged_kernel(const uint8_t *__restrict__ codes, uint8_t *__restrict__ l,
+                                float *__restrict__ lbub, const UserOffsets uoff,
                                 int64_t n_chunks, const float *__restrict__ codebook,
                                 const int64_t *__restrict__ seg_start, int n_seg, float s, int mean,
-                                int accumulate, float *__restrict__ out, const Rider rider, const PeerWait wait)
-{
+                                int accumulate, float *__restrict__ out, const Rider rider, const PeerWait wait,
+                                const DecQuant quant)
+{
+    static_assert(!QUANT || NU == 1, "levels are computed for one user's record");
+    constexpr int kBuf = NU * 2 * kStTile + (QUANT ? 3 * kStTile : 0);
     extern __shared__ float4 s_dyn[];
     float4 *s_cb = s_dyn;
     uint8_t *s_stage = reinterpret_cast<uint8_t *>(s_cb + 256 * 8);
-    float2 *s_lbub = reinterpret_cast<float2 *>(s_stage + 2 * NU * 2 * kStTile);
+    float2 *s_lbub = reinterpret_cast<float2 *>(s_stage + 2 * kBuf);
     int64_t *s_seg = reinterpret_cast<int64_t *>(s_lbub + NU * n_seg);
     __shared__ int64_t s_off[8];
     const int tid = threadIdx.x, lane = tid & 31;
@@ -558,13 +545,28 @@
     auto issue = [&](int64_t tile, int buf) {
         const int64_t c0 = tile * kStTile;
         const int64_t left = n_chunks - c0;
-        const int pieces = (int)(((left < kStTile ? left : (int64_t)kStTile) + 15) >> 4);
+        const int lim = (int)(left < kStTile ? left : (int64_t)kStTile);
+        const int pieces = (lim + 15) >> 4;
+        if (QUANT) {
+            for (int i = tid; i < 64 + 256; i += kDecodeThreads) {
+                if (i < 64) {
+                    if (i < pieces) cp_async16(s_stage + buf * kBuf + i * 16, codes + c0 + i * 16);
+                } else {
+                    const int p = i - 64;
+                    if (4 * p < lim)
+                        cp_async16_part(s_stage + buf * kBuf + kStTile + p * 16, quant.u + c0 + 4 * p,
+                                        4 * min(4, lim - 4 * p));
+                }
+            }
+            asm volatile("cp.async.commit_group;" ::: "memory");
+            return;
+        }
         for (int i = tid; i < NU * 128; i += kDecodeThreads) {
             const int u = i >> 7, which = (i >> 6) & 1, piece = i & 63;
             if (piece < pieces) {
                 const char *src = (which ? reinterpret_cast<const char *>(l) : reinterpret_cast<const char *>(codes)) +
                                   s_off[u] + c0 + piece * 16;
-                cp_async16(s_stage + ((buf * NU + u) * 2 + which) * kStTile + piece * 16, src);
+                cp_async16(s_stage + buf * kBuf + (u * 2 + which) * kStTile + piece * 16, src);
             }
         }
         asm volatile("cp.async.commit_group;" ::: "memory");
@@ -578,17 +580,28 @@
     SegCache segc;
     float4 *o4 = reinterpret_cast<float4 *>(out);
     const int64_t n4 = n_chunks * 4;
-    int64_t tile = blockIdx.x;
+    std::conditional_t<QUANT, int, int64_t> tile = blockIdx.x;
     int buf = 0;
     if (tile < n_tiles) issue(tile, 0);
-    for (int i = tid; i < NU * n_seg; i += kDecodeThreads) {
-        const int u = i / n_seg, sg = i - u * n_seg;
-        const float2 *b = reinterpret_cast<const float2 *>(reinterpret_cast<const char *>(lbub) + s_off[u]);
-        s_lbub[i] = __ldcv(b + sg);
+    if (QUANT) {
+        for (int i = tid; i < n_seg; i += kDecodeThreads) {
+            const float lb = key_to_float(__ldcg(quant.keys + 2 * i)), ub = key_to_float(__ldcg(quant.keys + 2 * i + 1));
+            s_lbub[i] = make_float2(lb, ub);
+            if (blockIdx.x == 0) {
+                lbub[2 * i] = lb;
+                lbub[2 * i + 1] = ub;
+            }
+        }
+    } else {
+        for (int i = tid; i < NU * n_seg; i += kDecodeThreads) {
+            const int u = i / n_seg, sg = i - u * n_seg;
+            const float2 *b = reinterpret_cast<const float2 *>(reinterpret_cast<const char *>(lbub) + s_off[u]);
+            s_lbub[i] = __ldcv(b + sg);
+        }
     }
     rider_run(rider, (int64_t)blockIdx.x * kDecodeThreads + tid, (int64_t)gridDim.x * kDecodeThreads);
     for (; tile < n_tiles; tile += gridDim.x, buf ^= 1) {
-        const int64_t next = tile + gridDim.x;
+        const auto next = tile + gridDim.x;
         if (next < n_tiles) {
             issue(next, buf ^ 1);
             asm volatile("cp.async.wait_group 1;" ::: "memory");
@@ -596,8 +609,45 @@
             asm volatile("cp.async.wait_group 0;" ::: "memory");
         }
         __syncthreads();
-        const uint32_t st = stage0 + (uint32_t)(buf * NU * 2 * kStTile);
+        const uint32_t st = stage0 + (uint32_t)(buf * kBuf);
         const int64_t c0 = tile * kStTile;
+        if (QUANT) {
+            const int i0 = (int)c0 + 4 * tid, n = (int)n_chunks;
+            uint32_t packed = 0u;
+            uint32_t *s_lv = reinterpret_cast<uint32_t *>(s_stage + buf * kBuf + kStTile);
+            if (i0 < n) {
+                const float4 xv = reinterpret_cast<const float4 *>(s_lv)[tid];
+                const float x[4] = {xv.x, xv.y, xv.z, xv.w};
+                float r[4] = {0.f, 0.f, 0.f, 0.f};
+                if (quant.random) {
+                    if (quant.uniforms != nullptr) {
+                        if (i0 + 3 < n) {
+                            const float4 t = __ldg(reinterpret_cast<const float4 *>(quant.uniforms + i0));
+                            r[0] = t.x; r[1] = t.y; r[2] = t.z; r[3] = t.w;
+                        } else {
+#pragma unroll
+                            for (int t = 0; t < 4; ++t) r[t] = (i0 + t < n) ? __ldg(quant.uniforms + i0 + t) : 0.0f;
+                        }
+                    } else {
+                        philox_uniform4(quant.seed, quant.offset, (uint64_t)i0, r);
+                    }
+                }
+                int seg = cached_segment_smem(segc, s_seg, n_seg, (int64_t)i0);
+                int lv[4];
+                psc_levels4(x, r, i0, n, s_seg, s_lbub, seg, s, quant.random, lv);
+                packed = (uint32_t)lv[0] | ((uint32_t)lv[1] << 8) | ((uint32_t)lv[2] << 16) | ((uint32_t)lv[3] << 24);
+                if (i0 + 3 < n) {
+                    reinterpret_cast<uint32_t *>(l)[i0 >> 2] = packed;
+                } else {
+#pragma unroll
+                    for (int t = 0; t < 4; ++t)
+                        if (i0 + t < n) l[i0 + t] = (uint8_t)lv[t];
+                }
+            }
+            __syncthreads();
+            s_lv[tid] = packed;
+            __syncthreads();
+        }
         for (int sl = warp; sl < kStTile / 32; sl += kDecodeThreads / 32) {
             const int64_t c = c0 + sl * 32 + lane;
             if (c0 + sl * 32 >= n_chunks) break;
@@ -683,13 +733,15 @@
     }
 }
 
-template <int NU>
+template <int NU, bool QUANT = false>
 static int launch_decode_staged(const void *codes, const void *l, const float *lbub, const UserOffsets &uoff,
                                 int64_t n_chunks, const float *codebook, const int64_t *seg_start,
-                                int n_seg, float s, int mean, int accumulate, float *out, cudaStream_t st)
-{
-    auto kern = hsq_decode_reduce_staged_kernel<NU>;
-    const size_t smem = 256 * 128 + (size_t)2 * NU * 2 * kStTile + (size_t)NU * n_seg * 8 + (size_t)(n_seg + 1) * 8;
+                                int n_seg, float s, int mean, int accumulate, float *out, cudaStream_t st,
+                                const DecQuant &quant = DecQuant{})
+{
+    auto kern = hsq_decode_reduce_staged_kernel<NU, QUANT>;
+    const size_t buf = (size_t)NU * 2 * kStTile + (QUANT ? 3 * kStTile : 0);
+    const size_t smem = 256 * 128 + 2 * buf + (size_t)NU * n_seg * 8 + (size_t)(n_seg + 1) * 8;
     GQ_CUDA(cudaFuncSetAttribute(kern, cudaFuncAttributeMaxDynamicSharedMemorySize, (int)smem));
     int occ = 1;
     GQ_CUDA(cudaOccupancyMaxActiveBlocksPerMultiprocessor(&occ, kern, kDecodeThreads, smem));
@@ -701,9 +753,20 @@
     const Rider rider = take_rider();
     const PeerWait wait = take_wait();
     GQ_CUDA(launch_pdl(kern, dim3((unsigned)grid), dim3(kDecodeThreads), smem, st, (const uint8_t *)codes,
-                       (const uint8_t *)l, lbub, uoff, n_chunks, codebook, seg_start, n_seg, s, mean,
-                       accumulate, out, rider, wait));
+                       (uint8_t *)l, (float *)lbub, uoff, n_chunks, codebook, seg_start, n_seg, s, mean,
+                       accumulate, out, rider, wait, quant));
     return GQ_OK;
+}
+
+int hsq_decode_quantize(const void *codes, void *l, float *lbub, const float *u, const uint32_t *keys,
+                        int64_t n_chunks, const float *codebook, const int64_t *seg_start, int n_seg, int n_bit,
+                        int random, const float *uniforms, uint64_t seed, uint64_t offset, int accumulate,
+                        float *out, cudaStream_t st)
+{
+    UserOffsets uoff = {};
+    const DecQuant quant = {u, keys, uniforms, seed, offset, random};
+    return launch_decode_staged<1, true>(codes, l, lbub, uoff, n_chunks, codebook, seg_start, n_seg,
+                                         (float)(1u << n_bit), 0, accumulate, out, st, quant);
 }
 
 template <int D, int MAXU, typename CodeT, typename LT>
diff --git a/gradient-quantization_b200/csrc/hsq_tc2.cu b/gradient-quantization_b200/csrc/hsq_tc2.cu
--- a/gradient-quantization_b200/csrc/hsq_tc2.cu
+++ b/gradient-quantization_b200/csrc/hsq_tc2.cu
@@ -732,37 +732,8 @@
             const int i0 = q * 4;
             const float x[4] = {xv[j].x, xv[j].y, xv[j].z, xv[j].w};
             const float r[4] = {rv[j].x, rv[j].y, rv[j].z, rv[j].w};
-            while (i0 >= s_seg[seg + 1]) ++seg;
             int lv[4];
-            if (i0 + 3 < s_seg[seg + 1]) {
-                const float2 bb = s_lbub[seg];
-                if (bb.x - bb.y == 0.0f) {
-                    lv[0] = lv[1] = lv[2] = lv[3] = 0;
-                } else {
-                    const float den = __fsub_rn(bb.y, bb.x);
-#pragma unroll
-                    for (int t = 0; t < 4; ++t) {
-                        const float scaled = fabsf(__fdiv_rn(__fsub_rn(x[t], bb.x), den)) * s;
-                        const float cl = fminf(fmaxf(scaled, 0.0f), s - 1.0f);
-                        int li = (int)cl;
-                        if (random) li += (__fsub_rn(scaled, (float)li) > r[t]) ? 1 : 0;
-                        lv[t] = li;
-                    }
-                }
-            } else {
-                int sg = seg;
-#pragma unroll
-                for (int t = 0; t < 4; ++t) {
-                    const int i = i0 + t;
-                    if (i < n_chunks) {
-                        while (i >= s_seg[sg + 1]) ++sg;
-                        const float2 bb = s_lbub[sg];
-                        lv[t] = psc_level(x[t], bb.x, bb.y, s, random, r[t]);
-                    } else {
-                        lv[t] = 0;
-                    }
-                }
-            }
+            psc_levels4(x, r, i0, n_chunks, s_seg, s_lbub, seg, s, random, lv);
             packed = (uint32_t)lv[0] | ((uint32_t)lv[1] << 8) | ((uint32_t)lv[2] << 16) | ((uint32_t)lv[3] << 24);
             if (i0 + 3 < n_chunks) {
                 reinterpret_cast<uint32_t *>(P.l)[q] = packed;
diff --git a/gradient-quantization_b200/quantizers/fused.py b/gradient-quantization_b200/quantizers/fused.py
--- a/gradient-quantization_b200/quantizers/fused.py
+++ b/gradient-quantization_b200/quantizers/fused.py
@@ -1,3 +1,5 @@
+import os
+
 import torch
 
 from .. import _lib
@@ -48,9 +50,20 @@
         self._classify()
         self._layout()
         self.arena = torch.zeros(self.arena_elems, dtype=torch.float32, device=device)
-        self.records = torch.zeros(n_users, self.record_bytes, dtype=torch.uint8, device=device)
+        self._records = torch.zeros(n_users, self.record_bytes, dtype=torch.uint8, device=device)
+        self._pending = None
         self.workspace = torch.empty(max(self.workspace_bytes, _ALIGN), dtype=torch.uint8, device=device)
         self.u_scratch = torch.empty(max(self.max_chunks, 1), dtype=torch.float32, device=device)
+
+    @property
+    def records(self):
+        self._complete()
+        return self._records
+
+    @records.setter
+    def records(self, buf):
+        self._complete()
+        self._records = buf
 
     def _classify(self):
         a = self.args
@@ -315,12 +328,17 @@
                 out[id(g)] = torch.cat([per_group[id(g)][i] for i in g.tensors]).to(self.device)
         return out, pos
 
-    def encode(self, user, src=None, uniforms=None, rng_user=None, shared_rng=False, part=None):
+    def encode(self, user, src=None, uniforms=None, rng_user=None, shared_rng=False, part=None, defer_levels=False):
         src = self.arena if src is None else src
         src_ptr = src if isinstance(src, int) else src.data_ptr()
         rng_user = user if rng_user is None else rng_user
         take = _lib.PHILOX.take_shared if shared_rng else (lambda n: _lib.PHILOX.take(n, rng_user))
-        rec = self.records[user]
+        if self._pending is not None:
+            if part is None and self._pending[0] == user:
+                self._pending = None
+            else:
+                self._complete()
+        rec = self._records[user]
         st = _lib.stream()
         base = rec.data_ptr()
         ident, carrier = self._rider_pair()
@@ -357,7 +375,12 @@
             if g.kind == "hsq":
                 n_rand = g.n_chunks if (self.random and g.n_bit != 32) else 0
                 seed, off = take(n_rand) if (n_rand and r is None) else (0, 0)
-                if g.n_bit == 32:
+                if defer_levels and part is None and self.can_defer_levels():
+                    _lib.call("gq_hsq_encode_search", gp, g.n_chunks, g.dim, _lib.ptr(g.codebook), g.K,
+                              _lib.ptr(g.seg_start), g.n_seg, base + g.codes_off, g.code_bytes,
+                              _lib.ptr(self.u_scratch), _lib.ptr(self.workspace), self.workspace.numel(), st)
+                    self._pending = (user, g, seed, off, r)
+                elif g.n_bit == 32:
                     _lib.call("gq_hsq_encode", gp, g.n_chunks, g.dim, _lib.ptr(g.codebook), g.K,
                               _lib.ptr(g.seg_start), g.n_seg, 32, 0, None, 0, 0, base + g.codes_off,
                               g.code_bytes, None, 4, None, base + g.l_off, _lib.ptr(self.workspace),
@@ -412,6 +435,28 @@
         return (g.dim in (8, 16, 32) and g.K == 256 and g.code_bytes == 1 and g.n_bit <= 7 and g.l_bytes == 1
                 and g.n_seg <= 1024 and g.n_chunks > 0)
 
+    def can_defer_levels(self):
+        if os.environ.get("GQ_DEFER_LEVELS", "1") == "0":
+            return False
+        if os.environ.get("GQ_TC_V", "2") == "1" or self.algo == _lib.ALGO_EXACT:
+            return False
+        hsq = [g for g in self.groups if g.kind != "identity"]
+        if len(hsq) != 1 or hsq[0].kind != "hsq":
+            return False
+        g = hsq[0]
+        return (g.dim == 16 and g.K == 256 and g.code_bytes == 1 and g.l_bytes == 1 and 1 <= g.n_bit <= 7
+                and g.n_seg <= 1024 and g.n_chunks > 0 and getattr(g, "part_cuts", None) is None)
+
+    def _complete(self):
+        if self._pending is None:
+            return
+        row, g, seed, off, r = self._pending
+        self._pending = None
+        base = self._records.data_ptr() + row * self.record_bytes
+        _lib.call("gq_norm_quantize", _lib.ptr(self.u_scratch), g.n_chunks, _lib.ptr(g.seg_start), g.n_seg, g.n_bit,
+                  self.random, _lib.ptr(r), seed, off, base + g.l_off, g.l_bytes, base + g.lbub_off,
+                  _lib.ptr(self.workspace), 1, _lib.stream())
+
     def supports_inplace_feedback(self):
         return all(g.kind != "topk" for g in self.groups)
 
@@ -423,6 +468,11 @@
         mean = 1 if mean else 0
         acc = int(accumulate)
         ident, carrier = self._rider_pair(n_users)
+        pending = self._pending
+        if pending is not None and not (user_offsets is None and part is None and n_users == 1
+                                        and first_user == pending[0]):
+            self._complete()
+            pending = None
         if user_offsets is not None:
             for g in self.groups:
                 op = out.data_ptr() + g.arena_off * 4
@@ -438,7 +488,7 @@
                     _lib.call("gq_f32_reduce_users_scattered", base_ptr + g.raw_off, user_offsets, n_users, g.n,
                               mean, acc, op, st)
             return out
-        base = self.records.data_ptr() + first_user * self.record_bytes
+        base = self._records.data_ptr() + first_user * self.record_bytes
         stride = self.record_bytes
         for g in self.groups:
             op = out.data_ptr() + g.arena_off * 4
@@ -462,7 +512,14 @@
                 _lib.call("gq_attach_f32_reduce", base + ident.raw_off, stride, None, n_users, ident.n, mean, acc,
                           out.data_ptr() + ident.arena_off * 4)
             if g.kind == "hsq":
-                if g.n_bit == 32:
+                if pending is not None:
+                    _, _, seed, off, r = pending
+                    self._pending = None
+                    _lib.call("gq_hsq_decode_quantize", base + g.codes_off, base + g.l_off, base + g.lbub_off,
+                              _lib.ptr(self.u_scratch), _lib.ptr(self.workspace), g.n_chunks, g.dim,
+                              _lib.ptr(g.codebook), g.K, _lib.ptr(g.seg_start), g.n_seg, g.n_bit, self.random,
+                              _lib.ptr(r), seed, off, acc, op, st)
+                elif g.n_bit == 32:
                     _lib.call("gq_hsq_decode_reduce", base + g.codes_off, g.code_bytes, None, 1, None,
                               base + g.l_off, stride, n_users, g.n_chunks, g.dim, _lib.ptr(g.codebook), g.K,
                               _lib.ptr(g.seg_start), g.n_seg, 32, mean, acc, op, st)
diff --git a/gradient-quantization_b200/quantizers/ps_quantizer.py b/gradient-quantization_b200/quantizers/ps_quantizer.py
--- a/gradient-quantization_b200/quantizers/ps_quantizer.py
+++ b/gradient-quantization_b200/quantizers/ps_quantizer.py
@@ -111,7 +111,8 @@
     def _encode(self, slot, user, src=None, uniforms=None):
         if self.fused_push:
             self.p2p.attach_delivery(self.plan)
-        self.plan.encode(slot, src=src, uniforms=uniforms, rng_user=user)
+        defer = not self.distributed and self.plan.n_users == 1 and self.p2p is None
+        self.plan.encode(slot, src=src, uniforms=uniforms, rng_user=user, defer_levels=defer)
 
     def _scratch(self):
         if not hasattr(self, "_scratch_buf"):
@@ -190,7 +191,7 @@
                 for p, v in zip(self.parameters, self.plan.views(self._server_err)):
                     p.server_error = v
             p2.gather(self.plan.views(g), buf=self._server_err, feedback=1, scale=1.0)
-            p2.encode(0, src=self._server_err, uniforms=uniforms, shared_rng=True)
+            p2.encode(0, src=self._server_err, uniforms=uniforms, shared_rng=True, defer_levels=True)
             p2.decode(mean=False, out=g)
             p2.decode(mean=False, accumulate=2, out=self._server_err)
             return g
@@ -200,7 +201,7 @@
                 for p, v in zip(self.parameters, self.plan.views(self._server_err)):
                     p.server_error = v
             _lib.call("gq_axpy", _lib.ptr(g), _lib.ptr(self._server_err), 1.0, n, _lib.ptr(g), _lib.stream())
-        p2.encode(0, src=g, uniforms=uniforms, shared_rng=True)
+        p2.encode(0, src=g, uniforms=uniforms, shared_rng=True, defer_levels=True)
         dec = p2.decode(mean=False, out=self._scratch())
         if self.error_feedback:
             _lib.call("gq_sub", _lib.ptr(g), _lib.ptr(dec), n, _lib.ptr(self._server_err), _lib.stream())
diff --git a/include/gqb200.h b/include/gqb200.h
--- a/include/gqb200.h
+++ b/include/gqb200.h
@@ -54,6 +54,14 @@
                          int64_t n_chunks, int d, const float *codebook, int K,
                          const int64_t *seg_start, int n_seg, int n_bit,
                          int mean, int accumulate, float *out, gq_stream_t stream);
+
+int gq_hsq_encode_search(const float *grad, int64_t n_chunks, int d, const float *codebook, int K,
+                         const int64_t *seg_start, int n_seg, void *codes, int code_bytes, float *u_out,
+                         void *workspace, size_t workspace_bytes, gq_stream_t stream);
+int gq_hsq_decode_quantize(const void *codes, void *l, float *lbub, const float *u, const uint32_t *minmax_keys,
+                           int64_t n_chunks, int d, const float *codebook, int K, const int64_t *seg_start,
+                           int n_seg, int n_bit, int random, const float *uniforms, uint64_t philox_seed,
+                           uint64_t philox_offset, int accumulate, float *out, gq_stream_t stream);
 
 int gq_hsq_decode_reduce_scattered(const void *codes, int code_bytes, const void *l, int l_bytes,
                                    const float *lbub, const int64_t *user_byte_offsets, int n_users,
```

Measured after the change: 262.9 billion, median of 6. +6.5%, better.
